# SixLabors/ZlibStream

Hardware: AMD Instinct MI355X
Metric: deflate MB/s (input) at level 6, 64 MiB buffers (higher is better)
Workload: dtype u8; 1 GPU; english64: 1 x 67108864-byte pseudo-random-English (Zipf words of alice29.txt) buffer per GPU, level 6, zlib framing, inputs resident in HBM; level=6, buffer_bytes=67108864, buffers_per_gpu=1, compressed_bytes=27425826, parallelism=independent buffers, 1 GPU(s), no collective in the data path

## Files before the change

### zlibstream_amd/csrc/zs_device.h

```cpp
#pragma once
#include <cstddef>
#include "zs_core.h"
#include "zs_lit_engine.h"
#include "zs_fast_sweep.h"
#include "zs_rle.h"

namespace zs {

constexpr int kMatchTile = 16384;
constexpr int kMatchBack = 32512;
constexpr int kMatchFwd = 272;
constexpr int kMatchLdsBytes = kMatchBack + kMatchTile + kMatchFwd;
constexpr int kMatchLdsLinks = kMatchBack + kMatchTile;
constexpr int kMatchLds = kMatchLdsBytes + 2 * kMatchLdsLinks;
constexpr int kAdlerPiece = 65536;

constexpr int64_t kScratchWindow = 0;
constexpr int64_t kScratchHead = 66560;
constexpr int64_t kScratchPrev = kScratchHead + 2 * kHashSize;
constexpr int64_t kScratchHead32 = kScratchPrev + 2 * kWSize;
constexpr int64_t kScratchBytes = kScratchHead32 + 4 * kHashSize;

struct StreamDesc {
    const uint8_t *in;
    uint8_t *out;
    int64_t out_cap;
    int64_t pos_off;
    int64_t sym_off;
    int32_t n;
    int32_t body_end;
    int32_t kl;
    int32_t nchunks;
    int32_t chunk_off;
    int32_t blk_off;
    int32_t max_blocks;
    int32_t adler_off;
    int32_t n_adler;
    int32_t fast_runs;
    int32_t run_off;
    int32_t run_slots;
    int32_t run_chunk;
    int32_t seg_off;
    int32_t nsegs;
    int32_t sup_off;
    const int32_t *seg_c0, *seg_after, *seg_base, *seg_S, *seg_cl;
    const uint32_t *cl;
    const int32_t *cstart;
    const int32_t *head;
    int32_t grid_chunks;
    int32_t n_wr;
    const int64_t *wr_end;
    const uint8_t *wr_flush;
    int32_t *wr_blk;
    int32_t out_chunk, raw;
    const BlockRec *plan_blk;
    int32_t plan_nblk;
    int32_t final_run;
    struct LitPersist *persist;
    int64_t abs_off;
    int32_t cont;
    int32_t resume, start_slot, cont_bits;
    int32_t mid_write;
    uint32_t start_syms;
    int64_t base0, start_block, persist_off, stop_abs;
    int64_t start_pos;
    uint32_t adler_stream;
    uint32_t carry_byte;
    int32_t fv_end;
    uint32_t *ins_bits;
    int32_t cut_off, cut_cap;
    int32_t rle_end, rle_tile_off;
    int32_t fr_first, fr_n;
    int32_t spec, spec_n, spec_off;
};

struct WorkOffsets {
    uint32_t off[10];
};
constexpr int kK5Feeders = 2;
constexpr int kK5Threads = 64 * (1 + kK5Feeders);
constexpr int kSupSegs = 16;
constexpr size_t kFvBitSlack = (16384 + 512) / 8 + 64;

struct LitPersist {
    int64_t base, avail_end, block_start_abs;
    int32_t strstart, lookahead, match_length, match_start, match_available, prev_length, prev_match;
    int32_t pending_syms;
    FlushAcct fa;
    int32_t fa_valid, stopped;
    int32_t good_prev, pad2_[3];
    uint8_t window[kWindowSize + 512];
    uint16_t prev[kWSize];
    uint16_t head[kHashSize];
    uint32_t syms[kLitBufsize];
};
static_assert(offsetof(LitPersist, window) % 16 == 0 && offsetof(LitPersist, prev) % 16 == 0 && offsetof(LitPersist, head) % 16 == 0, "16-byte copies");

struct StreamState {
    int32_t tail_p, tail_kind;
    uint32_t tail_pend;
    int32_t k_done, preins;
    uint32_t body_syms;
    uint32_t nsyms;
    int32_t nblocks;
    int64_t out_len;
    uint32_t adler;
    int32_t status;
    int64_t end_bits;
    int32_t r_seg, r_slot, r_kfired, r_kslot;
    uint32_t r_total;
    int32_t r_ncut;
    int32_t r_cut_e[8], r_cut_done[8];
    int32_t deferred, r_scan;
    int32_t r_cutidx;
    int32_t nc[2], cuts_same, cut_diff_idx, cut_diff_pos;
    int32_t poison;
    int32_t spec_run_tiles, spec_ok, spec_wrong;
};
constexpr uint32_t kSpecBail = 1u << 30;
ZS_HD uint32_t spec_pack(int guess, int exit_slot, int count, bool bail) {
    return (uint32_t)guess | ((uint32_t)exit_slot << 9) | ((uint32_t)count << 18) | (bail ? kSpecBail : 0u);
}
ZS_HD int spec_guess(uint32_t r) { return (int)(r & 0x1FF); }
ZS_HD int spec_exit(uint32_t r) { return (int)((r >> 9) & 0x1FF); }
ZS_HD int spec_count(uint32_t r) { return (int)((r >> 18) & 0xFFF); }
constexpr int kSpecMinInput = 1 << 20;
constexpr int kSpecLenBits = 10;
constexpr int kSpecWarm = 128;
constexpr int kSpecRunsDen = 8;
struct K5Spec {
    uint32_t *rec;
    uint32_t *base;
    int len_bits, warm, corrupt;
    uint32_t *syms;
    int stride;
};
static_assert(spec_slab_stride(kSpecMaxLenBits) - kSpecSlabPad <= 0xFFF, "spec_pack's count field holds the symbols of the longest chunk");
constexpr int kDeferBudget = 8;
constexpr int kCutBudget = 12;

constexpr int kFastChunk = 262144;
constexpr int kFastWarm = 65536;
constexpr int kFastMinInput = 4 << 20;
constexpr int kFastMinPeriodic = 64 << 10;
constexpr int64_t kFastRunSyms = kFastWarm + kFastChunk + 1024;
constexpr int64_t kFastRunBitWords = (kFastWarm + kFastChunk + 2048) / 32;
constexpr int64_t kFastRunScratch = 2 * kHashSize + 4 * kHashSize;
struct FastRunOut {
    int64_t mark_pos, mark_nsyms;
    int64_t end_pos, nsyms;
    int64_t final_base;
    int64_t sym_dst;
    int64_t ev[16];
    int64_t n_match;
    int32_t ok, n_ev;
};

struct BlockInfo {
    int32_t type;
    int32_t bits;
    int64_t bit_start;
};

}
```

### zlibstream_amd/csrc/zs_engine.hip

```cpp
#include <hip/hip_runtime.h>

#include <algorithm>
#include <cstdio>
#include <cstdlib>
#include <cstring>
#include <string>
#include <thread>
#include <vector>

#define ZS_BUILDING_LIBRARY
#include "../../include/zsgpu.h"
#include "zs_kernels.hip"
#include "zs_inflate_par.hip"
#include "zs_inflate_tok.hip"
#include "zs_png.hip"
#include "zs_crc32.hip"

using namespace zs;

namespace {

struct DevBuf {
    void *p = nullptr;
    size_t cap = 0;
};

enum Stage {
    kStClear, kStAdler, kStLinks, kStMatch, kStChunkMap, kStSegMap, kStResolve, kStExpand, kStEmitSyms, kStTail, kStTrees,
    kStOffsets, kStEmitBits, kStSpecWalk, kStSpecVerify, kStCrc32, kStSpecCompact, kStPngExpand, kStCount
};
const char *const kStageNames[kStCount] = {"clear", "adler", "links", "match", "chunkmap", "segmap", "resolve", "expand",
                                           "emit_syms", "tail", "trees", "offsets", "emit_bits", "spec_walk", "spec_verify", "crc32_frame",
                                           "spec_compact", "png_expand"};

}

struct zs_ctx {
    int device = 0;
    hipStream_t stream = nullptr;
    hipStream_t aux = nullptr;
    hipEvent_t ev_fork = nullptr, ev_join = nullptr, ev_pre0 = nullptr, ev_pre = nullptr;
    hipEvent_t ev_spec[4] = {};
    std::string err;
    bool profiling = false;
    int fast_fallbacks = 0;
    int round_runs = 0;
    int cut_rounds = 0;
    int lit_fallbacks = 0;
    int spec_streams = 0, spec_fallbacks = 0, spec_wrong_chunks = 0;
    int spec_periodic = 0;
    int64_t dbg_blk_off = 0, dbg_chunk_off = 0, dbg_nchunks = 0, dbg_spec_n = 0, dbg_n_spec = 0;
    int64_t lit_engine_bytes = 0;
    std::vector<int64_t> inf_used;
    int64_t *inf_probe = nullptr;
    int inf_lane_streams = 0;
    int64_t png_segments = 0;
    int fast_rounds = 0;
    bool no_rounds_once = false;
    int last_op = 0;
    hipEvent_t ev[kStCount + 1] = {};
    double stage_ms[kStCount] = {};
    uint32_t *crc_tab = nullptr;
    DevBuf sd, st, work, wpre, geo, link, mm, maps, chunk_far, segmap, supmap, seg_entry, seg_symbase, seg_stale, entry, symbase, stale, syms, blk_end, blk_top, blocks, trees, info, pieces, scratch,
        stage_in, stage_out, wr, inf_desc, inf_state, par_ps, par_st, par_work, par_cbits, par_ccnt, par_surv, par_scnt, par_cands, par_tabs, par_toktabs, par_toks, par_ctoks, par_tokstat, par_tails, par_retry, par_fxtab, par_blocks, par_cells,
        par_windows, par_fail, run_syms, run_bits, run_scratch, run_outs, run_fail, adl_tr, adl_res, plan_blk, ins_bits, mm_bak, cut_pos, cut_bkt, win_groups, win_sg, win_maps, win_entries, persist_bak, resume_flag, rle_tiles, own_in, fr_chunks, fr_meta, fr_planes, fr_prov, fr_base, fr_counters, spec_rec, spec_flags, spec_syms, png_img, png_seg, png_ctr, png_fimg, png_scratch, png_a7img, png_inflated, png_passes, crc_desc, crc_res, png_zs, png_gather, png_ximg, png_raw;
    uint32_t *crc32_tab = nullptr;
    hipEvent_t ev_crc[2] = {};
    hipEvent_t ev_expand[2] = {};
    bool resume_poisoned = false;
    void *pinned = nullptr;
    size_t pinned_cap = 0;
    void *pin_io = nullptr;
    size_t pin_io_cap = 0;
    bool pin_io_busy = false;
    void *pin_out = nullptr;
    size_t pin_out_cap = 0;
    bool pin_out_busy = false;
};

namespace {

bool fail(zs_ctx *c, const char *what, hipError_t e) {
    c->err = std::string(what) + ": " + hipGetErrorString(e);
    return false;
}
#define ZS_HIP(c, call)                                  \
    do {                                                 \
        hipError_t e_ = (call);                          \
        if (e_ != hipSuccess) return fail(c, #call, e_); \
    } while (0)

bool ensure(zs_ctx *c, DevBuf &b, size_t bytes) {
    if (bytes <= b.cap) return true;
    if (b.p) (void)hipFree(b.p);
    b.p = nullptr;
    b.cap = 0;
    size_t want = bytes + bytes / 8 + 4096;
    if (hipMalloc(&b.p, want) != hipSuccess) {
        (void)hipGetLastError();
        b.p = nullptr;
        want = bytes + 4096;
        if (hipMalloc(&b.p, want) != hipSuccess) {
            (void)hipGetLastError();
            b.p = nullptr;
            char msg[160];
            snprintf(msg, sizeof msg, "workspace: %zu bytes do not fit the device's free memory (the pipeline needs ~17 bytes per input byte: split the batch)", bytes);
            c->err = msg;
            return false;
        }
    }
    b.cap = want;
    return true;
}
bool ensure_pinned(zs_ctx *c, size_t bytes) {
    if (bytes <= c->pinned_cap) return true;
    if (c->pinned) (void)hipHostFree(c->pinned);
    c->pinned = nullptr;
    c->pinned_cap = 0;
    ZS_HIP(c, hipHostMalloc(&c->pinned, bytes + 4096, hipHostMallocDefault));
    c->pinned_cap = bytes + 4096;
    return true;
}

struct WorkList {
    std::vector<int32_t> pre;
    void add(int stream, int64_t count) {
        while ((int)pre.size() <= stream) pre.push_back(pre.empty() ? 0 : pre.back());
        pre.push_back(pre.back() + (int32_t)count);
    }
    void finish(int n) {
        if (pre.empty()) pre.push_back(0);
        while ((int)pre.size() <= n) pre.push_back(pre.back());
    }
    size_t size() const { return pre.empty() ? 0 : (size_t)pre.back(); }
    bool empty() const { return size() == 0; }
};
constexpr int kWorkLists = 9;
struct Plan {
    std::vector<StreamDesc> sd;
    WorkList w_clear, w_adler, w_links, w_match, w_chunks, w_segs, w_sups, w_blocks, w_runs;
    int64_t n_pos = 0, n_syms = 0;
    int64_t n_chunks = 0, n_segs = 0, n_sups = 0, n_blocks = 0, n_pieces = 0, n_runs = 0;
    int64_t n_spec = 0;
    int max_spec_n = 0, n_spec_streams = 0;
    bool any_fv = false, any_rle = false;
    bool any_dual = false;
    int64_t n_rle_tiles = 0;
    int64_t lit_bytes = 0;
    std::vector<FsChunk> fr_chunks;
    size_t fr_prov = 0;
    int fr_max_n = 0;
    int64_t n_cuts = 0;
    std::vector<int32_t> seg_c0, seg_after, seg_base, seg_S, seg_cl, cstart, head;
    std::vector<uint32_t> cl;
    std::vector<BlockRec> plan_blk;
    std::vector<int32_t> plan_wr_blk;
};

template <class T>
T *dev(DevBuf &b) {
    return (T *)b.p;
}

struct WriteSpec {
    std::vector<int64_t> ends;
    std::vector<uint8_t> flush;
    int chunk = 512;
    bool raw = false;
    bool flushing() const {
        for (uint8_t f : flush)
            if (f) return true;
        return false;
    }
};

struct RunOpts {
    bool final_run = true, cont = false;
    int64_t hist = 0;
    LitPersist *persist = nullptr;
    int64_t abs_off = 0;
    uint32_t adler_stream = 1, carry_byte = 0;
    int64_t end_bits = 0;
    int64_t stop_abs = -1;
    bool resume = false, mid_write = false, at_read = false;
    int64_t p0 = 0, E0 = 0, base0 = 0, start_block = 0;
    int slot = 0;
    uint32_t start_syms = 0;
};

bool run_pipeline(zs_ctx *c, int n, const void *const *in, const int64_t *in_len, void *const *out, const int64_t *out_cap,
                  int64_t *out_len, int *status, int level, int strategy, int hash_variant, hipStream_t stream,
                  const WriteSpec *const *writes = nullptr, int force_seq = 0, RunOpts *ro = nullptr, bool rounds = false,
                  const std::vector<uint8_t> *force_lit = nullptr) {
    if (level == -1) level = 6;
    LevelCfg lv = level_cfg(level);
    static const bool host_times = getenv("ZS_HOST_TIMES") != nullptr;
    const auto ht0 = std::chrono::steady_clock::now();
    auto ht_us = [&]() { return std::chrono::duration<double, std::micro>(std::chrono::steady_clock::now() - ht0).count(); };
    double ht_plan = 0, ht_launched = 0;
    for (int i = 0; i < n; i++) {
        out_len[i] = 0;
        if (status) status[i] = ZS_STREAM_ERROR;
    }
    bool any_writes = false;
    for (int i = 0; i < n && writes; i++) any_writes = any_writes || writes[i] != nullptr;
    if (any_writes && n > 1)
        for (int i = 0; i < n; i++)
            if (ro || (writes[i] && writes[i]->flushing())) {
                c->err = "flush modes and incremental runs take one stream a call";
                return false;
            }
    std::vector<WriteSpec> rle_one;
    std::vector<const WriteSpec *> rle_writes;
    if (any_writes && strategy == kRle && level >= 1 && !ro && !getenv("ZS_NO_RLE_MULTI")) {
        rle_one.resize((size_t)n);
        rle_writes.assign(writes, writes + n);
        for (int i = 0; i < n; i++) {
            const WriteSpec *wr = writes[i];
// ... 210 lines not shown
        }
    }
    {
        int64_t need = 0;
        for (int i = 0; i < n; i++) need += (pl.sd[(size_t)i].spec_n + 63) / 64;
        if (pl.n_spec && (int64_t)((pl.max_spec_n + 63) / 64) * n > 4 * need + 4096) {
            for (int i = 0; i < n; i++) pl.sd[(size_t)i].spec = 0, pl.sd[(size_t)i].spec_n = 0, pl.sd[(size_t)i].spec_off = 0;
            pl.n_spec = 0, pl.max_spec_n = 0, pl.n_spec_streams = 0;
        }
    }
    if (allow_dual && dual_broken) {
        allow_dual = false, dual_broken = false;
        goto plan_again;
    }
    pl.any_dual = allow_dual;
    c->lit_engine_bytes += pl.lit_bytes;
    auto plan_rerun = [&]() { c->lit_engine_bytes -= pl.lit_bytes; };
    c->fast_rounds = 0;
    const bool no_rounds_this_call = c->no_rounds_once;
    c->no_rounds_once = false;
    if (pl.any_fv && !getenv("ZS_FAST_NO_ROUNDS") && !no_rounds_this_call && !(ro && ro->resume && getenv("ZS_NO_RESUME_ROUNDS"))) {
        int64_t pos_fv = 0, max_fv = 0;
        for (int i = 0; i < n; i++)
            if (pl.sd[(size_t)i].fv_end >= 0) {
                pos_fv += pl.sd[(size_t)i].fv_end + 1 - pl.sd[(size_t)i].start_pos;
                max_fv = std::max<int64_t>(max_fv, pl.sd[(size_t)i].fv_end + 1 - pl.sd[(size_t)i].start_pos);
            }
        const double t_stream = (double)max_fv / (level >= 3 ? 20e6 : level == 2 ? 35e6 : 46e6);
        const double t_rounds = std::min(0.016, (double)max_fv / 60e6) + (double)pos_fv / 3.5e9;
        if (getenv("ZS_FR_RATIO") ? (double)pos_fv <= atof(getenv("ZS_FR_RATIO")) * (double)max_fv : t_rounds < t_stream) {
            int64_t target = getenv("ZS_FR_CHUNK") ? atoll(getenv("ZS_FR_CHUNK")) : pos_fv / 250;
            target = target < 2048 ? 2048 : target > kFsChunkMax ? kFsChunkMax : target;
            bool too_short = false;
            for (;;) {
                pl.fr_chunks.clear();
                pl.fr_max_n = 0;
                too_short = false;
                for (int i = 0; i < n; i++) {
                    StreamDesc &s = pl.sd[(size_t)i];
                    if (s.fv_end < 0) continue;
                    s.fr_first = (int32_t)pl.fr_chunks.size();
                    {
                        const int32_t *after = pl.seg_after.data() + s.seg_off;
                        const bool res = s.resume != 0;
                        const int64_t shortest = fs_build_chunks(i, (int64_t)s.fv_end, s.nsegs - 1, [&](int k) { return (int64_t)after[k - 1] - (kMinLookahead - 1); }, (int)target, pl.fr_chunks,
                                                                 res ? 2 : 1, res ? s.start_pos : 0);
                        if (shortest < kFsMinSpan) too_short = true;
                    }
                    s.fr_n = (int32_t)pl.fr_chunks.size() - s.fr_first;
                    pl.fr_max_n = s.fr_n > pl.fr_max_n ? s.fr_n : pl.fr_max_n;
                }
                if (pl.fr_chunks.size() <= 256 || target >= kFsChunkMax || getenv("ZS_FR_CHUNK")) break;
                target += 128;
            }
            if (too_short) {
                pl.fr_chunks.clear();
                pl.fr_max_n = 0;
                for (int i = 0; i < n; i++) pl.sd[(size_t)i].fr_first = pl.sd[(size_t)i].fr_n = 0;
            }
            for (FsChunk &ck : pl.fr_chunks) {
                ck.prov_off = (uint32_t)pl.fr_prov;
                pl.fr_prov += (size_t)(ck.b_hi - ck.b_lo) + kMaxMatch + 64;
            }
            if (pl.fr_prov > 0xFFFF0000u) {
                pl.fr_chunks.clear();
                pl.fr_max_n = 0, pl.fr_prov = 0;
                for (int i = 0; i < n; i++) pl.sd[(size_t)i].fr_first = pl.sd[(size_t)i].fr_n = 0;
            }
        }
    }
    WorkList *const lists[kWorkLists] = {&pl.w_clear, &pl.w_adler, &pl.w_links, &pl.w_match, &pl.w_chunks, &pl.w_segs, &pl.w_sups, &pl.w_blocks, &pl.w_runs};
    for (WorkList *l : lists) l->finish(n);
    size_t n_work = pl.w_clear.size() + pl.w_adler.size() + pl.w_links.size() + pl.w_match.size() + pl.w_chunks.size() +
                    pl.w_segs.size() + pl.w_sups.size() + pl.w_blocks.size() + pl.w_runs.size();
    if (!ensure(c, c->sd, sizeof(StreamDesc) * (size_t)n) || !ensure(c, c->st, sizeof(StreamState) * (size_t)n) ||
        !ensure(c, c->work, sizeof(uint2) * (n_work + 1)) || !ensure(c, c->link, 2 * (size_t)pl.n_pos + 64) ||
        !ensure(c, c->mm, 8 * (size_t)pl.n_pos + 256) ||
        !ensure(c, c->maps, 4 * (size_t)(pl.n_chunks + 1) * kSlots) || !ensure(c, c->segmap, 8 * (size_t)(pl.n_segs + 1) * kSlots) ||
        !ensure(c, c->supmap, 8 * (size_t)(pl.n_sups + 1) * kSlots) || !ensure(c, c->chunk_far, 2 * (size_t)pl.n_chunks + 64) ||
        !ensure(c, c->seg_entry, 2 * (size_t)(pl.n_segs + 2)) || !ensure(c, c->seg_symbase, 4 * (size_t)(pl.n_segs + 2)) ||
        !ensure(c, c->seg_stale, (size_t)pl.n_segs + 64) || !ensure(c, c->entry, 2 * (size_t)(pl.n_chunks + 2)) ||
        !ensure(c, c->symbase, 4 * (size_t)(pl.n_chunks + 2)) || !ensure(c, c->stale, (size_t)pl.n_chunks + 64) ||
        !ensure(c, c->syms, 4 * (size_t)pl.n_syms + 64) || !ensure(c, c->blk_end, 4 * (size_t)pl.n_blocks + 64) ||
        !ensure(c, c->blk_top, 4 * (size_t)pl.n_blocks + 64) || !ensure(c, c->blocks, sizeof(BlockRec) * (size_t)pl.n_blocks) ||
        !ensure(c, c->trees, sizeof(TreeWork) * (size_t)pl.n_blocks) || !ensure(c, c->info, sizeof(BlockInfo) * (size_t)pl.n_blocks) ||
        !ensure(c, c->pieces, 4 * (size_t)pl.n_pieces + 64) || !ensure(c, c->scratch, (size_t)kScratchBytes * (size_t)n) ||
        !ensure(c, c->cut_pos, 8 * (size_t)pl.n_cuts + 64) || !ensure(c, c->cut_bkt, 8 * (size_t)pl.n_cuts + 64) ||
        (pl.n_spec && (!ensure(c, c->spec_rec, 8 * (size_t)pl.n_spec + 64) || !ensure(c, c->spec_flags, 4 * (size_t)n + 64) ||
                       !ensure(c, c->spec_syms, 4 * (size_t)pl.n_spec * (size_t)spec_slab_stride(spec_bits) + 64))))
        return false;
    const size_t o_segcl = 16 * (size_t)pl.n_segs, o_cstart = o_segcl + 4 * ((size_t)pl.n_segs + (size_t)n),
                 o_head = o_cstart + 4 * ((size_t)pl.n_chunks + (size_t)n), o_cl = o_head + 4 * (size_t)pl.n_chunks;
    const size_t geo_bytes = o_cl + 4 * pl.cl.size();
    if (!ensure(c, c->geo, geo_bytes + 64)) return false;
    for (int i = 0; i < n; i++) {
        StreamDesc &s = pl.sd[(size_t)i];
        const int32_t *g = (const int32_t *)c->geo.p;
        const uint8_t *gb = (const uint8_t *)c->geo.p;
        s.seg_c0 = g + s.seg_off, s.seg_after = g + pl.n_segs + s.seg_off, s.seg_base = g + 2 * pl.n_segs + s.seg_off;
        s.seg_S = g + 3 * pl.n_segs + s.seg_off;
        s.seg_cl = (const int32_t *)(gb + o_segcl) + s.seg_off + i;
        s.cstart = (const int32_t *)(gb + o_cstart) + s.chunk_off + i;
        s.head = (const int32_t *)(gb + o_head) + s.chunk_off;
        s.cl = (const uint32_t *)(gb + o_cl);
    }
    if (pl.any_fv) {
        if (!ensure(c, c->ins_bits, (size_t)pl.n_pos / 8 + kFvBitSlack)) return false;
        for (int i = 0; i < n; i++)
            if (pl.sd[(size_t)i].fv_end >= 0) pl.sd[(size_t)i].ins_bits = dev<uint32_t>(c->ins_bits) + pl.sd[(size_t)i].pos_off / 32;
    }
    if (!pl.plan_blk.empty()) {
        if (!ensure(c, c->plan_blk, sizeof(BlockRec) * pl.plan_blk.size())) return false;
        for (int i = 0; i < n; i++)
            if (pl.sd[(size_t)i].plan_nblk) pl.sd[(size_t)i].plan_blk = dev<BlockRec>(c->plan_blk) + (uintptr_t)pl.sd[(size_t)i].plan_blk;
    }
    if (pl.n_runs &&
        (!ensure(c, c->run_syms, 4 * (size_t)pl.n_runs * kFastRunSyms) || !ensure(c, c->run_bits, 4 * (size_t)pl.n_runs * kFastRunBitWords) ||
         !ensure(c, c->run_scratch, (size_t)pl.n_runs * kFastRunScratch) || !ensure(c, c->run_outs, sizeof(FastRunOut) * (size_t)pl.n_runs) ||
         !ensure(c, c->run_fail, 4 * (size_t)n + 64)))
        return false;
    if (any_writes) {
        std::vector<size_t> nws((size_t)n, 0), offs;
        for (int i = 0; i < n; i++) {
            const WriteSpec *wr = writes[i];
            if (wr && (wr->ends.size() > 1 || wr->flushing() || ro)) nws[(size_t)i] = wr->ends.size();
        }
        const size_t wr_bytes = layout_write_blocks(nws, offs);
        if (!ensure(c, c->wr, wr_bytes + 64)) return false;
        std::vector<uint8_t> hw(rounds ? 0 : wr_bytes + 64, 0);
        for (int i = 0; i < n; i++) {
            const WriteSpec *wr = writes[i];
            const size_t nw = nws[(size_t)i];
            if (!wr || !(wr->ends.size() > 1 || wr->flushing() || ro)) continue;
            uint8_t *blk = (uint8_t *)c->wr.p + offs[(size_t)i];
            pl.sd[(size_t)i].wr_end = (const int64_t *)blk;
            if (wr->flushing() || ro) {
                pl.sd[(size_t)i].wr_blk = (int32_t *)(blk + 8 * nw);
                pl.sd[(size_t)i].wr_flush = blk + 12 * nw;
            }
            if (rounds || !nw) continue;
            memcpy(hw.data() + offs[(size_t)i], wr->ends.data(), sizeof(int64_t) * nw);
            if (wr->flushing() || ro) memcpy(hw.data() + offs[(size_t)i] + 12 * nw, wr->flush.data(), nw);
            if (!pl.plan_wr_blk.empty()) memcpy(hw.data() + offs[(size_t)i] + 8 * nw, pl.plan_wr_blk.data(), 4 * nw);
        }
        if (!rounds && wr_bytes) {
            ZS_HIP(c, hipMemcpyAsync(c->wr.p, hw.data(), hw.size(), hipMemcpyHostToDevice, stream));
            ZS_HIP(c, hipStreamSynchronize(stream));
        }
    }
    if (!rounds && !pl.plan_blk.empty()) {
        ZS_HIP(c, hipMemcpyAsync(c->plan_blk.p, pl.plan_blk.data(), sizeof(BlockRec) * pl.plan_blk.size(), hipMemcpyHostToDevice, stream));
        ZS_HIP(c, hipStreamSynchronize(stream));
    }
    const size_t pre_bytes = 4 * (size_t)kWorkLists * (size_t)(n + 1);
    size_t up_bytes = sizeof(StreamDesc) * (size_t)n + pre_bytes + geo_bytes + 16;
    if (!ensure_pinned(c, std::max(up_bytes, sizeof(StreamState) * (size_t)n)) || !ensure(c, c->wpre, pre_bytes + 64)) return false;
    uint8_t *hp = (uint8_t *)c->pinned;
    memcpy(hp, pl.sd.data(), sizeof(StreamDesc) * (size_t)n);
    int32_t *hpre = (int32_t *)(hp + sizeof(StreamDesc) * (size_t)n);
    size_t o_clear = 0, o_adler, o_links, o_match, o_chunks, o_segs, o_sups, o_blocks, o_runs;
    WorkOffsets wo;
    {
        size_t *const offs[kWorkLists] = {&o_clear, &o_adler, &o_links, &o_match, &o_chunks, &o_segs, &o_sups, &o_blocks, &o_runs};
        size_t at = 0;
        for (int l = 0; l < kWorkLists; l++) {
            *offs[l] = at;
            wo.off[l] = (uint32_t)at;
            memcpy(hpre + (size_t)l * (size_t)(n + 1), lists[l]->pre.data(), 4 * (size_t)(n + 1));
            at += lists[l]->size();
        }
        wo.off[kWorkLists] = (uint32_t)at;
    }
    if (geo_bytes) {
        uint8_t *hg = hp + sizeof(StreamDesc) * (size_t)n + pre_bytes;
        if (pl.n_segs) {
            memcpy(hg, pl.seg_c0.data(), 4 * (size_t)pl.n_segs);
            memcpy(hg + 4 * (size_t)pl.n_segs, pl.seg_after.data(), 4 * (size_t)pl.n_segs);
            memcpy(hg + 8 * (size_t)pl.n_segs, pl.seg_base.data(), 4 * (size_t)pl.n_segs);
            memcpy(hg + 12 * (size_t)pl.n_segs, pl.seg_S.data(), 4 * (size_t)pl.n_segs);
        }
        memcpy(hg + o_segcl, pl.seg_cl.data(), 4 * pl.seg_cl.size());
        memcpy(hg + o_cstart, pl.cstart.data(), 4 * pl.cstart.size());
        if (pl.n_chunks) memcpy(hg + o_head, pl.head.data(), 4 * (size_t)pl.n_chunks);
        if (!pl.cl.empty()) memcpy(hg + o_cl, pl.cl.data(), 4 * pl.cl.size());
        if (!rounds) ZS_HIP(c, hipMemcpyAsync(c->geo.p, hg, geo_bytes, hipMemcpyHostToDevice, stream));
    }
    if (!rounds) ZS_HIP(c, hipMemcpyAsync(c->sd.p, hp, sizeof(StreamDesc) * (size_t)n, hipMemcpyHostToDevice, stream));
    if (n_work && !rounds) {
        ZS_HIP(c, hipMemcpyAsync(c->wpre.p, hpre, pre_bytes, hipMemcpyHostToDevice, stream));
        hipLaunchKernelGGL(zs_worklist_kernel, dim3((unsigned)((n_work + 255) / 256)), dim3(256), 0, stream, dev<int32_t>(c->wpre), n, wo,
                           dev<uint2>(c->work));
    }
    if (!rounds) {
        ZeroRegions z;
        auto reg = [&](int r, DevBuf &b, size_t bytes) {
            z.p[r] = b.p;
            z.n16[r] = (uint32_t)(((bytes + 15) / 16 < b.cap / 16) ? (bytes + 15) / 16 : b.cap / 16);
        };
        reg(0, c->stale, (size_t)pl.n_chunks + 64);
        reg(1, c->seg_stale, (size_t)pl.n_segs + 64);
        reg(2, c->st, sizeof(StreamState) * (size_t)n);
        if (pl.any_fv) reg(3, c->ins_bits, (size_t)pl.n_pos / 8 + kFvBitSlack);
        else z.p[3] = nullptr, z.n16[3] = 0;
        uint32_t most = 0;
        for (int r = 0; r < 4; r++) most = z.n16[r] > most ? z.n16[r] : most;
        unsigned blocks = (most + 255) / 256;
        if (blocks > 2048) blocks = 2048;
        if (blocks < 1) blocks = 1;
        hipLaunchKernelGGL(zs_zero_kernel, dim3(blocks), dim3(256), 0, stream, z);
        if (ro && ro->resume && pl.sd[0].fv_end >= 0) {
            const int64_t lo = std::max<int64_t>(0, ro->p0 - kWSize - 64) / 32, hi = ro->p0 / 32;
            if (hi > lo) ZS_HIP(c, hipMemsetAsync(pl.sd[0].ins_bits + lo, 0xFF, (size_t)(hi - lo) * 4, stream));
            ZS_HIP(c, hipMemsetD32Async((hipDeviceptr_t)(pl.sd[0].ins_bits + hi), (int)((1u << (ro->p0 & 31)) - 1u), 1, stream));
        }
    }

    const StreamDesc *d_sd = dev<StreamDesc>(c->sd);
    StreamState *d_st = dev<StreamState>(c->st);
    const uint2 *d_work = dev<uint2>(c->work);
    const bool prof = c->profiling;
    const int k5_ahead = getenv("ZS_K5_AHEAD") ? atoi(getenv("ZS_K5_AHEAD")) : 1;
    c->dbg_blk_off = pl.sd[0].blk_off, c->dbg_chunk_off = pl.sd[0].chunk_off, c->dbg_nchunks = pl.sd[0].nchunks;
    c->dbg_spec_n = pl.sd[0].spec_n, c->dbg_n_spec = pl.n_spec;
    const K5Spec k5s{dev<uint32_t>(c->spec_rec), dev<uint32_t>(c->spec_rec) + pl.n_spec, spec_bits, spec_warm, spec_corrupt,
                     dev<uint32_t>(c->spec_syms), spec_slab_stride(spec_bits)};
    int spec_ok_streams = 0;
    bool need_maps = true, spec_ran = false;
    if (!rounds) c->spec_streams = c->spec_fallbacks = c->spec_wrong_chunks = c->spec_periodic = 0;
    auto mark = [&](int i) {
        if (prof) (void)hipEventRecord(c->ev[i], stream);
    };
    ht_plan = ht_us();
    ZS_HIP(c, hipEventRecord(c->ev_pre0, stream));
    auto side_work = [&]() -> bool {
        ZS_HIP(c, hipStreamWaitEvent(c->aux, c->ev_pre0, 0));
        if (!pl.w_clear.empty())
            hipLaunchKernelGGL(zs_clear_kernel, dim3((unsigned)pl.w_clear.size()), dim3(256), 0, c->aux, d_sd, d_work + o_clear);
        if (!pl.w_adler.empty())
            hipLaunchKernelGGL(zs_adler_kernel, dim3((unsigned)pl.w_adler.size()), dim3(256), 0, c->aux, d_sd, d_work + o_adler,
                               dev<uint32_t>(c->pieces));
        ZS_HIP(c, hipEventRecord(c->ev_pre, c->aux));
        return true;
    };
    const int cut_budget = getenv("ZS_FORCE_ROUNDS") ? 0 : kCutBudget;
    const int defer_mode = ((ro || getenv("ZS_NO_DEFER")) ? 0 : 1) | (getenv("ZS_DEBUG_CUTS") ? 0x100 : 0) | (cut_budget << 16);
    const int cut_stride = (int)pl.n_cuts;
    const bool use_sup = !pl.w_sups.empty() && !getenv("ZS_NO_SUPMAP");
    auto launch_resolve = [&](int mode, int iter) {
        hipLaunchKernelGGL(zs_resolve_kernel, dim3((unsigned)n), dim3(1024), kResolveLds, stream, d_sd, d_st, dev<uint16_t>(c->link),
                           dev<uint2>(c->mm), dev<uint32_t>(c->maps), dev<uint2>(c->segmap),
                           dev<uint16_t>(c->seg_entry), dev<uint32_t>(c->seg_symbase), dev<uint8_t>(c->stale),
                           dev<uint8_t>(c->seg_stale), c->crc_tab, lv, strategy, hash_variant, 0x7FFFFFFF, 0x7FFFFFFF,
                           use_sup ? dev<uint2>(c->supmap) : (const uint2 *)nullptr, dev<uint16_t>(c->chunk_far), mode, dev<int32_t>(c->cut_pos),
                           dev<uint32_t>(c->cut_bkt), cut_stride, iter);
    };
    auto run_cut_rounds = [&]() -> bool {
        const size_t far_off = 8 * (size_t)pl.n_pos + 256;
        if (!ensure(c, c->mm_bak, far_off + 2 * (size_t)pl.n_chunks + 64)) return false;
        ZS_HIP(c, hipMemcpyAsync(c->mm_bak.p, c->mm.p, 8 * (size_t)pl.n_pos + 256, hipMemcpyDeviceToDevice, stream));
        ZS_HIP(c, hipMemcpyAsync((uint8_t *)c->mm_bak.p + far_off, c->chunk_far.p, 2 * (size_t)pl.n_chunks + 64, hipMemcpyDeviceToDevice, stream));
        ZS_HIP(c, hipMemsetAsync(c->cut_pos.p, 0xFF, 8 * (size_t)pl.n_cuts + 64, stream));
        StreamState *hr = (StreamState *)c->pinned;
        for (int iter = 0;; iter++) {
            launch_resolve(3 | (defer_mode & 0x100), iter);
            ZS_HIP(c, hipMemcpyAsync(hr, d_st, sizeof(StreamState) * (size_t)n, hipMemcpyDeviceToHost, stream));
            ZS_HIP(c, hipStreamSynchronize(stream));
            bool all_same = true;
            int max_nc = 0;
            for (int i = 0; i < n; i++)
                if (hr[i].deferred == 1 && !hr[i].cuts_same) all_same = false, max_nc = std::max(max_nc, hr[i].nc[iter & 1]);
            hipLaunchKernelGGL(zs_cuts_apply_kernel, dim3((unsigned)n), dim3(256), 0, stream, d_sd, d_st, dev<uint16_t>(c->link), dev<int32_t>(c->cut_pos),
                               cut_stride, iter);
            if (getenv("ZS_DEBUG")) {
                int nd = 0, nsame = 0;
                for (int i = 0; i < n; i++) nd += hr[i].deferred == 1, nsame += hr[i].deferred == 1 && hr[i].cuts_same;
                fprintf(stderr, "zs: cut round %d: %d streams in the rounds, %d settled, most cuts %d, stream 0: %d cuts, first difference at cut %d (position %d)\n", iter,
                        nd, nsame, max_nc, hr[0].nc[iter & 1], hr[0].cut_diff_idx, hr[0].cut_diff_pos);
            }
            if (all_same && getenv("ZS_DEBUG_CUTS")) {
                const int ncap = hr[0].nc[iter & 1];
                std::vector<int32_t> cp((size_t)ncap);
                std::vector<uint32_t> cb((size_t)ncap);
                (void)hipMemcpy(cp.data(), dev<int32_t>(c->cut_pos) + (size_t)(iter & 1) * (size_t)cut_stride + pl.sd[0].cut_off, 4 * (size_t)ncap, hipMemcpyDeviceToHost);
                (void)hipMemcpy(cb.data(), dev<uint32_t>(c->cut_bkt) + (size_t)(iter & 1) * (size_t)cut_stride + pl.sd[0].cut_off, 4 * (size_t)ncap, hipMemcpyDeviceToHost);
                fprintf(stderr, "zs: cuts of stream 0 (slot: position / bucket):");
                for (int k = 0; k < ncap; k++)
                    if (cp[(size_t)k] >= 0) fprintf(stderr, " %d: %d / %u", k, cp[(size_t)k], cb[(size_t)k]);
                fprintf(stderr, "\n");
            }
            if (all_same) break;
            if (iter >= 4096) {
                c->err = "the cut rounds did not settle";
                return false;
            }
            c->cut_rounds++;
            if (iter > 0)
            hipLaunchKernelGGL(zs_cut_restore_kernel, dim3(2048, (unsigned)std::min(n, 65535)), dim3(256), 0, stream, d_sd, d_st, dev<uint2>(c->mm), (const uint2 *)c->mm_bak.p,
                               dev<uint8_t>(c->stale), dev<uint8_t>(c->seg_stale), dev<uint16_t>(c->chunk_far), (const uint16_t *)((const uint8_t *)c->mm_bak.p + far_off), n);
            if (max_nc > 0) {
                if (max_nc <= 64)
                    hipLaunchKernelGGL((zs_cuts_repair_kernel<256, 1>), dim3(128, (unsigned)max_nc, (unsigned)std::min(n, 65535)), dim3(256), kRepairLds, stream, d_sd, d_st,
                                       dev<uint16_t>(c->link), dev<uint2>(c->mm), dev<uint8_t>(c->stale), dev<uint8_t>(c->seg_stale),
                                       dev<uint16_t>(c->chunk_far), c->crc_tab, lv, hash_variant, dev<int32_t>(c->cut_pos), dev<uint32_t>(c->cut_bkt),
                                       cut_stride, iter, n);
                else if (max_nc <= 2048)
                    hipLaunchKernelGGL((zs_cuts_repair_kernel<256, 8>), dim3(16, (unsigned)max_nc, (unsigned)std::min(n, 65535)), dim3(256), kRepairLds, stream, d_sd, d_st,
                                       dev<uint16_t>(c->link), dev<uint2>(c->mm), dev<uint8_t>(c->stale), dev<uint8_t>(c->seg_stale),
                                       dev<uint16_t>(c->chunk_far), c->crc_tab, lv, hash_variant, dev<int32_t>(c->cut_pos), dev<uint32_t>(c->cut_bkt),
                                       cut_stride, iter, n);
                else
                    hipLaunchKernelGGL((zs_cuts_repair_kernel<1024, 32>), dim3(1, (unsigned)std::min(max_nc, 65535), (unsigned)std::min(n, 65535)), dim3(1024), kRepairLds, stream, d_sd,
                                       d_st, dev<uint16_t>(c->link), dev<uint2>(c->mm), dev<uint8_t>(c->stale), dev<uint8_t>(c->seg_stale),
                                       dev<uint16_t>(c->chunk_far), c->crc_tab, lv, hash_variant, dev<int32_t>(c->cut_pos), dev<uint32_t>(c->cut_bkt),
                                       cut_stride, iter, n);
            }
            hipLaunchKernelGGL(zs_chunkmap_kernel, dim3((unsigned)pl.w_chunks.size()), dim3(512), 0, stream, d_sd, d_work + o_chunks,
                               dev<uint2>(c->mm), dev<uint16_t>(c->link), dev<uint32_t>(c->maps), c->crc_tab, lv, strategy,
                               hash_variant, dev<uint16_t>(c->chunk_far), dev<uint8_t>(c->stale), (const StreamState *)d_st);
            hipLaunchKernelGGL(zs_segmap_kernel, dim3((unsigned)pl.w_segs.size()), dim3(320), 0, stream, d_sd, d_work + o_segs,
                               dev<uint32_t>(c->maps), dev<uint2>(c->segmap));
            ZS_HIP(c, hipMemsetAsync(c->seg_stale.p, 0, (size_t)pl.n_segs + 64, stream));
            if (use_sup)
                hipLaunchKernelGGL(zs_supmap_kernel, dim3((unsigned)pl.w_sups.size()), dim3(320), 0, stream, d_sd, d_work + o_sups,
                                   dev<uint2>(c->segmap), dev<uint8_t>(c->seg_stale), dev<uint2>(c->supmap));
        }
        return true;
    };
    if (!rounds) {
    mark(2);
    if (!pl.w_links.empty())
        hipLaunchKernelGGL(zs_links_kernel, dim3((unsigned)pl.w_links.size()), dim3(1024), kLkLds, stream, d_sd, d_work + o_links,
                           dev<uint16_t>(c->link), c->crc_tab, hash_variant, (int)link_span);
    if (ro && ro->resume)
        hipLaunchKernelGGL(zs_import_chains_kernel, dim3(64), dim3(1024), 0, stream, d_sd, 0, dev<uint16_t>(c->link), c->crc_tab, hash_variant, ro->p0);
    if (pl.any_dual) {
        bool periodic = true;
        if (!getenv("ZS_FAST_NO_PROBE")) {
            hipLaunchKernelGGL(zs_fast_probe_kernel, dim3((unsigned)n), dim3(256), 0, stream, d_sd, dev<uint16_t>(c->link), dev<int32_t>(c->run_fail));
            std::vector<int32_t> np((size_t)n, 0);
            ZS_HIP(c, hipMemcpyAsync(np.data(), c->run_fail.p, 4 * (size_t)n, hipMemcpyDeviceToHost, stream));
            ZS_HIP(c, hipStreamSynchronize(stream));
            for (int i = 0; i < n; i++) periodic = periodic && np[(size_t)i] == 0;
        }
        for (int i = 0; i < n; i++) {
            StreamDesc &sk = pl.sd[(size_t)i];
            if (periodic) sk.fv_end = -1, sk.fr_first = 0, sk.fr_n = 0;
            else sk.fast_runs = 0, sk.run_slots = 0;
        }
        if (periodic) pl.any_fv = false, pl.fr_chunks.clear(), pl.fr_max_n = 0;
        else pl.n_runs = 0;
        memcpy(c->pinned, pl.sd.data(), sizeof(StreamDesc) * (size_t)n);
        ZS_HIP(c, hipMemcpyAsync(c->sd.p, c->pinned, sizeof(StreamDesc) * (size_t)n, hipMemcpyHostToDevice, stream));
        if (getenv("ZS_DEBUG")) fprintf(stderr, "zs: %d stream(s) below 4 MiB at level %d: %s\n", n, level, periodic ? "all period, the speculative runs" : "the sweeps");
    }
    mark(3);
    if (strategy == kHuffmanOnly) {
        ZS_HIP(c, hipMemsetAsync(c->mm.p, 0, 8 * (size_t)pl.n_pos + 64, stream));
    } else if (!pl.w_match.empty())
        hipLaunchKernelGGL(zs_match_kernel, dim3((unsigned)pl.w_match.size()), dim3(1024), kMatchLds + 16, stream, d_sd, d_work + o_match,
                           dev<uint16_t>(c->link), dev<uint2>(c->mm), lv, strategy, d_st);
    mark(4);
    if (!side_work()) return false;
    if (pl.n_spec) {
        spec_ran = true;
        hipLaunchKernelGGL((zs_emit_syms_lane_kernel<4, 1>), dim3((unsigned)((pl.max_spec_n + 63) / 64), (unsigned)n), dim3(kK5Threads), 0, stream, d_sd, d_st,
                           (const uint2 *)nullptr, 0, dev<uint2>(c->mm), dev<uint16_t>(c->link), (const uint16_t *)nullptr, (const uint32_t *)nullptr,
                           (uint32_t *)nullptr, (int32_t *)nullptr, (int32_t *)nullptr, c->crc_tab, lv, strategy, hash_variant, k5_ahead, k5s);
        if (prof) (void)hipEventRecord(c->ev_spec[0], stream);
        hipLaunchKernelGGL(zs_spec_verify_kernel, dim3((unsigned)n), dim3(1024), 0, stream, d_sd, d_st, dev<uint2>(c->mm), dev<uint16_t>(c->link), c->crc_tab, lv,
                           strategy, hash_variant, k5s, dev<int32_t>(c->spec_flags));
        int32_t *hf = (int32_t *)c->pinned;
        ZS_HIP(c, hipMemcpyAsync(hf, c->spec_flags.p, 4 * (size_t)n, hipMemcpyDeviceToHost, stream));
        ZS_HIP(c, hipStreamSynchronize(stream));
        if (prof) (void)hipEventRecord(c->ev_spec[1], stream);
        for (int i = 0; i < n; i++) {
            if (hf[i] == 0) continue;
            c->spec_streams++;
            if (hf[i] == 1) spec_ok_streams++;
            else c->spec_fallbacks++;
            if (hf[i] == 2) c->spec_periodic++;
        }
        if (spec_ok_streams < c->spec_streams) {
            StreamState *hs = (StreamState *)c->pinned;
            ZS_HIP(c, hipMemcpyAsync(hs, d_st, sizeof(StreamState) * (size_t)n, hipMemcpyDeviceToHost, stream));
            ZS_HIP(c, hipStreamSynchronize(stream));
            for (int i = 0; i < n; i++) c->spec_wrong_chunks += hs[i].spec_wrong;
        }
        if (getenv("ZS_DEBUG"))
            fprintf(stderr, "zs: speculative walk: %d streams tried, %d verified, %d wrong guesses (chunks of %d, warm-up %d)\n", c->spec_streams, spec_ok_streams,
                    c->spec_wrong_chunks, 1 << spec_bits, spec_warm);
    }
    need_maps = spec_ok_streams < n;
    const StreamState *spec_st = spec_ok_streams ? (const StreamState *)d_st : nullptr;
    if (!pl.w_chunks.empty() && need_maps)
        hipLaunchKernelGGL(zs_chunkmap_kernel, dim3((unsigned)pl.w_chunks.size()), dim3(512), 0, stream, d_sd, d_work + o_chunks,
                           dev<uint2>(c->mm), dev<uint16_t>(c->link), dev<uint32_t>(c->maps), c->crc_tab, lv, strategy,
                           hash_variant, dev<uint16_t>(c->chunk_far), (uint8_t *)nullptr, (const StreamState *)nullptr, spec_st);
    mark(5);
    if (!pl.w_segs.empty() && need_maps)
        hipLaunchKernelGGL(zs_segmap_kernel, dim3((unsigned)pl.w_segs.size()), dim3(320), 0, stream, d_sd, d_work + o_segs,
                           dev<uint32_t>(c->maps), dev<uint2>(c->segmap), spec_st);
    if (use_sup && need_maps)
        hipLaunchKernelGGL(zs_supmap_kernel, dim3((unsigned)pl.w_sups.size()), dim3(320), 0, stream, d_sd, d_work + o_sups,
                           dev<uint2>(c->segmap), dev<uint8_t>(c->seg_stale), dev<uint2>(c->supmap), spec_st);
    mark(6);
    if (need_maps) launch_resolve(defer_mode, 0);
    }
    mark(7);
    if (pl.any_fv) {
        constexpr int fs_lds = fs_lds_bytes<1024, kFsTile1>();
        if (!pl.fr_chunks.empty()) {
            const size_t nch = pl.fr_chunks.size(), plane_words = (size_t)pl.n_pos / 32 + kFvBitSlack / 4 + 64;
            static const int env_max_rounds = getenv("ZS_FR_MAX_ROUNDS") ? atoi(getenv("ZS_FR_MAX_ROUNDS")) : 0;
            static const int env_range = getenv("ZS_FR_RANGE") ? std::max(1, atoi(getenv("ZS_FR_RANGE"))) : 0;
            static const int env_group = getenv("ZS_FR_GROUP") ? atoi(getenv("ZS_FR_GROUP")) : 4;
            static const int env_tail = getenv("ZS_FR_TAIL_RANGE") ? atoi(getenv("ZS_FR_TAIL_RANGE")) : 1;
            static const bool env_no_seed = getenv("ZS_FR_NO_SEED") != nullptr, env_fixed = getenv("ZS_FR_RANGE_FIXED") != nullptr, env_dbg = getenv("ZS_DEBUG") != nullptr;
            const int max_rounds = env_max_rounds ? env_max_rounds : pl.fr_max_n + 2;
            if (!ensure(c, c->fr_chunks, nch * sizeof(FsChunk)) || !ensure(c, c->fr_meta, 2 * nch * sizeof(FsMeta)) || !ensure(c, c->fr_planes, 16 * plane_words) ||
                !ensure(c, c->fr_prov, 4 * pl.fr_prov + 64) || !ensure(c, c->fr_base, 4 * nch + 64) || !ensure(c, c->fr_counters, 4 * ((size_t)max_rounds + 16))) {
                c->err.clear();
                ZS_HIP(c, hipStreamSynchronize(c->aux));
                ZS_HIP(c, hipStreamSynchronize(stream));
                c->no_rounds_once = true;
                return plan_rerun(), run_pipeline(c, n, in, in_len, out, out_cap, out_len, status, level, strategy, hash_variant, stream, writes, force_seq, ro, false, force_lit);
            }
            ZS_HIP(c, hipMemcpyAsync(c->fr_chunks.p, pl.fr_chunks.data(), nch * sizeof(FsChunk), hipMemcpyHostToDevice, stream));
            ZS_HIP(c, hipMemsetAsync(c->fr_counters.p, 0, 4 * ((size_t)max_rounds + 16), stream));
            const int range_max = env_range ? env_range : nch >= 512 ? (int)((nch + 255) / 256) : 1;
            FsRounds fr{dev<FsChunk>(c->fr_chunks), dev<FsMeta>(c->fr_meta), dev<uint32_t>(c->fr_planes), dev<uint32_t>(c->fr_prov), dev<uint32_t>(c->fr_counters),
                        (int64_t)plane_words, (int)nch, 0, env_no_seed ? 1 : 0, range_max};
            const int group = env_group;
            uint32_t changed = 1;
            int r = 0;
            std::string trace;
            while (r < max_rounds && changed) {
                const int g_n = fr.range > 1 ? 1 : group;
                const unsigned n_wg = (unsigned)((nch + (size_t)fr.range - 1) / (size_t)fr.range);
                for (int g = 0; g < g_n && r < max_rounds; g++, r++) {
                    fr.round = r;
                    hipLaunchKernelGGL((zs_fast_sweep_kernel<1024, kFsTile1, true>), dim3(n_wg), dim3(1024), fs_lds, stream, d_sd, d_st, dev<uint16_t>(c->link),
                                       dev<uint32_t>(c->syms), dev<int32_t>(c->blk_end), dev<int32_t>(c->blk_top), lv, strategy, fr);
                }
                ZS_HIP(c, hipMemcpyAsync(&changed, dev<uint32_t>(c->fr_counters) + (r - 1), 4, hipMemcpyDeviceToHost, stream));
                ZS_HIP(c, hipStreamSynchronize(stream));
                if (env_dbg) {
                    static auto t_last = std::chrono::steady_clock::now();
                    const auto t_now = std::chrono::steady_clock::now();
                    char b[64];
                    snprintf(b, sizeof b, " %u/%d(%.2f)", changed, fr.range, r <= g_n ? 0.0 : std::chrono::duration<double, std::milli>(t_now - t_last).count());
                    t_last = t_now;
                    trace += b;
                }
                if (!env_fixed) {
                    static const double env_wake = getenv("ZS_FR_WAKE") ? atof(getenv("ZS_FR_WAKE")) : 4.0;
                    const size_t awake = std::min<size_t>(nch, (size_t)(env_wake * (double)changed));
                    const int tail = env_tail;
                    fr.range = std::min<int>(range_max, std::max<int>(tail, (int)((awake + 255) / 256)));
                }
            }
            c->fast_rounds = r;
            if (env_dbg) fprintf(stderr, "zs: DeflateFast over %zu chunks of %d streams, up to %d to a workgroup: %d rounds (changed/range:%s)\n", nch, n, range_max, r, trace.c_str());
            if (changed) {
                ZS_HIP(c, hipStreamSynchronize(c->aux));
                c->no_rounds_once = true;
                return plan_rerun(), run_pipeline(c, n, in, in_len, out, out_cap, out_len, status, level, strategy, hash_variant, stream, writes, force_seq, ro, false, force_lit);
            }
            const FsMeta *mf = dev<FsMeta>(c->fr_meta) + (size_t)((r - 1) & 1) * nch;
            hipLaunchKernelGGL(zs_fast_commit_scan_kernel, dim3((unsigned)n), dim3(1024), 0, stream, d_sd, d_st, mf, dev<int32_t>(c->fr_base));
            hipLaunchKernelGGL(zs_fast_commit_kernel, dim3((unsigned)nch), dim3(256), 0, stream, d_sd, fr, mf, dev<int32_t>(c->fr_base), dev<uint16_t>(c->link),
                               dev<uint32_t>(c->syms), dev<int32_t>(c->blk_end), dev<int32_t>(c->blk_top));
        } else {
            hipLaunchKernelGGL((zs_fast_sweep_kernel<1024, kFsTile1, false>), dim3((unsigned)n), dim3(1024), fs_lds, stream, d_sd, d_st, dev<uint16_t>(c->link),
                               dev<uint32_t>(c->syms), dev<int32_t>(c->blk_end), dev<int32_t>(c->blk_top), lv, strategy, FsRounds());
        }
    }
    if (pl.any_rle) {
        const size_t nt = (size_t)pl.n_rle_tiles;
        if (!ensure(c, c->rle_tiles, 4 * (4 * nt + (size_t)n) + 256)) return false;
        int32_t *rb = dev<int32_t>(c->rle_tiles);
        RleTiles rt{rb, rb + nt, rb + 2 * nt, rb + 3 * nt, rb + 4 * nt};
        int max_tiles = 0;
        for (int i = 0; i < n; i++)
            if (pl.sd[(size_t)i].rle_end >= 0) max_tiles = std::max(max_tiles, (pl.sd[(size_t)i].rle_end + kMaxMatch + 1 + 4095) / 4096);
        auto tiles = [&](auto &&launch) {
            for (int s0 = 0; s0 < n; s0 += 65535) launch(dim3((unsigned)((max_tiles + 3) / 4), (unsigned)std::min(n - s0, 65535)), s0);
        };
        tiles([&](dim3 tg, int s0) { hipLaunchKernelGGL(zs_rle_starts_kernel, tg, dim3(256), 0, stream, d_sd, rt, s0); });
        hipLaunchKernelGGL(zs_rle_scan_kernel, dim3((unsigned)n), dim3(1024), 0, stream, d_sd, rt);
        tiles([&](dim3 tg, int s0) {
            hipLaunchKernelGGL(zs_rle_pass_kernel<0>, tg, dim3(256), 0, stream, d_sd, rt, dev<uint32_t>(c->syms), dev<int32_t>(c->blk_end), dev<int32_t>(c->blk_top), s0);
        });
        hipLaunchKernelGGL(zs_rle_sums_kernel, dim3((unsigned)n), dim3(1024), 0, stream, d_sd, d_st, rt);
        tiles([&](dim3 tg, int s0) {
            hipLaunchKernelGGL(zs_rle_pass_kernel<1>, tg, dim3(256), 0, stream, d_sd, rt, dev<uint32_t>(c->syms), dev<int32_t>(c->blk_end), dev<int32_t>(c->blk_top), s0);
        });
    }
    const bool tail_late = ro && (!ro->final_run || ro->resume);
    const bool tail_serial = !tail_late && n >= 64 && (pl.n_pos / n >= (96 << 10) || getenv("ZS_TAIL_SERIAL")) && !getenv("ZS_TAIL_FORK");
    if (!tail_late && !tail_serial) {
        ZS_HIP(c, hipEventRecord(c->ev_fork, stream));
        ZS_HIP(c, hipStreamWaitEvent(c->aux, c->ev_fork, 0));
        hipLaunchKernelGGL(zs_tail_kernel, dim3((unsigned)n), dim3(1024), kTailLds, c->aux, d_sd, d_st, dev<uint16_t>(c->link),
                           dev<uint32_t>(c->syms), dev<int32_t>(c->blk_end), dev<int32_t>(c->blk_top), dev<BlockRec>(c->blocks),
                           dev<uint8_t>(c->scratch), c->crc_tab, lv, strategy, hash_variant, level);
        ZS_HIP(c, hipEventRecord(c->ev_join, c->aux));
    }
    if (!pl.w_segs.empty() && need_maps)
        hipLaunchKernelGGL(zs_expand_kernel, dim3((unsigned)((pl.w_segs.size() + 63) / 64)), dim3(64), 0, stream, d_sd, d_st,
                           d_work + o_segs, (int)pl.w_segs.size(), dev<uint2>(c->mm), dev<uint16_t>(c->link),
                           dev<uint32_t>(c->maps), dev<uint16_t>(c->seg_entry), dev<uint32_t>(c->seg_symbase),
                           dev<uint8_t>(c->stale), dev<uint16_t>(c->entry), dev<uint32_t>(c->symbase), c->crc_tab, lv, strategy,
                           hash_variant);
    mark(8);
    if (!pl.w_chunks.empty() && need_maps)
        hipLaunchKernelGGL((zs_emit_syms_lane_kernel<4, 0>), dim3((unsigned)((pl.w_chunks.size() + 63) / 64)), dim3(kK5Threads), 0, stream, d_sd, d_st,
                           d_work + o_chunks, (int)pl.w_chunks.size(), dev<uint2>(c->mm), dev<uint16_t>(c->link), dev<uint16_t>(c->entry),
                           dev<uint32_t>(c->symbase), dev<uint32_t>(c->syms), dev<int32_t>(c->blk_end), dev<int32_t>(c->blk_top),
                           c->crc_tab, lv, strategy, hash_variant, k5_ahead, k5s);
    if (spec_ok_streams) {
        if (prof) (void)hipEventRecord(c->ev_spec[2], stream);
        hipLaunchKernelGGL(zs_spec_compact_kernel, dim3((unsigned)((pl.max_spec_n + 3) / 4), (unsigned)n), dim3(256), 0, stream, d_sd, d_st, k5s,
                           dev<uint32_t>(c->syms), dev<int32_t>(c->blk_end), dev<int32_t>(c->blk_top));
        if (prof) (void)hipEventRecord(c->ev_spec[3], stream);
    }
    mark(9);
    if (tail_serial)
        hipLaunchKernelGGL(zs_tail_kernel, dim3((unsigned)n), dim3(1024), kTailLds, stream, d_sd, d_st, dev<uint16_t>(c->link),
                           dev<uint32_t>(c->syms), dev<int32_t>(c->blk_end), dev<int32_t>(c->blk_top), dev<BlockRec>(c->blocks),
                           dev<uint8_t>(c->scratch), c->crc_tab, lv, strategy, hash_variant, level);
    else if (!tail_late) ZS_HIP(c, hipStreamWaitEvent(stream, c->ev_join, 0));
    hipLaunchKernelGGL(zs_body_blocks_kernel, dim3((unsigned)n), dim3(256), 0, stream, d_sd, d_st, dev<int32_t>(c->blk_end),
                       dev<int32_t>(c->blk_top), dev<BlockRec>(c->blocks), dev<uint32_t>(c->syms));
    if (tail_late)
        hipLaunchKernelGGL(zs_tail_kernel, dim3((unsigned)n), dim3(1024), kTailLds, stream, d_sd, d_st, dev<uint16_t>(c->link),
                           dev<uint32_t>(c->syms), dev<int32_t>(c->blk_end), dev<int32_t>(c->blk_top), dev<BlockRec>(c->blocks),
                           dev<uint8_t>(c->scratch), c->crc_tab, lv, strategy, hash_variant, level);
    if (pl.n_runs) {
        if (!getenv("ZS_FAST_NO_PROBE") && force_seq == 0 && !pl.any_dual) {
            hipLaunchKernelGGL(zs_fast_probe_kernel, dim3((unsigned)n), dim3(256), 0, stream, d_sd, dev<uint16_t>(c->link), dev<int32_t>(c->run_fail));
            std::vector<int32_t> np((size_t)n, 0);
            ZS_HIP(c, hipMemcpyAsync(np.data(), c->run_fail.p, 4 * (size_t)n, hipMemcpyDeviceToHost, stream));
            ZS_HIP(c, hipStreamSynchronize(stream));
            for (int i = 0; i < n; i++)
                if (np[(size_t)i]) {
                    ZS_HIP(c, hipStreamSynchronize(c->aux));
                    return plan_rerun(), run_pipeline(c, n, in, in_len, out, out_cap, out_len, status, level, strategy, hash_variant, stream, writes, 1, ro, false, force_lit);
                }
        }
        ZS_HIP(c, hipMemsetAsync(c->run_fail.p, 0, 4 * (size_t)n + 64, stream));
        hipLaunchKernelGGL(zs_fast_run_kernel, dim3((unsigned)pl.w_runs.size()), dim3(1024), kFastRunLds, stream, d_sd, d_work + o_runs,
                           dev<uint16_t>(c->link), dev<uint32_t>(c->run_syms), dev<uint32_t>(c->run_bits), dev<uint8_t>(c->run_scratch),
                           dev<FastRunOut>(c->run_outs), c->crc_tab, lv, strategy, hash_variant);
        hipLaunchKernelGGL(zs_fast_verify_kernel, dim3((unsigned)pl.w_runs.size()), dim3(256), 0, stream, d_sd, d_work + o_runs,
                           dev<uint32_t>(c->run_bits), dev<FastRunOut>(c->run_outs), dev<int32_t>(c->run_fail));
        std::vector<int32_t> rfail((size_t)n, 0);
        ZS_HIP(c, hipMemcpyAsync(rfail.data(), c->run_fail.p, 4 * (size_t)n, hipMemcpyDeviceToHost, stream));
        ZS_HIP(c, hipStreamSynchronize(stream));
        for (int i = 0; i < n; i++)
            if (rfail[(size_t)i]) {
                ZS_HIP(c, hipStreamSynchronize(c->aux));
                c->fast_fallbacks++;
                std::vector<FastRunOut> outs((size_t)pl.n_runs);
                ZS_HIP(c, hipMemcpy(outs.data(), c->run_outs.p, sizeof(FastRunOut) * outs.size(), hipMemcpyDeviceToHost));
                if (getenv("ZS_DEBUG"))
                    for (int j = 0; j < pl.sd[(size_t)i].fast_runs; j++) {
                        const FastRunOut &o = outs[(size_t)pl.sd[(size_t)i].run_off + j];
                        fprintf(stderr, "zs: stream %d run %d ok=%d mark=%lld (+%lld syms) end=%lld nsyms=%lld n_ev=%d\n", i, j, o.ok,
                                (long long)o.mark_pos, (long long)o.mark_nsyms, (long long)o.end_pos, (long long)o.nsyms, o.n_ev);
                    }
                double t_engine = 0, t_sweeps = 0;
                for (int k = 0; k < n; k++) {
                    const StreamDesc &sk = pl.sd[(size_t)k];
                    if (sk.fast_runs <= 0) continue;
                    int64_t syms = 0, matches = 0;
                    for (int j = 0; j < sk.fast_runs; j++) syms += outs[(size_t)sk.run_off + j].nsyms, matches += outs[(size_t)sk.run_off + j].n_match;
                    const double scale = sk.fast_runs > 1 ? 0.8 : 1.0;
                    const double te = scale * (1.2e-6 * (double)matches + 0.03e-6 * (double)(syms - matches)) + (double)sk.n / 1.5e9;
                    if (getenv("ZS_DEBUG")) fprintf(stderr, "zs: stream %d: ~%.0f symbols one at a time, ~%.0f in runs of literals, %d bytes\n", k, scale * (double)matches, scale * (double)(syms - matches), sk.n);
                    t_engine = std::max(t_engine, te);
                    t_sweeps = std::max(t_sweeps, (double)sk.n / (level >= 3 ? 20e6 : level == 2 ? 35e6 : 46e6));
                }
                const int mode = (force_seq == 0 && !getenv("ZS_NO_WHOLE_RUNS") && (getenv("ZS_WHOLE_RUNS") || t_engine < 0.7 * t_sweeps)) ? 2 : 1;
                if (getenv("ZS_DEBUG")) fprintf(stderr, "zs: the runs did not verify: %s (engine %.1f ms, sweeps up to %.1f ms)\n", mode == 2 ? "one run per stream" : "the sweeps", t_engine * 1e3, t_sweeps * 1e3);
                return plan_rerun(), run_pipeline(c, n, in, in_len, out, out_cap, out_len, status, level, strategy, hash_variant, stream, writes, mode, ro, false, force_lit);
            }
        hipLaunchKernelGGL(zs_fast_plan_kernel, dim3((unsigned)n), dim3(256), 0, stream, d_sd, d_st, dev<FastRunOut>(c->run_outs), n);
        hipLaunchKernelGGL(zs_fast_stitch_kernel, dim3((unsigned)pl.w_runs.size()), dim3(256), 0, stream, d_sd, d_work + o_runs,
                           dev<uint32_t>(c->run_syms), dev<FastRunOut>(c->run_outs), dev<uint32_t>(c->syms), dev<int32_t>(c->blk_end),
                           dev<int32_t>(c->blk_top));
        hipLaunchKernelGGL(zs_fast_blocks_kernel, dim3((unsigned)n), dim3(64), 0, stream, d_sd, d_st, dev<FastRunOut>(c->run_outs),
                           dev<int32_t>(c->blk_end), dev<int32_t>(c->blk_top), dev<BlockRec>(c->blocks), n);
    }
    mark(10);
    const int trees_threads = pl.w_blocks.size() > 8192 ? 128 : 256;
    if (n >= 64 && !getenv("ZS_NO_LIVE_LIST")) {
        hipLaunchKernelGGL(zs_live_scan_kernel, dim3(1), dim3(1024), 0, stream, d_st, n, dev<int32_t>(c->wpre));
        hipLaunchKernelGGL(zs_live_fill_kernel, dim3((unsigned)((pl.w_blocks.size() + 255) / 256)), dim3(256), 0, stream, dev<int32_t>(c->wpre), n,
                           (uint32_t)pl.w_blocks.size(), dev<uint2>(c->work) + o_blocks);
    }
    hipLaunchKernelGGL(zs_trees_kernel, dim3((unsigned)pl.w_blocks.size()), dim3(trees_threads), 0, stream, d_sd, d_st, d_work + o_blocks,
                       dev<uint32_t>(c->syms), dev<BlockRec>(c->blocks), dev<TreeWork>(c->trees), dev<BlockInfo>(c->info), strategy, level, 2);
    mark(11);
    ZS_HIP(c, hipStreamWaitEvent(stream, c->ev_pre, 0));
    hipLaunchKernelGGL(zs_offsets_kernel, dim3((unsigned)n), dim3(256), 0, stream, d_sd, d_st, dev<BlockRec>(c->blocks),
                       dev<BlockInfo>(c->info), dev<TreeWork>(c->trees), dev<uint32_t>(c->pieces), level, n);
    mark(12);
    hipLaunchKernelGGL(zs_emit_bits_kernel, dim3((unsigned)pl.w_blocks.size()), dim3(256), 0, stream, d_sd, d_st, d_work + o_blocks,
                       dev<uint32_t>(c->syms), dev<BlockRec>(c->blocks), dev<TreeWork>(c->trees), dev<BlockInfo>(c->info));
    mark(13);
    ZS_HIP(c, hipGetLastError());
    StreamState *hst = (StreamState *)c->pinned;
    ZS_HIP(c, hipMemcpyAsync(hst, d_st, sizeof(StreamState) * (size_t)n, hipMemcpyDeviceToHost, stream));
    ht_launched = ht_us();
    ZS_HIP(c, hipStreamSynchronize(stream));
    if (host_times) fprintf(stderr, "zs: host: plan + uploads %.0f us, all launched at %.0f us, device done at %.0f us\n", ht_plan, ht_launched, ht_us());
    c->last_op = lv.func == 1 ? 2 : 0;
    if (getenv("ZS_DEBUG_CHAIN") && n == 1) {
        const int64_t q0 = atoll(getenv("ZS_DEBUG_CHAIN")) - (ro ? ro->abs_off : 0);
        if (q0 > 0 && q0 < in_len[0]) {
            std::vector<uint16_t> lk((size_t)in_len[0]);
            (void)hipMemcpy(lk.data(), dev<uint16_t>(c->link) + pl.sd[0].pos_off, 2 * (size_t)in_len[0], hipMemcpyDeviceToHost);
            fprintf(stderr, "[zs] run of %lld bytes (stream position %lld on), resume %d at %lld: chain of %lld:", (long long)in_len[0], (long long)(ro ? ro->abs_off : 0),
                    pl.sd[0].resume, (long long)pl.sd[0].start_pos, (long long)q0);
            int64_t q = q0;
            int hops = 0;
            const int64_t want = getenv("ZS_DEBUG_CHAIN_WANT") ? atoll(getenv("ZS_DEBUG_CHAIN_WANT")) - (ro ? ro->abs_off : 0) : -1;
            int want_at = -1;
            while (lk[(size_t)q] && hops < 100000) {
                q -= lk[(size_t)q], hops++;
                if (hops <= 12) fprintf(stderr, " %lld", (long long)q);
                if (q == want) want_at = hops;
            }
            fprintf(stderr, " ... %d hops, ends at %lld; position %lld is hop %d\n", hops, (long long)q, (long long)want, want_at);
        }
    }
    if (getenv("ZS_DEBUG_FA") && writes && writes[0] && pl.sd[0].wr_blk) {
        const WriteSpec *wr = writes[0];
        const size_t nw = wr->ends.size();
        std::vector<int32_t> wb(nw);
        (void)hipMemcpy(wb.data(), pl.sd[0].wr_blk, 4 * nw, hipMemcpyDeviceToHost);
        fprintf(stderr, "[zs] run of %lld bytes, %zu Writes, %d blocks, body ends at %d, resume %d; blocks before each Write:", (long long)in_len[0], nw, hst[0].nblocks,
                pl.sd[0].body_end, pl.sd[0].resume);
        for (size_t k = 0; k < nw && k < 24; k++) fprintf(stderr, " %d(end %lld, flush %d)", wb[k], (long long)wr->ends[k], wr->flush.empty() ? 0 : wr->flush[k]);
        fprintf(stderr, "\n");
    }
    if (prof) {
        for (int i = 0; i < kStCount; i++) {
            float ms = 0;
            if (i >= kStLinks && i <= kStEmitBits) (void)hipEventElapsedTime(&ms, c->ev[i], c->ev[i + 1]);
            c->stage_ms[i] = ms;
        }
        if (spec_ran) {
            float a = 0, b = 0, m = 0;
            (void)hipEventElapsedTime(&a, c->ev[kStChunkMap], c->ev_spec[0]);
            (void)hipEventElapsedTime(&b, c->ev_spec[0], c->ev_spec[1]);
            (void)hipEventElapsedTime(&m, c->ev_spec[1], c->ev[kStChunkMap + 1]);
            c->stage_ms[kStSpecWalk] = a, c->stage_ms[kStSpecVerify] = b, c->stage_ms[kStChunkMap] = m;
            float k = 0;
            if (spec_ok_streams) (void)hipEventElapsedTime(&k, c->ev_spec[2], c->ev_spec[3]);
            c->stage_ms[kStSpecCompact] = k;
        }
    }
    {
        bool any_poison = false;
        std::vector<uint8_t> fl(force_lit ? *force_lit : std::vector<uint8_t>((size_t)n, 0));
        for (int i = 0; i < n; i++)
            if (hst[i].poison) any_poison = true, fl[(size_t)i] = 1;
        if (any_poison) {
            ZS_HIP(c, hipStreamSynchronize(c->aux));
            if (ro && ro->resume) {
                c->err = "the resumed run met a read the bulk pipeline leaves to the literal engine";
                c->resume_poisoned = true;
                return false;
            }
            c->lit_fallbacks++;
            return plan_rerun(), run_pipeline(c, n, in, in_len, out, out_cap, out_len, status, level, strategy, hash_variant, stream, writes, force_seq, ro, false, &fl);
        }
    }
    if (!ro && !rounds) {
        bool gave_up = false;
        for (int i = 0; i < n; i++) gave_up = gave_up || hst[i].deferred == 1;
        if (gave_up) {
            ZS_HIP(c, hipStreamSynchronize(c->aux));
            c->round_runs++;
            if (!run_cut_rounds()) return false;
            return plan_rerun(), run_pipeline(c, n, in, in_len, out, out_cap, out_len, status, level, strategy, hash_variant, stream, writes, force_seq, ro, true, force_lit);
        }
    }
    if (ro) ro->end_bits = hst[0].end_bits;
    bool all_ok = true;
    for (int i = 0; i < n; i++) {
        out_len[i] = hst[i].out_len;
        if (status) status[i] = hst[i].status;
        if (hst[i].status != 0 && all_ok) {
            c->err = hst[i].status == ZS_BUF_ERROR ? "buffer error"
                                                   : "stored block larger than the reference's pending buffer (the managed engine throws here)";
            all_ok = false;
        }
    }
    return all_ok;
}

bool device_adlers(zs_ctx *c, int m, const void *const *bufs, const int64_t *lens, const void *const *trailers, uint32_t *adlers,
                   int *ok, hipStream_t stream) {
    if (m <= 0) return true;
    std::vector<StreamDesc> sd((size_t)m);
    std::vector<uint2> work;
    int64_t n_pieces = 0;
    for (int i = 0; i < m; i++) {
        StreamDesc &s = sd[(size_t)i];
        memset(&s, 0, sizeof s);
        s.in = (const uint8_t *)bufs[i];
        s.n = (int32_t)lens[i];
        s.adler_off = (int32_t)n_pieces;
        s.n_adler = (int32_t)((lens[i] + kAdlerPiece - 1) / kAdlerPiece);
        n_pieces += s.n_adler;
        for (int k = 0; k < s.n_adler; k++) work.push_back(make_uint2((unsigned)i, (unsigned)k));
    }
    const size_t b_sd = sizeof(StreamDesc) * (size_t)m, b_work = sizeof(uint2) * work.size(), b_tr = sizeof(void *) * (size_t)m;
    if (!ensure(c, c->sd, b_sd) || !ensure(c, c->work, b_work + 16) || !ensure(c, c->pieces, 4 * (size_t)n_pieces + 64) ||
        !ensure(c, c->adl_tr, b_tr) || !ensure(c, c->adl_res, sizeof(uint2) * (size_t)m) ||
        !ensure_pinned(c, b_sd + b_work + b_tr + sizeof(uint2) * (size_t)m))
        return false;
    uint8_t *hp = (uint8_t *)c->pinned;
    memcpy(hp, sd.data(), b_sd);
    if (b_work) memcpy(hp + b_sd, work.data(), b_work);
    if (trailers) memcpy(hp + b_sd + b_work, trailers, b_tr);
    ZS_HIP(c, hipMemcpyAsync(c->sd.p, hp, b_sd, hipMemcpyHostToDevice, stream));
    if (b_work) ZS_HIP(c, hipMemcpyAsync(c->work.p, hp + b_sd, b_work, hipMemcpyHostToDevice, stream));
    if (trailers) ZS_HIP(c, hipMemcpyAsync(c->adl_tr.p, hp + b_sd + b_work, b_tr, hipMemcpyHostToDevice, stream));
    if (!work.empty())
        hipLaunchKernelGGL(zs_adler_kernel, dim3((unsigned)work.size()), dim3(256), 0, stream, dev<StreamDesc>(c->sd), dev<uint2>(c->work),
                           dev<uint32_t>(c->pieces));
    hipLaunchKernelGGL(zs_adler_finish_kernel, dim3((unsigned)m), dim3(256), 0, stream, dev<StreamDesc>(c->sd), dev<uint32_t>(c->pieces),
                       trailers ? (const uint8_t *const *)c->adl_tr.p : nullptr, dev<uint2>(c->adl_res));
    uint2 *hres = (uint2 *)(hp + b_sd + b_work + b_tr);
    ZS_HIP(c, hipMemcpyAsync(hres, c->adl_res.p, sizeof(uint2) * (size_t)m, hipMemcpyDeviceToHost, stream));
    ZS_HIP(c, hipStreamSynchronize(stream));
    for (int i = 0; i < m; i++) {
        if (adlers) adlers[i] = hres[i].x;
        if (ok) ok[i] = (int)hres[i].y;
    }
    return true;
}

int batch_prefix_that_fits(zs_ctx *c, int n, const int64_t *in_len, const int64_t *out_cap, int lo, int per_byte) {
    size_t free_b = 0, total_b = 0;
    if (hipMemGetInfo(&free_b, &total_b) != hipSuccess) return n;
    const DevBuf *held[] = {&c->link, &c->mm, &c->maps, &c->segmap, &c->supmap, &c->syms, &c->trees, &c->blocks, &c->info, &c->stage_in, &c->stage_out,
                            &c->scratch, &c->ins_bits, &c->mm_bak};
    size_t have = 0;
    for (const DevBuf *b : held) have += b->cap;
    const double budget = 0.55 * ((double)free_b + (double)have);
    double need = 0;
    int hi = lo;
    while (hi < n) {
        const double add = (double)in_len[hi] * per_byte + (per_byte > 19 ? (double)out_cap[hi] : 0.0) + 4.0e6;
        if (hi > lo && need + add > budget) break;
        need += add;
        hi++;
    }
    return hi;
}

bool check_args(zs_ctx *c, int n, const int64_t *in_len, int level, int strategy) {
    if (!c) return false;
    if (n < 0 || level < -1 || level > 9 || strategy < 0 || strategy > 4) {
        c->err = "stream error";
        return false;
    }
    for (int i = 0; i < n; i++)
        if (in_len[i] < 0 || in_len[i] > 0x7FFFFFFF - 1024) {
            c->err = "stream error";
            return false;
        }
    return true;
}

}

extern "C" {

void zs_ctx_destroy(zs_ctx *c);
int zs_ctx_create(int device, zs_ctx **out) {
    if (!out) return ZS_STREAM_ERROR;
    *out = nullptr;
    int count = 0;
    if (hipGetDeviceCount(&count) != hipSuccess || count <= 0 || device < 0 || device >= count) return ZS_STREAM_ERROR;
    if (hipSetDevice(device) != hipSuccess) return ZS_STREAM_ERROR;
    zs_ctx *c = new zs_ctx();
    c->device = device;
    if (hipStreamCreateWithFlags(&c->stream, hipStreamNonBlocking) != hipSuccess) {
        zs_ctx_destroy(c);
        return ZS_MEM_ERROR;
    }
    for (auto &e : c->ev) (void)hipEventCreate(&e);
    for (auto &e : c->ev_spec) (void)hipEventCreate(&e);
    for (auto &e : c->ev_crc) (void)hipEventCreate(&e);
    for (auto &e : c->ev_expand) (void)hipEventCreate(&e);
    {
        int *d_ok = nullptr, ok = 0;
        if (hipMalloc((void **)&d_ok, sizeof(int)) != hipSuccess) {
            zs_ctx_destroy(c);
            return ZS_MEM_ERROR;
        }
        hipLaunchKernelGGL(zs_lds_order_kernel, dim3(1), dim3(64), 0, c->stream, d_ok);
        const bool copied = hipMemcpyAsync(&ok, d_ok, sizeof(int), hipMemcpyDeviceToHost, c->stream) == hipSuccess &&
                            hipStreamSynchronize(c->stream) == hipSuccess;
        (void)hipFree(d_ok);
        if (!copied || !ok) {
            fprintf(stderr, "zsgpu: LDS lane-order self-test failed on device %d; this build cannot run there\n", device);
            zs_ctx_destroy(c);
            return ZS_STREAM_ERROR;
        }
    }
    if (hipStreamCreateWithFlags(&c->aux, hipStreamNonBlocking) != hipSuccess ||
        hipEventCreateWithFlags(&c->ev_fork, hipEventDisableTiming) != hipSuccess ||
        hipEventCreateWithFlags(&c->ev_join, hipEventDisableTiming) != hipSuccess ||
        hipEventCreateWithFlags(&c->ev_pre0, hipEventDisableTiming) != hipSuccess ||
        hipEventCreateWithFlags(&c->ev_pre, hipEventDisableTiming) != hipSuccess) {
        zs_ctx_destroy(c);
        return ZS_MEM_ERROR;
    }
    std::vector<uint32_t> tab(1024);
    for (int t = 0; t < 4; t++)
        for (int i = 0; i < 256; i++) tab[(size_t)t * 256 + i] = crc32c_table_entry(t, (uint32_t)i);
    if (hipMalloc((void **)&c->crc_tab, 4096) != hipSuccess ||
        hipMemcpy(c->crc_tab, tab.data(), 4096, hipMemcpyHostToDevice) != hipSuccess ||
        hipFuncSetAttribute((const void *)zs_match_kernel, hipFuncAttributeMaxDynamicSharedMemorySize, kMatchLds + 16) != hipSuccess ||
        hipFuncSetAttribute((const void *)zs_resolve_kernel, hipFuncAttributeMaxDynamicSharedMemorySize, kResolveLds) != hipSuccess ||
        hipFuncSetAttribute((const void *)zs_links_kernel, hipFuncAttributeMaxDynamicSharedMemorySize, kLkLds) != hipSuccess ||
        hipFuncSetAttribute((const void *)zs_tail_kernel, hipFuncAttributeMaxDynamicSharedMemorySize, kTailLds) != hipSuccess ||
        hipFuncSetAttribute((const void *)zs_fast_run_kernel, hipFuncAttributeMaxDynamicSharedMemorySize, kFastRunLds) != hipSuccess ||
        hipFuncSetAttribute((const void *)zs_fast_sweep_kernel<1024, kFsTile1, false>, hipFuncAttributeMaxDynamicSharedMemorySize, (fs_lds_bytes<1024, kFsTile1>())) != hipSuccess ||
        hipFuncSetAttribute((const void *)zs_fast_sweep_kernel<1024, kFsTile1, true>, hipFuncAttributeMaxDynamicSharedMemorySize, (fs_lds_bytes<1024, kFsTile1>())) != hipSuccess ||
        hipFuncSetAttribute((const void *)zs_inf_window_kernel, hipFuncAttributeMaxDynamicSharedMemorySize, kWinMapLds) != hipSuccess ||
        hipFuncSetAttribute((const void *)zs_inf_chain_par_kernel, hipFuncAttributeMaxDynamicSharedMemorySize, kChainParLds) != hipSuccess ||
        hipFuncSetAttribute((const void *)zs_inf_expand_kernel, hipFuncAttributeMaxDynamicSharedMemorySize, kExpLds) != hipSuccess ||
        hipFuncSetAttribute((const void *)zs_cuts_repair_kernel<256, 1>, hipFuncAttributeMaxDynamicSharedMemorySize, kRepairLds) != hipSuccess ||
        hipFuncSetAttribute((const void *)zs_cuts_repair_kernel<256, 8>, hipFuncAttributeMaxDynamicSharedMemorySize, kRepairLds) != hipSuccess ||
        hipFuncSetAttribute((const void *)zs_cuts_repair_kernel<1024, 32>, hipFuncAttributeMaxDynamicSharedMemorySize, kRepairLds) != hipSuccess ||
        hipFuncSetAttribute((const void *)zs_png_unfilter_kernel, hipFuncAttributeMaxDynamicSharedMemorySize, kPngMaxLds) != hipSuccess ||
        hipFuncSetAttribute((const void *)zs_inflate_kernel, hipFuncAttributeMaxDynamicSharedMemorySize, kInfLds) != hipSuccess) {
        zs_ctx_destroy(c);
        return ZS_MEM_ERROR;
    }
    hipFuncAttributes fa;
    if (hipFuncGetAttributes(&fa, (const void *)zs_match_kernel) != hipSuccess || fa.sharedSizeBytes != 0) {
        fprintf(stderr, "zsgpu: zs_match_kernel has static LDS; its tile addressing assumes none\n");
        zs_ctx_destroy(c);
        return ZS_STREAM_ERROR;
    }
    *out = c;
    return ZS_OK;
}

void zs_ctx_destroy(zs_ctx *c) {
    if (!c) return;
    (void)hipSetDevice(c->device);
    DevBuf *bufs[] = {&c->sd, &c->st, &c->work, &c->wpre, &c->geo, &c->link, &c->mm, &c->maps, &c->chunk_far, &c->segmap, &c->supmap, &c->seg_entry, &c->seg_symbase, &c->seg_stale, &c->entry, &c->symbase, &c->stale, &c->syms,
                      &c->blk_end, &c->blk_top, &c->blocks, &c->trees, &c->info, &c->pieces, &c->scratch, &c->stage_in, &c->stage_out, &c->wr, &c->inf_desc, &c->inf_state, &c->par_ps, &c->par_st, &c->par_work, &c->par_cbits, &c->par_ccnt, &c->par_surv, &c->par_scnt,
                      &c->par_cands, &c->par_tabs, &c->par_toktabs, &c->par_toks, &c->par_ctoks, &c->par_tokstat, &c->par_tails, &c->par_retry, &c->par_fxtab, &c->par_blocks, &c->par_cells, &c->par_windows, &c->par_fail, &c->run_syms, &c->run_bits,
                      &c->run_scratch, &c->run_outs, &c->run_fail, &c->adl_tr, &c->adl_res, &c->plan_blk, &c->ins_bits, &c->mm_bak, &c->cut_pos, &c->cut_bkt, &c->win_groups, &c->win_sg, &c->win_maps, &c->win_entries, &c->persist_bak, &c->resume_flag, &c->rle_tiles, &c->own_in, &c->fr_chunks, &c->fr_meta, &c->fr_planes, &c->fr_prov, &c->fr_base, &c->fr_counters, &c->spec_rec, &c->spec_flags, &c->spec_syms, &c->png_img, &c->png_seg, &c->png_ctr, &c->png_fimg, &c->png_scratch, &c->png_a7img, &c->png_inflated, &c->png_passes, &c->crc_desc, &c->crc_res, &c->png_zs, &c->png_gather, &c->png_ximg, &c->png_raw};
    for (DevBuf *b : bufs)
        if (b->p) (void)hipFree(b->p);
    if (c->crc_tab) (void)hipFree(c->crc_tab);
    if (c->crc32_tab) (void)hipFree(c->crc32_tab);
    for (auto &e : c->ev_crc)
        if (e) (void)hipEventDestroy(e);
    for (auto &e : c->ev_expand)
        if (e) (void)hipEventDestroy(e);
    if (c->pinned) (void)hipHostFree(c->pinned);
    if (c->pin_io) (void)hipHostFree(c->pin_io);
    if (c->pin_out) (void)hipHostFree(c->pin_out);
    for (auto &e : c->ev)
        if (e) (void)hipEventDestroy(e);
    for (auto &e : c->ev_spec)
        if (e) (void)hipEventDestroy(e);
    if (c->ev_fork) (void)hipEventDestroy(c->ev_fork);
    if (c->ev_join) (void)hipEventDestroy(c->ev_join);
    if (c->ev_pre0) (void)hipEventDestroy(c->ev_pre0);
    if (c->ev_pre) (void)hipEventDestroy(c->ev_pre);
    if (c->aux) (void)hipStreamDestroy(c->aux);
    if (c->stream) (void)hipStreamDestroy(c->stream);
    delete c;
}

const char *zs_ctx_last_error(const zs_ctx *c) { return c ? c->err.c_str() : "no context"; }

int64_t zs_deflate_bound(int64_t n) { return n + (n >> 3) + 1024; }

void zs_ctx_set_profiling(zs_ctx *c, int enable) {
    if (c) c->profiling = enable != 0;
}
int zs_ctx_stage_count(const zs_ctx *) { return kStCount; }
int64_t zs_ctx_counter(const zs_ctx *c, const char *name) {
    if (!c || !name) return -1;
    const std::string k(name);
    if (k == "fast_rounds") return c->fast_rounds;
    if (k == "fast_fallbacks") return c->fast_fallbacks;
    if (k == "round_runs") return c->round_runs;
    if (k == "cut_rounds") return c->cut_rounds;
    if (k == "lit_fallbacks") return c->lit_fallbacks;
    if (k == "lit_engine_bytes") return c->lit_engine_bytes;
    if (k == "spec_streams") return c->spec_streams;
    if (k == "spec_fallbacks") return c->spec_fallbacks;
    if (k == "spec_periodic") return c->spec_periodic;
    if (k == "spec_wrong_chunks") return c->spec_wrong_chunks;
    if (k == "inf_lane_streams") return c->inf_lane_streams;
    if (k == "png_segments") return c->png_segments;
    return -1;
}

int64_t zs_ctx_debug_read(zs_ctx *c, const char *name, void *out, int64_t cap) {
    if (!c || !name || !out || !c->st.p) return -1;
    const std::string k(name);
    (void)hipSetDevice(c->device);
    StreamState ss;
    if (hipMemcpy(&ss, c->st.p, sizeof ss, hipMemcpyDeviceToHost) != hipSuccess) return -1;
    const void *src = nullptr;
    int64_t bytes = 0;
    const int32_t state[6] = {ss.tail_p, ss.tail_kind, (int32_t)ss.tail_pend, ss.k_done, ss.preins, (int32_t)ss.body_syms};
    if (k == "state") {
        if (cap < (int64_t)sizeof state) return -1;
        memcpy(out, state, sizeof state);
        return sizeof state;
    }
    if (k == "blk_end") src = dev<int32_t>(c->blk_end) + c->dbg_blk_off, bytes = 4 * (int64_t)(ss.body_syms / kBlockSyms);
    else if (k == "blk_top") src = dev<int32_t>(c->blk_top) + c->dbg_blk_off, bytes = 4 * (int64_t)(ss.body_syms / kBlockSyms);
    else if (k == "symbase") src = dev<uint32_t>(c->symbase) + c->dbg_chunk_off, bytes = 4 * c->dbg_nchunks;
    else if (k == "spec_base") src = dev<uint32_t>(c->spec_rec) + c->dbg_n_spec, bytes = 4 * c->dbg_spec_n;
    else return -1;
    if (bytes > cap || (bytes > 0 && !src)) return -1;
    if (bytes > 0 && hipMemcpy(out, src, (size_t)bytes, hipMemcpyDeviceToHost) != hipSuccess) return -1;
    return bytes;
}

const char *zs_ctx_stage_name(const zs_ctx *c, int s) {
    static const char *const inf_names[6] = {"inf_find", "inf_measure", "inf_chain", "inf_decode", "inf_windows", "inf_resolve"};
    if (s == kStCrc32 || s == kStSpecCompact || s == kStPngExpand) return kStageNames[s];
    if (c && c->last_op == 1) return s >= 0 && s < 6 ? inf_names[s] : "";
    if (c && c->last_op == 2 && s == kStExpand) return "fast_sweep";
    if (c && c->last_op == 2 && s == kStTail) return "fast_runs+tail";
    return s >= 0 && s < kStCount ? kStageNames[s] : "";
}
double zs_ctx_stage_ms(const zs_ctx *c, int s) { return c && s >= 0 && s < kStCount ? c->stage_ms[s] : 0.0; }

int zs_deflate_batch_device(zs_ctx *c, int n, const void *const *in, const int64_t *in_len, void *const *out,
                            const int64_t *out_cap, int64_t *out_len, int *status, int level, int strategy, int hash_variant,
                            void *hip_stream) {
    if (!check_args(c, n, in_len, level, strategy)) return ZS_STREAM_ERROR;
    if (n == 0) return ZS_OK;
    if (hipSetDevice(c->device) != hipSuccess) return ZS_STREAM_ERROR;
    hipStream_t s = hip_stream ? (hipStream_t)hip_stream : c->stream;
    int rc = ZS_OK;
    for (int lo = 0; lo < n;) {
        const int hi = batch_prefix_that_fits(c, n, in_len, out_cap, lo, 19);
        if (!run_pipeline(c, hi - lo, in + lo, in_len + lo, out + lo, out_cap + lo, out_len + lo, status ? status + lo : nullptr, level, strategy,
                          hash_variant, s) && rc == ZS_OK)
            rc = c->err == "buffer error" ? ZS_BUF_ERROR : ZS_STREAM_ERROR;
        lo = hi;
    }
    return rc;
}

int zs_deflate_writes_batch_device(zs_ctx *c, int n, const void *const *in, const int64_t *in_len, const int64_t *const *write_ends,
                                   const int64_t *n_writes, void *const *out, const int64_t *out_cap, int64_t *out_len, int *status, int level,
                                   int strategy, int hash_variant, void *hip_stream) {
    if (!write_ends) return zs_deflate_batch_device(c, n, in, in_len, out, out_cap, out_len, status, level, strategy, hash_variant, hip_stream);
    if (!check_args(c, n, in_len, level, strategy)) return ZS_STREAM_ERROR;
    if (n == 0) return ZS_OK;
    std::vector<WriteSpec> specs((size_t)n);
    std::vector<const WriteSpec *> ptrs((size_t)n, nullptr);
    for (int i = 0; i < n; i++) {
        if (!write_ends[i] || (n_writes && n_writes[i] <= 0)) continue;
        if (!n_writes || !write_list_ends(write_ends[i], n_writes[i], in_len[i], specs[(size_t)i].ends)) {
            c->err = "stream error";
            return ZS_STREAM_ERROR;
        }
        if (specs[(size_t)i].ends.empty()) continue;
        specs[(size_t)i].flush.assign(specs[(size_t)i].ends.size(), 0);
        ptrs[(size_t)i] = &specs[(size_t)i];
    }
    if (hipSetDevice(c->device) != hipSuccess) return ZS_STREAM_ERROR;
    hipStream_t s = hip_stream ? (hipStream_t)hip_stream : c->stream;
    int rc = ZS_OK;
    for (int lo = 0; lo < n;) {
        const int hi = batch_prefix_that_fits(c, n, in_len, out_cap, lo, 19);
        if (!run_pipeline(c, hi - lo, in + lo, in_len + lo, out + lo, out_cap + lo, out_len + lo, status ? status + lo : nullptr, level, strategy,
                          hash_variant, s, ptrs.data() + lo) && rc == ZS_OK)
            rc = c->err == "buffer error" ? ZS_BUF_ERROR : ZS_STREAM_ERROR;
        lo = hi;
    }
    return rc;
}

int zs_deflate_writes_device(zs_ctx *c, const void *in, int64_t in_len, const int64_t *write_ends, int64_t n_writes, void *out,
                             int64_t out_cap, int64_t *out_len, int level, int strategy, int hash_variant, void *hip_stream) {
    if (!check_args(c, 1, &in_len, level, strategy)) return ZS_STREAM_ERROR;
    if (hipSetDevice(c->device) != hipSuccess) return ZS_STREAM_ERROR;
    WriteSpec ws;
    if (!write_list_ends(write_ends, n_writes, in_len, ws.ends)) {
        c->err = "stream error";
        return ZS_STREAM_ERROR;
    }
    ws.flush.assign(ws.ends.size(), 0);
    const WriteSpec *const one = &ws;
    hipStream_t s = hip_stream ? (hipStream_t)hip_stream : c->stream;
    int st = 0;
    if (!run_pipeline(c, 1, &in, &in_len, &out, &out_cap, out_len, &st, level, strategy, hash_variant, s, ws.ends.size() > 1 ? &one : nullptr))
        return c->err == "buffer error" ? ZS_BUF_ERROR : ZS_STREAM_ERROR;
    return ZS_OK;
}

namespace {
int deflate_batch_host_once(zs_ctx *c, int n, const void *const *in, const int64_t *in_len, void *const *out, const int64_t *out_cap,
                            int64_t *out_len, int *status, int level, int strategy, int hash_variant) {
    std::vector<const void *> din((size_t)n);
    std::vector<void *> dout((size_t)n);
    std::vector<int64_t> dcap((size_t)n);
    size_t tin = 0, tout = 0;
    for (int i = 0; i < n; i++) {
        tin += ((size_t)in_len[i] + 255) & ~(size_t)255;
        dcap[(size_t)i] = out_cap[i];
        tout += ((size_t)out_cap[i] + 255) & ~(size_t)255;
    }
    auto chk = [&](hipError_t e, const char *what) {
        if (e != hipSuccess) fail(c, what, e);
        return e == hipSuccess;
    };
    if (!ensure(c, c->stage_in, tin + 256) || !ensure(c, c->stage_out, tout + 256)) return ZS_MEM_ERROR;
    size_t oi = 0, oo = 0;
    for (int i = 0; i < n; i++) {
        din[(size_t)i] = (uint8_t *)c->stage_in.p + oi;
        dout[(size_t)i] = (uint8_t *)c->stage_out.p + oo;
        if (in_len[i] &&
            !chk(hipMemcpyAsync((void *)din[(size_t)i], in[i], (size_t)in_len[i], hipMemcpyHostToDevice, c->stream), "H2D"))
            return ZS_STREAM_ERROR;
        oi += ((size_t)in_len[i] + 255) & ~(size_t)255;
        oo += ((size_t)out_cap[i] + 255) & ~(size_t)255;
    }
    std::vector<int> st_local;
    if (!status) st_local.assign((size_t)n, 0), status = st_local.data();
    const bool ok = run_pipeline(c, n, din.data(), in_len, dout.data(), dcap.data(), out_len, status, level, strategy, hash_variant, c->stream);
    const std::string first_err = c->err;
    for (int i = 0; i < n; i++)
        if (status[i] == 0 && out_len[i] > 0 && out_len[i] <= out_cap[i] &&
            !chk(hipMemcpyAsync(out[i], dout[(size_t)i], (size_t)out_len[i], hipMemcpyDeviceToHost, c->stream), "D2H"))
            return ZS_STREAM_ERROR;
    if (!chk(hipStreamSynchronize(c->stream), "sync")) return ZS_STREAM_ERROR;
    if (!ok) {
        c->err = first_err;
        return first_err == "buffer error" ? ZS_BUF_ERROR : ZS_STREAM_ERROR;
    }
    return ZS_OK;
}
}

int zs_deflate_batch(zs_ctx *c, int n, const void *const *in, const int64_t *in_len, void *const *out, const int64_t *out_cap,
                     int64_t *out_len, int *status, int level, int strategy, int hash_variant) {
    if (!check_args(c, n, in_len, level, strategy)) return ZS_STREAM_ERROR;
// ... 1559 lines not shown
```

### zlibstream_amd/csrc/zs_kernels.hip

```cpp
#include <hip/hip_runtime.h>

#include <type_traits>

#include "zs_device.h"
#include "zs_png.h"

namespace zs {

typedef uint32_t __attribute__((aligned(1))) u32u;
typedef uint64_t __attribute__((aligned(1))) u64u;
typedef const __attribute__((address_space(1))) uint8_t *gcbytes;
typedef __attribute__((address_space(1))) uint8_t *gbytes_w;
__device__ __forceinline__ gcbytes as_global(const uint8_t *p) { return (gcbytes)(uintptr_t)p; }
__device__ __forceinline__ gbytes_w as_global(uint8_t *p) { return (gbytes_w)(uintptr_t)p; }
typedef const __attribute__((address_space(1))) uint32_t __attribute__((aligned(1))) *gcu32u;
typedef const __attribute__((address_space(1))) uint64_t __attribute__((aligned(1))) *gcu64u;
__device__ __forceinline__ uint32_t g_u32_bytes(gcbytes p) {
    return (uint32_t)p[0] | ((uint32_t)p[1] << 8) | ((uint32_t)p[2] << 16) | ((uint32_t)p[3] << 24);
}
typedef uint32_t u32x4 __attribute__((ext_vector_type(4)));
typedef const __attribute__((address_space(1))) u32x4 *gcu32x4;
__device__ __forceinline__ uint32_t lds_u32(const uint8_t *base, int idx) {
    const uint32_t *q = (const uint32_t *)(base + (idx & ~3));
    return __builtin_amdgcn_alignbyte(q[1], q[0], (uint32_t)idx & 3u);
// ... 940 lines not shown
                    if (!snap && (n_eval == k4 || nice_exit)) ny = best >= kMinMatch ? pack_match(best, bdist) : kNoMatch, snap = true;
                    if (nice_exit || n_eval == lv.chain) break;
                    l = lkf(c);
                    if (!l) break;
                    c -= l;
                    if (c < 1 || q - c >= kMaxDist) break;
                }
                nx = best >= kMinMatch ? pack_match(best, bdist) : kNoMatch;
                if (!snap) ny = nx;
            }
        }
        if (nx != x || ny != y) {
            a[p] = make_uint2(nx | (old.x & ~kRecMask), ny);
            int cp = chunk_of(s, p);
            for (int k = 0; k < 2; k++) {
                const int cc = cp + k;
                if (k == 1 && !(p + 1 == (int64_t)s.cstart[cp + 1] && cp + 1 < nch)) break;
                r.seg_stale[s.seg_off + seg_of(s, cc)] = 1;
                r.stale[s.chunk_off + cc] = 1;
                if (mark && cc - c0r >= 0 && cc - c0r < 24 && atomicExch(&mark[cc - c0r], 1u) == 0) {
                    const int at = atomicAdd(nlist, 1);
                    if (at < 24) list[at] = cc;
                }
            }
        }
    }
    __threadfence();
    __syncthreads();
    return 2;
}

__global__ __launch_bounds__(1024) void zs_resolve_kernel(const StreamDesc *sd, StreamState *st, uint16_t *link, uint2 *mm,
                                                         uint32_t *maps, const uint2 *segmap,
                                                         uint16_t *seg_entry, uint32_t *seg_symbase, uint8_t *stale,
                                                         uint8_t *seg_stale, const uint32_t *crc_tab_g, LevelCfg lv,
                                                         int strategy, int hash_variant, int seg_limit, int mm_limit,
                                                         const uint2 *supmap, const uint16_t *chunk_far, int defer_mode_in,
                                                         int32_t *cut_pos, uint32_t *cut_bkt, int cut_stride, int cut_iter) {
    const int defer_mode = defer_mode_in & 0xFF;
    const bool dry = defer_mode == 3;
    const uint32_t attn = dry ? 0x4000u : 0x8000u;
    const int cut_budget = (defer_mode_in >> 16) & 0xFF;
    const bool dbg = (defer_mode_in & 0x100) != 0;
    extern __shared__ __attribute__((aligned(16))) uint8_t smem[];
    uint2 *rows = (uint2 *)smem;
    uint32_t *tab = (uint32_t *)(smem + kSegBatch * kSlots * 8);
    uint32_t *out_base = tab + 1024;
    uint16_t *out_slot = (uint16_t *)(out_base + kSegBatch);
    uint32_t *row_meta = (uint32_t *)(out_slot + kSegBatch);
    uint2 *gmap = (uint2 *)(row_meta + kSegBatch);
    __shared__ int g_slot[kSegBatch / kSegGroup], g_kf[kSegBatch / kSegGroup], g_ks[kSegBatch / kSegGroup], g_fast[kSegBatch / kSegGroup];
    __shared__ uint32_t g_base[kSegBatch / kSegGroup];
    __shared__ int sh_kf, sh_ks;
    __shared__ int sh_seg, sh_slot, sh_scan, sh_kfired, sh_kslot;
    __shared__ int sh_defer, sh_nexp, sh_ncut_any, sh_cutidx, sh_poison, sh_cut_e, sh_nc, sh_diff;
    __shared__ int row_cs[kSegBatch];
    __shared__ int b_seg0, b_nrow, b_groups;
    __shared__ uint32_t sh_total;
    const StreamDesc s = sd[blockIdx.x];
    StreamState &ss = st[blockIdx.x];
#ifdef ZS_FV_PROF
    const long long k4_t0 = wall_clock64();
#endif
    load_crc_tab(tab, crc_tab_g);
    if (threadIdx.x == 0)
        sh_seg = ss.r_seg, sh_slot = ss.r_slot, sh_total = ss.r_total, sh_kfired = ss.r_kfired, sh_kslot = ss.r_kslot, sh_scan = ss.r_scan,
        ss.r_scan = dry ? ss.r_scan : 0, b_seg0 = 0, b_nrow = 0, b_groups = 0, sh_defer = 0, sh_nexp = 0, sh_ncut_any = 0, sh_cutidx = ss.r_cutidx, sh_poison = 0,
        sh_cut_e = -1, sh_nc = 0, sh_diff = 0x7FFFFFFF;
    __syncthreads();
    if (dry && ss.deferred != 1) return;
    if (ss.spec_ok) return;
    if (s.resume && threadIdx.x == 0 && sh_seg == 0 && sh_slot == 0 && sh_total == 0) sh_slot = s.start_slot, sh_total = s.start_syms;
    __syncthreads();
    if (s.body_end < 0) {
        if (threadIdx.x == 0) ss.tail_p = 0, ss.tail_kind = kR, ss.tail_pend = 0, ss.k_done = 0, ss.preins = -1, ss.body_syms = 0;
        return;
    }
    uint16_t *lk = link + s.pos_off;
    uint2 *a = mm + s.pos_off;
    GlobalAcc acc{as_global(s.in), a, tab, strategy, hash_variant, lk};
    const int nseg = s.nsegs < seg_limit ? s.nsegs : seg_limit, nch = s.nchunks;
    const int64_t mm_end = (int64_t)s.body_end < (int64_t)mm_limit ? (int64_t)s.body_end : (int64_t)mm_limit;
    __shared__ int rp_to, rp_nlist, rp_list[24];
    __shared__ unsigned int rp_mark[24];
    auto repair = [&](int64_t e, int64_t from, int64_t to_all, bool scan_only) {
        RepairArgs ra{&s, a, lk, tab, (uint8_t *)rows, stale, seg_stale, chunk_far, nch, lv, hash_variant};
        const int rc = repair_cut<1024, 32>(ra, e, from, to_all, scan_only, &rp_to, rp_list, &rp_nlist, rp_mark);
        if (rc != 2) return rc;
        if (supmap != nullptr && rp_nlist <= 24) {
            uint32_t *c_fk = (uint32_t *)rows, *c_fk4 = c_fk + kChunk + 1, *c_tbl = c_fk4 + kChunk + 1;
            const int nl = rp_nlist;
            for (int k = 0; k < nl; k++) {
                const int cc = rp_list[k];
                __syncthreads();
                chunkmap_compute<1024>(s, cc, mm, link, maps, lv, strategy, hash_variant, c_fk, c_fk4, c_tbl, tab, nullptr, nullptr);
                __syncthreads();
                if (threadIdx.x == 0) stale[s.chunk_off + cc] = 0;
            }
        }
        __syncthreads();
        if (threadIdx.x == 0) b_nrow = 0;
        return rc;
    };
    const bool can_sup = supmap != nullptr && seg_limit >= s.nsegs && (int64_t)mm_limit >= (int64_t)s.body_end && s.nsegs > kSupSegs;
    __shared__ int fs_try, fs_n;
    __shared__ unsigned long long fp_kf;
    {
        const int nc = ss.r_ncut;
        int keep = 0;
        for (int i = 0; i < nc; i++) {
            const int64_t e = ss.r_cut_e[i], from = ss.r_cut_done[i];
            int64_t full = e + kMaxDist;
            if (full > s.body_end) full = s.body_end;
            const int64_t to = full < mm_end ? full : mm_end;
            if (to > from) repair(e, from, to, false);
            __syncthreads();
            if (threadIdx.x == 0 && to < full) ss.r_cut_e[keep] = (int32_t)e, ss.r_cut_done[keep] = (int32_t)to;
            if (to < full) keep++;
        }
        __threadfence_block();
        __syncthreads();
        if (threadIdx.x == 0) ss.r_ncut = keep;
    }
    struct NthEqualEv {
        int want, seen;
        int64_t pos;
        __device__ void operator()(int64_t p, bool eq) {
            if (!eq) return;
            if (seen == want) pos = p;
            seen++;
        }
    };
    auto process_cuts = [&]() {
        const ChunkCtx cx = chunk_ctx(s, s.seg_c0[sh_seg]);
        for (;;) {
            if (threadIdx.x == 0) {
                if (cx.m == 1) {
                    sh_cut_e = sh_cutidx == 0 ? (int)(sh_slot <= 256 ? cx.cs + sh_slot : cx.cs) : -1;
                } else {
                    NthEqualEv ne{sh_cutidx, 0, -1};
                    NullSink nsk;
                    int kind, ns;
                    int64_t pp;
                    uint32_t fl;
                    chunk_special_prefix(acc, nsk, cx, sh_slot, lv, strategy, kind, pp, ns, fl, ne);
                    sh_cut_e = (int)ne.pos;
                    if (fl & kMapPoisonBit) sh_poison = 1;
                }
            }
            __syncthreads();
            const int64_t e = sh_cut_e;
            if (dbg && threadIdx.x == 0) printf("zs resolve: segment %d slot %d cut #%d at %ld (defer mode %d)\n", sh_seg, sh_slot, sh_cutidx, (long)e, defer_mode);
            if (e < 0 || sh_poison) break;
            if (threadIdx.x == 0) lk[e] = 0, sh_cutidx++;
            __threadfence_block();
            __syncthreads();
            int64_t full = e + kMaxDist;
            if (full > s.body_end) full = s.body_end;
            const int64_t to = full < mm_end ? full : mm_end;
            {
                const int rc = repair(e, e, to, false);
                if (threadIdx.x == 0 && to < full) {
                    const int k = ss.r_ncut < 8 ? ss.r_ncut++ : 7;
                    ss.r_cut_e[k] = (int32_t)e, ss.r_cut_done[k] = (int32_t)to;
                }
                if (defer_mode == 1 && threadIdx.x == 0 && ((rc == 2 && ++sh_nexp > (cut_budget < kDeferBudget ? cut_budget : kDeferBudget)) || ++sh_ncut_any > cut_budget)) sh_defer = 1;
            }
            __threadfence_block();
            __syncthreads();
            if (sh_defer) break;
        }
        __syncthreads();
        if (threadIdx.x == 0 && !sh_defer) sh_cutidx = 0;
        __syncthreads();
    };
    int32_t *cl_out = cut_pos ? cut_pos + (size_t)(cut_iter & 1) * (size_t)cut_stride + s.cut_off : nullptr;
    const int cl_cap = s.nsegs > 0 ? s.seg_cl[s.nsegs] - s.seg_cl[0] + s.nsegs : 0;
    if (dry) {
        for (int i = threadIdx.x; i < cl_cap; i += blockDim.x) cl_out[i] = -1;
        __threadfence_block();
        __syncthreads();
    }
    auto collect_cuts = [&](int seg, int slot, int skip, int cs_single) {
        const int k0 = s.seg_cl[seg];
        int32_t *dst = cl_out + (k0 - s.seg_cl[0]) + seg;
        if (cs_single < 0) {
            const int64_t cs = cs_single & 0x7FFFFFFF;
            if (skip == 0) dst[0] = (int32_t)(slot <= 256 ? cs + slot : cs);
            return;
        }
        const ChunkCtx cx = chunk_ctx(s, seg_first(s, seg));
        if (cx.m == 1) {
            if (skip == 0) dst[0] = (int32_t)(slot <= 256 ? cx.cs + slot : cx.cs);
            return;
        }
        struct SlotEqualEv {
            int32_t *dst;
            int skip, seen, n, cap;
            __device__ void operator()(int64_t p, bool eq) {
                if (eq && seen++ >= skip && n < cap) dst[n++] = (int32_t)p;
            }
        } ae{dst, skip, 0, 0, cx.m};
        NullSink nsk;
        int kind, ns;
        int64_t pp;
        uint32_t fl;
        chunk_special_prefix(acc, nsk, cx, slot, lv, strategy, kind, pp, ns, fl, ae);
        if (fl & kMapPoisonBit) sh_poison = 1;
    };
    if (sh_scan && sh_seg < nseg) {
        if (dry) {
            if (threadIdx.x == 0) collect_cuts(sh_seg, sh_slot, sh_cutidx, 0);
            __syncthreads();
        } else {
            process_cuts();
        }
    }
#ifdef ZS_FV_PROF
    long long kp[6] = {0, 0, 0, 0, 0, 0}, kt = wall_clock64();
    const long long k4_t1 = kt;
    int kiter = 0;
#define K4_PF(i) { const long long now_ = wall_clock64(); kp[i] += now_ - kt; kt = now_; }
#else
#define K4_PF(i)
#endif
    constexpr int kPendRows = 512;
    __shared__ uint16_t pf_slot[kPendRows];
    __shared__ uint32_t pf_base[kPendRows];
    __shared__ int pf_g0, pf_n;
    if (threadIdx.x == 0) pf_g0 = 0, pf_n = 0, fp_kf = 0;
    __syncthreads();
    auto flush_fill = [&]() {
        const int n_p = pf_n, g_p = pf_g0;
        if (n_p == 0) return;
        for (int t = threadIdx.x; t < n_p; t += blockDim.x) {
            const int g = g_p + t;
            int cur = pf_slot[t];
            uint32_t total = pf_base[t];
            unsigned long long kf = 0;
            uint32_t metas[kSupSegs];
#pragma unroll
            for (int r = 0; r < kSupSegs; r++) {
                const int seg = g * kSupSegs + r;
                metas[r] = seg < s.nsegs ? seg_row_meta(s, seg, seg_stale) : 0u;
            }
#pragma unroll
            for (int r = 0; r < kSupSegs; r++) {
                const int seg = g * kSupSegs + r;
                if (seg < s.nsegs) {
                    const uint2 v = segmap[((int64_t)s.seg_off + seg) * kSlots + cur];
                    const uint32_t m = metas[r];
                    if ((m & 1u) && (uint32_t)(cur <= 256 ? cur : 0) <= (m >> 2)) {
                        kf = ((unsigned long long)(seg + 1) << 16) | (unsigned)cur;
                        if (dry && (v.x & kMapEqualBit) && strategy != kHuffmanOnly) collect_cuts(seg, cur, 0, 0);
                    }
                    seg_entry[s.seg_off + seg] = (uint16_t)cur;
                    seg_symbase[s.seg_off + seg] = total;
                    cur = (int)(v.x & 0x1FF);
                    total += v.y;
                }
            }
            if (kf) atomicMax(&fp_kf, kf);
        }
        __syncthreads();
        if (threadIdx.x == 0) {
            if (fp_kf) sh_kfired = (int)(fp_kf >> 16) - 1, sh_kslot = (int)(fp_kf & 0xFFFF);
            pf_n = 0, fp_kf = 0;
        }
        __syncthreads();
    };
    for (;;) {
        const bool k4_done = sh_seg >= nseg || sh_defer || sh_poison;
#ifdef ZS_FV_PROF
        kiter++;
        kt = wall_clock64();
#endif
        bool went_fast = false;
        if (!k4_done && can_sup && (sh_seg % kSupSegs) == 0 && !sh_scan) {
            const int g0 = sh_seg / kSupSegs, nsup = (s.nsegs + kSupSegs - 1) / kSupSegs;
            int nrow = nsup - g0;
            if (nrow > kSegBatch) nrow = kSegBatch;
            if (threadIdx.x == 0) fs_try = !(supmap[((int64_t)s.sup_off + g0) * kSlots + sh_slot].x & attn), fs_n = 0;
            __syncthreads();
            K4_PF(0);
            if (fs_try) {
                const uint4 *src = (const uint4 *)(supmap + ((int64_t)s.sup_off + g0) * kSlots);
                for (int i = threadIdx.x; i < nrow * kSlots / 2; i += blockDim.x) ((uint4 *)rows)[i] = src[i];
                if ((int)threadIdx.x < nrow) {
                    uint32_t st_any = 0;
                    for (int r = 0; r < kSupSegs; r++) {
                        const int seg = (g0 + (int)threadIdx.x) * kSupSegs + r;
                        if (seg < s.nsegs) st_any |= seg_stale[s.seg_off + seg];
                    }
                    row_meta[threadIdx.x] = st_any;
                }
                __syncthreads();
                K4_PF(1);
                if (threadIdx.x == 0) {
                    int slot = sh_slot, i = 0;
                    uint32_t total = sh_total;
                    if (pf_n == 0) pf_g0 = g0;
                    for (; i < nrow; i++) {
                        const uint2 e = rows[i * kSlots + slot];
                        if ((e.x & attn) || row_meta[i]) break;
                        pf_slot[pf_n + i] = (uint16_t)slot, pf_base[pf_n + i] = total;
                        slot = (int)(e.x & 0x1FF), total += e.y;
                    }
// ... 153 lines not shown
                out_base[i] = total;
                cur = (int)(v.x & 0x1FF);
                total += v.y;
            }
            g_kf[g] = kf, g_ks[g] = ks;
        }
        __syncthreads();
        if (threadIdx.x == 0) {
            int kf = sh_kf, ks = sh_ks;
            for (int g = 0; g < kSegBatch / kSegGroup; g++)
                if (g_fast[g] && g_kf[g] > kf) kf = g_kf[g], ks = g_ks[g];
            if (kf >= 0) sh_kfired = kf, sh_kslot = ks;
        }
        __syncthreads();
        for (int i = threadIdx.x; i < sh_seg - seg0; i += blockDim.x) {
            seg_entry[s.seg_off + seg0 + i] = out_slot[i];
            seg_symbase[s.seg_off + seg0 + i] = out_base[i];
        }
        K4_PF(3);
        if (sh_poison) break;
        if (!sh_scan) {
            if (sh_seg >= nseg) break;
            continue;
        }
        process_cuts();
        __syncthreads();
        K4_PF(4);
        if (sh_defer || sh_poison) break;
    }
#ifdef ZS_FV_PROF
    const long long k4_t2 = wall_clock64();
    if (threadIdx.x == 0 && blockIdx.x == 0 && kiter > 4)
        printf("K4PROF iterations=%d ticks: stage+meta=%lld compose=%lld walk=%lld fill+flush=%lld repair=%lld\n", kiter, kp[0], kp[1], kp[2], kp[3], kp[4]);
#endif
    if (threadIdx.x == 0 && !dry) ss.r_seg = sh_seg, ss.r_slot = sh_slot, ss.r_total = sh_total, ss.r_kfired = sh_kfired, ss.r_kslot = sh_kslot, ss.r_cutidx = sh_cutidx;
    if (dry && !sh_poison) {
        const int cur = cut_iter & 1;
        const int32_t *a = cut_pos + (size_t)cur * (size_t)cut_stride + s.cut_off, *b = cut_pos + (size_t)(cur ^ 1) * (size_t)cut_stride + s.cut_off;
        uint32_t *cbw = cut_bkt + (size_t)cur * (size_t)cut_stride + s.cut_off;
        __threadfence_block();
        __syncthreads();
        for (int i = threadIdx.x; i < cl_cap; i += blockDim.x) {
            const int32_t e = a[i];
            if (e >= 0) cbw[i] = acc.bucket(e);
            if (e != b[i]) atomicMin(&sh_diff, i);
        }
        __syncthreads();
        if (threadIdx.x == 0) {
            const int di = sh_diff < cl_cap ? sh_diff : cl_cap;
            int64_t dp = 0x7FFFFFFF;
            if (di < cl_cap) {
                if (a[di] >= 0) dp = a[di];
                if (b[di] >= 0 && b[di] < dp) dp = b[di];
            }
            ss.nc[cur] = cl_cap, ss.cuts_same = di >= cl_cap ? 1 : 0, ss.cut_diff_idx = di, ss.cut_diff_pos = (int32_t)dp;
        }
    }
    if (sh_poison) {
        if (threadIdx.x == 0) ss.poison = 1, ss.deferred = 3;
        return;
    }
    if (sh_defer) {
        if (threadIdx.x == 0) ss.deferred = sh_defer, ss.r_scan = 1;
        return;
    }
    if (sh_seg < s.nsegs) return;
    if (threadIdx.x == 0) {
        int slot = sh_slot;
        int64_t ce = (int64_t)s.body_end + 1;
        int kind = slot <= 256 ? kR : slot - 256;
        int64_t p = slot <= 256 ? ce + slot : ce;
        ss.tail_p = (int32_t)p;
        ss.tail_kind = kind;
        ss.tail_pend = kind == kXK ? acc.mK(p - 1) : kind == kXK4 ? acc.mK4(p - 1) : 0;
        ss.k_done = sh_kfired;
        struct LastEv {
            int64_t pos;
            __device__ void operator()(int64_t q, bool) { pos = q; }
        } lev{-1};
        if (s.nsegs > 0) {
            NullSink nsk;
            int k2, n2;
            int64_t p2;
            uint32_t f2;
            chunk_special_prefix(acc, nsk, chunk_ctx(s, s.seg_c0[sh_kfired]), sh_kslot, lv, strategy, k2, p2, n2, f2, lev);
        }
        ss.preins = lev.pos >= 0 ? (int32_t)lev.pos + 1 : -1;
        ss.body_syms = sh_total;
#ifdef ZS_FV_PROF
        const long long k4_t3 = wall_clock64();
        if (blockIdx.x == 0) printf("K4PROF ticks: prologue=%lld loop=%lld epilogue=%lld segs=%d; fast stretches: try=%lld stage=%lld walk=%lld fill=%lld\n", k4_t1 - k4_t0, k4_t2 - k4_t1, k4_t3 - k4_t2, s.nsegs, kp[0], kp[1], kp[2], kp[5]);
#endif
    }
}

constexpr int kRepairLds = ((kMaxDist + 16 + 273 + 15) & ~15) + 2 * (kMaxDist + 32) + 64;
__global__ __launch_bounds__(256) void zs_cut_restore_kernel(const StreamDesc *sd, const StreamState *st, uint2 *mm, const uint2 *bak, uint8_t *stale,
                                                             uint8_t *seg_stale, uint16_t *chunk_far, const uint16_t *far_bak, int n_streams) {
    for (int si = (int)blockIdx.y; si < n_streams; si += (int)gridDim.y) {
        const StreamDesc s = sd[si];
        const StreamState &ss = st[si];
        if (ss.deferred != 1 || ss.cuts_same) continue;
        const int64_t from = (int64_t)ss.cut_diff_pos + 1, to = s.body_end;
        for (int64_t p = from + (int64_t)blockIdx.x * 256 + threadIdx.x; p <= to; p += (int64_t)gridDim.x * 256) {
            const uint2 want = bak[s.pos_off + p], have = mm[s.pos_off + p];
            if (want.x == have.x && want.y == have.y) continue;
            mm[s.pos_off + p] = want;
            const int cp = chunk_of(s, p);
            stale[s.chunk_off + cp] = 1, seg_stale[s.seg_off + seg_of(s, cp)] = 1;
            chunk_far[s.chunk_off + cp] = far_bak[s.chunk_off + cp];
            if (p + 1 == (int64_t)s.cstart[cp + 1] && cp + 1 < s.nchunks) stale[s.chunk_off + cp + 1] = 1, seg_stale[s.seg_off + seg_of(s, cp + 1)] = 1;
        }
    }
}
template <int NT, int U>
__global__ __launch_bounds__(NT) void zs_cuts_repair_kernel(const StreamDesc *sd, const StreamState *st, uint16_t *link, uint2 *mm, uint8_t *stale,
                                                             uint8_t *seg_stale, const uint16_t *chunk_far, const uint32_t *crc_tab_g, LevelCfg lv,
                                                             int hash_variant, const int32_t *cut_pos, const uint32_t *cut_bkt, int cut_stride, int cut_iter,
                                                             int n_streams) {
    extern __shared__ __attribute__((aligned(16))) uint8_t smem[];
    __shared__ uint32_t tab[1024];
    __shared__ int sh_to;
    load_crc_tab(tab, crc_tab_g);
    __syncthreads();
    for (int si = (int)blockIdx.z; si < n_streams; si += (int)gridDim.z) {
        const StreamDesc s = sd[si];
        const StreamState &ss = st[si];
        if (ss.deferred != 1 || ss.cuts_same) continue;
        const int cur = cut_iter & 1, nc = ss.nc[cur];
        const int32_t *cl = cut_pos + (size_t)cur * (size_t)cut_stride + s.cut_off;
        const uint32_t *cb = cut_bkt + (size_t)cur * (size_t)cut_stride + s.cut_off;
        const int64_t dp = ss.cut_diff_pos;
        for (int j = (int)blockIdx.y; j < nc; j += (int)gridDim.y) {
            const int64_t e = cl[j];
            if (e < 0) continue;
            int64_t full = e + kMaxDist;
            if (full > s.body_end) full = s.body_end;
            const int64_t from = e > dp ? e : dp;
            if (from >= full) continue;
            RepairArgs ra{&s, mm + s.pos_off, link + s.pos_off, tab, smem, stale, seg_stale, chunk_far, s.nchunks, lv, hash_variant, cl, cb, j, nc};
            repair_cut<NT, U>(ra, e, from, full, false, &sh_to, nullptr, nullptr, nullptr, (int)blockIdx.x, (int)gridDim.x);
            __syncthreads();
        }
    }
}
__global__ __launch_bounds__(256) void zs_cuts_apply_kernel(const StreamDesc *sd, StreamState *st, uint16_t *link, const int32_t *cut_pos, int cut_stride,
                                                            int cut_iter) {
    const StreamDesc s = sd[blockIdx.x];
    StreamState &ss = st[blockIdx.x];
    if (ss.deferred != 1 || !ss.cuts_same) return;
    const int cur = cut_iter & 1, nc = ss.nc[cur];
    const int32_t *cl = cut_pos + (size_t)cur * (size_t)cut_stride + s.cut_off;
    for (int i = threadIdx.x; i < nc; i += 256)
        if (cl[i] >= 0) link[s.pos_off + cl[i]] = 0;
    __syncthreads();
    if (threadIdx.x == 0) ss.deferred = 0, ss.r_scan = 0;
}

__global__ __launch_bounds__(64) void zs_expand_kernel(const StreamDesc *sd, const StreamState *st, const uint2 *work, int nwork, const uint2 *mm,
                                                       const uint16_t *link, const uint32_t *maps, const uint16_t *seg_entry,
                                                       const uint32_t *seg_symbase, const uint8_t *stale, uint16_t *entry,
                                                       uint32_t *symbase, const uint32_t *crc_tab_g, LevelCfg lv, int strategy,
                                                       int hash_variant) {
    int i = blockIdx.x * 64 + threadIdx.x;
    if (i >= nwork) return;
    uint2 w = work[i];
    if (st[w.x].deferred || st[w.x].spec_ok) return;
    const StreamDesc s = sd[w.x];
    const int seg = (int)w.y;
    GlobalAcc acc{as_global(s.in), mm + s.pos_off, crc_tab_g, strategy, hash_variant, link + s.pos_off};
    int slot = seg_entry[s.seg_off + seg];
    uint32_t total = seg_symbase[s.seg_off + seg];
    const int c0 = seg_first(s, seg), c1 = seg_first(s, seg + 1);
    for (int c = c0; c < c1; c++) {
        entry[s.chunk_off + c] = (uint16_t)slot;
        symbase[s.chunk_off + c] = total;
        int ex, cnt;
        if (stale[s.chunk_off + c]) {
            NullSink ns;
            walk_chunk(acc, ns, chunk_ctx(s, c), slot, lv, strategy, ex, cnt);
        } else {
            uint32_t m = maps[((int64_t)s.chunk_off + c) * kSlots + slot];
            ex = map_exit(m), cnt = map_count(m);
        }
        slot = ex;
        total += (uint32_t)cnt;
    }
}

struct GlobalSymSink {
    uint32_t *out;
    uint32_t base;
    int32_t *blk_end, *blk_top;
    uint32_t next_cut;
    __device__ GlobalSymSink(uint32_t *o, uint32_t b, int32_t *be, int32_t *bt)
        : out(o), base(b), blk_end(be), blk_top(bt), next_cut((b / kBlockSyms + 1) * kBlockSyms - 1 - b) {}
    __device__ void operator()(int i, uint32_t sym, int64_t end, int64_t top) {
        out[i] = sym;
        if ((uint32_t)i == next_cut) {
            const uint32_t bi = (base + (uint32_t)i) / kBlockSyms;
            blk_end[bi] = (int32_t)end;
            blk_top[bi] = (int32_t)top;
            next_cut += kBlockSyms;
        }
    }
};
constexpr uint32_t kK5Idle = 0xFFFFFFFEu, kK5Done = 0xFFFFFFFFu;
template <int R>
__device__ __forceinline__ uint32_t k5_slot(uint32_t line) {
    if constexpr (R == 4) return line & 3u;
    else return line - (uint32_t)R * ((line * (uint32_t)(512 / R + 1)) >> 9);
}
static_assert(512 / 3 + 1 == 171, "k5_slot<3>: floor(L * 171 / 512) = floor(L / 3) for L < 512");
typedef __attribute__((address_space(3))) uint32_t *lds_u32p;
__device__ __forceinline__ void k5_publish(lds_u32p slot, uint32_t v) {
    asm volatile("ds_write_b32 %0, %1" ::"v"((uint32_t)(uintptr_t)slot), "v"(v) : "memory");
}
__device__ __forceinline__ uint32_t k5_peek(lds_u32p slot) { return *(volatile __attribute__((address_space(3))) uint32_t *)slot; }
__device__ __forceinline__ uint64_t k5_peek64(uint32_t addr) { return *(volatile __attribute__((address_space(3))) uint64_t *)(uintptr_t)addr; }
template <int kK5Ring, int MODE>
__global__ __launch_bounds__(kK5Threads) void zs_emit_syms_lane_kernel(const StreamDesc *sd, const StreamState *st, const uint2 *work, int nwork, const uint2 *mm,
                                                               const uint16_t *link, const uint16_t *entry, const uint32_t *symbase, uint32_t *syms,
                                                               int32_t *blk_end, int32_t *blk_top, const uint32_t *crc_tab_g,
                                                               LevelCfg lv, int strategy, int hash_variant, int ahead, K5Spec sp) {
    __shared__ uint4 sh_ring_[kK5Ring * 64 * 128 / 16];
    __shared__ uint32_t sh_line_[64], sh_last_[64], sh_base_[64], sh_filled_[64];
    const int lane = (int)(threadIdx.x & 63);
    const lds_u32p sh_line = (lds_u32p)sh_line_ + lane, sh_last = (lds_u32p)sh_last_ + lane, sh_base = (lds_u32p)sh_base_ + lane,
                   sh_filled = (lds_u32p)sh_filled_ + lane;
    if (threadIdx.x < 64) {
        k5_publish(sh_line, kK5Idle);
        k5_publish(sh_filled, (uint32_t)-1);
    }
    __syncthreads();
    if (threadIdx.x >= 64) {
        if (ahead <= 0) return;
        constexpr int kG = 8 / kK5Feeders;
        const int piece = lane & 7, wsub = lane >> 3;
        const int g0 = __builtin_amdgcn_readfirstlane((int)(threadIdx.x >> 6) - 1) * kG;
        int32_t nf[kG];
#pragma unroll
        for (int g = 0; g < kG; g++) nf[g] = 0;
        for (;;) {
            uint32_t c[kG], la[kG], ba[kG];
#pragma unroll
            for (int g = 0; g < kG; g++) {
                c[g] = k5_peek((lds_u32p)sh_line_ + 8 * (g0 + g) + wsub);
                la[g] = k5_peek((lds_u32p)sh_last_ + 8 * (g0 + g) + wsub);
                ba[g] = k5_peek((lds_u32p)sh_base_ + 8 * (g0 + g) + wsub);
            }
            bool busy = false, did = false;
            int32_t pub[kG];
#pragma unroll
            for (int g = 0; g < kG; g++) {
                busy |= c[g] != kK5Done;
                pub[g] = -1;
                if (c[g] < kK5Idle) {
                    const int32_t cl = (int32_t)c[g], lo = nf[g] > cl ? nf[g] : cl;
                    int32_t hi = cl + kK5Ring - 1;
                    hi = hi > (int32_t)la[g] ? (int32_t)la[g] : hi;
                    const int lo_slot = (int)k5_slot<kK5Ring>((uint32_t)lo);
#pragma unroll
                    for (int r = 0; r < kK5Ring; r++) {
                        const int32_t L = lo + (r >= lo_slot ? r - lo_slot : r + kK5Ring - lo_slot);
                        if (L <= hi) {
                            const uint2 *src = mm + (((size_t)ba[g] + (size_t)L) << 4) + 2 * piece;
                            __builtin_amdgcn_global_load_lds((const __attribute__((address_space(1))) void *)(uintptr_t)src,
                                                             (__attribute__((address_space(3))) void *)((__attribute__((address_space(3))) uint8_t *)sh_ring_ + r * 8192 + (g0 + g) * 1024),
                                                             16, 0, 0);
                            did = true;
                        }
                    }
                    if (lo <= hi) {
                        nf[g] = hi + 1;
                        pub[g] = hi;
                    }
                }
            }
            if (__ballot(busy) == 0) break;
            if (__ballot(did) != 0) {
                asm volatile("s_waitcnt vmcnt(0)" ::: "memory");
#pragma unroll
                for (int g = 0; g < kG; g++)
                    if (pub[g] >= 0 && piece == 0) k5_publish((lds_u32p)sh_filled_ + 8 * (g0 + g) + wsub, (uint32_t)pub[g]);
            } else {
                __builtin_amdgcn_s_sleep(2);
            }
        }
        asm volatile("s_waitcnt vmcnt(0)" ::: "memory");
        return;
    }
    struct Done {
        lds_u32p slot;
        __device__ ~Done() { k5_publish(slot, kK5Done); }
    } done{sh_line};
    const int i = blockIdx.x * 64 + lane;
    int si, c;
    if constexpr (MODE == 0) {
        if (i >= nwork) return;
        const uint2 w = work[i];
        if (st[w.x].deferred || st[w.x].spec_ok) return;
        si = (int)w.x, c = (int)w.y;
    } else {
        si = (int)blockIdx.y, c = i;
        if (!sd[si].spec || c >= sd[si].spec_n) return;
        if (spec_periodic(sd[si], st[si])) return;
    }
// ... 180 lines not shown
#pragma unroll
        for (int e = 0; e < kPer; e++) {
            r[e] = sh_rec[kPer * t + e];
            const int c = T + kPer * t + e;
            if (c < n) {
                bad |= (r[e] & kSpecBail) != 0;
                wrong += spec_guess(r[e]) != (c > 0 ? spec_exit(prev) : 0);
                sum += (uint32_t)spec_count(r[e]);
            }
            prev = r[e];
        }
        uint32_t inc = sum;
#pragma unroll
        for (int d = 1; d < 64; d <<= 1) {
            const uint32_t v = __shfl_up(inc, d, 64);
            if ((t & 63) >= d) inc += v;
        }
        if ((t & 63) == 63) sh_wave[t >> 6] = inc;
        __syncthreads();
        uint32_t at = sh_carry + inc - sum;
        for (int w = 0; w < (t >> 6); w++) at += sh_wave[w];
#pragma unroll
        for (int e = 0; e < kPer; e++) {
            sh_rec[kPer * t + e] = at;
            at += T + kPer * t + e < n ? (uint32_t)spec_count(r[e]) : 0u;
        }
        __syncthreads();
#pragma unroll
        for (int k = 0; k < kPer; k++)
            if (T + t + 1024 * k < n) base[T + t + 1024 * k] = sh_rec[t + 1024 * k];
        if (t == 1023) sh_carry = at, sh_prev = r[kPer - 1];
    }
    if (bad) atomicOr(&sh_bad, 1);
    if (wrong) atomicAdd(&sh_wrong, wrong);
    __syncthreads();
    const bool ok = !sh_bad && sh_wrong == 0;
    if (!ok) {
        if (t == 0) flags[si] = sh_bad ? 3 : 4, ss.spec_ok = 0, ss.spec_wrong = sh_wrong;
        return;
    }
    if (t != 0) return;
    GlobalAcc acc{as_global(s.in), mm + s.pos_off, crc_tab_g, strategy, hash_variant, link + s.pos_off};
    const int slot = spec_exit(rec[n - 1]);
    const int64_t ce = (int64_t)s.body_end + 1;
    const int kind = slot <= 256 ? (int)kR : slot - 256;
    const int64_t p = slot <= 256 ? ce + slot : ce;
    ss.tail_p = (int32_t)p;
    ss.tail_kind = kind;
    ss.tail_pend = kind == kXK ? acc.mK(p - 1) : kind == kXK4 ? acc.mK4(p - 1) : 0;
    int k_done = 0;
    int64_t preins = -1;
    for (int k = s.nsegs - 1; k >= 1; k--) {
        const int j = (int)(((int64_t)kWindowSize + (int64_t)kWSize * (k - 1)) >> sp.len_bits);
        if (j >= n) continue;
        const ChunkCtx cx = spec_chunk_ctx(s, j, sp.len_bits);
        const int g = spec_guess(rec[j]);
        if ((g <= 256 ? cx.cs + g : cx.cs) > (int64_t)s.body_end) continue;
        struct LastEv {
            int64_t pos;
            __device__ void operator()(int64_t q, bool) { pos = q; }
        } lev{-1};
        NullSink nsk;
        int k2, n2;
        int64_t p2;
        uint32_t f2;
        chunk_special_prefix(acc, nsk, cx, g, lv, strategy, k2, p2, n2, f2, lev);
        k_done = k;
        preins = lev.pos >= 0 ? lev.pos + 1 : -1;
        break;
    }
    ss.k_done = k_done;
    ss.preins = (int32_t)preins;
    ss.body_syms = sh_carry;
    ss.deferred = 0;
    ss.spec_ok = 1, ss.spec_wrong = 0;
    flags[si] = 1;
}

__global__ __launch_bounds__(256) void zs_spec_compact_kernel(const StreamDesc *sd, const StreamState *st, K5Spec sp, uint32_t *syms, int32_t *blk_end,
                                                             int32_t *blk_top) {
    const int si = (int)blockIdx.y, c = (int)blockIdx.x * 4 + (int)(threadIdx.x >> 6), lane = (int)(threadIdx.x & 63);
    const StreamDesc &s = sd[si];
    if (!s.spec || c >= s.spec_n || !st[si].spec_ok) return;
    const uint32_t r = sp.rec[s.spec_off + c], base = sp.base[s.spec_off + c];
    const int count = spec_count(r), cut = spec_cut_index(base, count);
    const uint32_t *slab = sp.syms + (size_t)(s.spec_off + c) * (size_t)sp.stride;
    uint32_t *out = syms + s.sym_off + base;
    int before = 0;
    for (int i = lane; i < count; i += 64) {
        const uint32_t v = slab[i];
        out[i] = v;
        before += i < cut ? sym_len(v) : 0;
    }
    if (cut < 0) return;
#pragma unroll
    for (int d = 32; d >= 1; d >>= 1) before += __shfl_xor(before, d, 64);
    if (lane != 0) return;
    const ChunkCtx cx = spec_chunk_ctx(s, c, sp.len_bits);
    const int64_t start = spec_first_start(cx.cs, spec_guess(r)) + before;
    const bool odd = cx.m != 0 && slab[sp.stride - 1] == (uint32_t)cut;
    const uint32_t bi = (base + (uint32_t)cut) / kBlockSyms;
    blk_end[s.blk_off + bi] = (int32_t)spec_sym_end(start, slab[cut]);
    blk_top[s.blk_off + bi] = (int32_t)spec_sym_top(start, odd);
}

__global__ __launch_bounds__(256) void zs_body_blocks_kernel(const StreamDesc *sd, const StreamState *st, const int32_t *blk_end,
                                                             const int32_t *blk_top, BlockRec *blocks, uint32_t *syms) {
    const StreamDesc s = sd[blockIdx.x];
    if (s.fast_runs > 0 || st[blockIdx.x].deferred) return;
    if (s.resume)
        for (uint32_t i = threadIdx.x; i < s.start_syms; i += blockDim.x) syms[s.sym_off + i] = s.persist->syms[i];
    const int nb_body = (int)(st[blockIdx.x].body_syms / kBlockSyms);
    BlockRec *blk = blocks + s.blk_off;
    for (int i = threadIdx.x; i < nb_body; i += blockDim.x) {
        int64_t start = i ? blk_end[s.blk_off + i - 1] : (s.resume ? s.start_block : 0);
        int64_t end = blk_end[s.blk_off + i];
        BlockRec r;
        r.start = start;
        r.sym_start = (int64_t)i * kBlockSyms;
        r.stored_len = (int32_t)(end - start);
        r.nsyms = kBlockSyms;
        r.can_store = start >= s.base0 + (int64_t)kWSize * (s.rle_end >= 0 ? rle_refills_fired_at(blk_top[s.blk_off + i], s.kl)
                                                                            : refills_fired_at(blk_top[s.blk_off + i] - s.base0, s.kl));
        r.eof = 0;
        blk[i] = r;
    }
    if (s.wr_blk && s.wr_end && s.n_wr > 1) {
        const StreamState &ss = st[blockIdx.x];
        const int64_t read_to = s.nsegs > 0 ? (int64_t)s.seg_after[ss.k_done] : 0;
        for (int w = 1 + (int)threadIdx.x; w < s.n_wr; w += blockDim.x) {
            if (s.wr_end[w - 1] >= read_to) continue;
            const int64_t bound = s.wr_end[w - 1] - (kMinLookahead - 1);
            int lo = 0, hi = nb_body;
            while (lo < hi) {
                const int mid = (lo + hi) >> 1;
                if ((int64_t)blk_top[s.blk_off + mid] < bound) lo = mid + 1;
                else hi = mid;
            }
            s.wr_blk[w] = lo;
        }
    }
    if (threadIdx.x == 0 && nb_body > 0 && s.final_run) {
        BlockRec r = blk[nb_body];
        if (r.can_store < 0) {
            const int64_t base = (int64_t)(-r.can_store - 1) * kWSize, start = blk_end[s.blk_off + nb_body - 1];
            r.start = start;
            r.stored_len -= (int32_t)start;
            r.can_store = start >= base;
            blk[nb_body] = r;
        }
    }
}

__global__ __launch_bounds__(1024) void zs_tail_kernel(const StreamDesc *sd, StreamState *st, const uint16_t *link, uint32_t *syms,
                                                     const int32_t *blk_end, const int32_t *blk_top, BlockRec *blocks,
                                                     uint8_t *scratch, const uint32_t *crc_tab_g, LevelCfg lv, int strategy,
                                                     int hash_variant, int level) {
#ifdef ZS_FV_PROF
    const long long tk_start = wall_clock64();
    long long pf_restore[4] = {0, 0, 0, 0};
#endif
    const StreamDesc s = sd[blockIdx.x];
    if (s.fast_runs > 0) return;
    StreamState &ss = st[blockIdx.x];
    if (ss.deferred) return;
    const int tid = threadIdx.x, nth = blockDim.x;
    if (s.plan_nblk > 0) {
        for (int i = tid; i < s.plan_nblk; i += nth) blocks[s.blk_off + i] = s.plan_blk[i];
        if (tid == 0) ss.nsyms = 0, ss.nblocks = s.plan_nblk;
        return;
    }
    uint8_t *sc = scratch + (int64_t)blockIdx.x * kScratchBytes;
    BlockRec *blk = blocks + s.blk_off;
    const uint32_t body_syms = ss.body_syms;
    const int nb_body = (int)(body_syms / kBlockSyms);
    extern __shared__ __attribute__((aligned(16))) uint8_t smem[];
    LitEngine e;
    le_defaults(e);
    e.window = smem;
    e.head = (uint16_t *)(sc + kScratchHead);
    e.prev = (uint16_t *)(smem + kScratchHead);
    uint32_t *head32 = (uint32_t *)(sc + kScratchHead32);
    uint32_t *tabl = (uint32_t *)(smem + kScratchHead + 2 * kWSize);
    load_crc_tab(tabl, crc_tab_g);
    e.crc_tab = tabl;
    e.data = s.in;
    e.n = s.n;
    e.wr_end = s.wr_end;
    e.n_wr = s.n_wr;
    e.cur_wr = 0;
    e.wr_flush = s.wr_flush;
    e.wr_blk = s.wr_blk;
    e.lv = lv;
    e.strategy = strategy;
    e.hash_variant = hash_variant;
    e.syms = syms + s.sym_off;
    e.nsyms = body_syms;
    e.blocks = blk;
    e.nblocks = nb_body;
    e.block_start_abs = 0;
    e.defer_start = nb_body > 0;
    if ((!s.final_run || s.resume) && nb_body > 0) {
        e.block_start_abs = blk_end[s.blk_off + nb_body - 1];
        e.defer_start = 0;
    }
    if (s.resume && nb_body == 0) e.block_start_abs = s.start_block;
    e.block_sym_start = (int64_t)nb_body * kBlockSyms;
    e.block_syms = level == 0 ? (kLitBufsize / 2) - 1 : kBlockSyms;
    const uint16_t *lk = link + s.pos_off;
    const int64_t p = ss.tail_p;
    e.final_run = s.final_run;
    LitPersist *ps = s.persist;
    bool use_rec = false, no_head = false;
    if (s.cont) {
        for (int i = tid * 16; i < kWindowSize + 512; i += nth * 16) *(uint4 *)(smem + i) = *(const uint4 *)(ps->window + i);
        for (int i = tid * 8; i < kWSize; i += nth * 8) *(uint4 *)(e.prev + i) = *(const uint4 *)(ps->prev + i);
        for (int i = tid; i < ps->pending_syms; i += nth) e.syms[i] = ps->syms[i];
        e.head = ps->head;
        e.data = s.in - s.abs_off;
        e.n = s.abs_off + (int64_t)s.n;
        e.base = ps->base, e.avail_end = ps->avail_end, e.block_start_abs = ps->block_start_abs;
        e.strstart = ps->strstart, e.lookahead = ps->lookahead, e.match_length = ps->match_length, e.match_start = ps->match_start;
        e.match_available = ps->match_available, e.prev_length = ps->prev_length, e.prev_match = ps->prev_match;
        e.nsyms = ps->pending_syms, e.block_sym_start = 0, e.nblocks = 0, e.defer_start = 0;
        e.stop_abs = s.stop_abs;
        __syncthreads();
    } else {
        const bool have_seg = s.nsegs > 0;
#ifdef ZS_FV_PROF
        long long tk0 = wall_clock64(), tk1 = 0, tk2 = 0, tk3 = 0;
#endif
        int64_t base_in = have_seg ? s.seg_base[ss.k_done] : 0;
        const int64_t after_in = have_seg ? s.seg_after[ss.k_done] : 0;
        const bool preslid = lv.func == 2 && strategy != kRle && strategy != kHuffmanOnly && s.fv_end < 0 &&
                             le_tail_preslide(e, p, base_in, after_in, ss.preins);
        if (preslid) base_in += kWSize;
        le_restore(e, p, base_in, after_in, ss.tail_kind, ss.tail_pend, lk, ss.preins, tid, nth, preslid);
        const int64_t img_base = preslid ? e.base - kWSize : e.base;
        const bool same_window = s.resume && ps && ps->base - s.persist_off == img_base;
        if (same_window) {
            const int64_t valid = e.avail_end - img_base;
            for (int w = tid; w < kWindowSize + 512; w += nth) {
                const int wi = preslid && w < kWSize ? w + kWSize : w;
                if (wi >= valid) e.window[w] = ps->window[wi];
            }
        }
        use_rec = lv.func == 2 && strategy != kRle && strategy != kHuffmanOnly && s.fv_end < 0 && le_tail_reads_done(e) && ss.preins < p &&
                  le_tail_record_end(e) > p && le_tail_record_end(e) - p <= kTailRecMax;
        no_head = use_rec && s.final_run && !e.wr_end && le_no_head_ok(e) && !(s.resume && p - (kWSize - 1) < s.start_pos);
        if (!no_head) {
            const int64_t shift = s.resume && ps ? e.base - (ps->base - s.persist_off) : 0;
            for (int i = tid; i < kHashSize; i += nth) {
                int64_t hv = s.resume && ps ? (int64_t)ps->head[i] : 0;
                hv = hv != 0 && hv - shift > 0 ? hv - shift : 0;
                head32[i] = hv ? (uint32_t)hv + 1u : 0u;
            }
        }
        __syncthreads();
#ifdef ZS_FV_PROF
        tk1 = wall_clock64();
#endif
        if (e.avail_end > 0) {
            int64_t lo = p - (kWSize - 1);
            if (lo < e.base) lo = e.base;
            if (lo < 0) lo = 0;
            int64_t hi = p;
            if (hi > (int64_t)s.n - 5) hi = (int64_t)s.n - 5;
            const uint32_t *gb = s.ins_bits;
            auto insf = [gb](int64_t c) { return ((gb[c >> 5] >> (c & 31)) & 1u) != 0; };
            for (int64_t q = lo + tid; q < hi; q += nth) {
                if (s.fv_end >= 0) {
                    if (!insf(q)) continue;
                    le_restore_prev_ins(e, q, lk, insf);
                } else {
                    le_restore_prev(e, q, lk);
                }
                if (!no_head && q >= s.start_pos) atomicMax(&head32[le_bucket(e, q)], (uint32_t)(q - e.base) + 1u);
            }
            __syncthreads();
#ifdef ZS_FV_PROF
            tk2 = wall_clock64();
#endif
            if (!no_head)
                for (int i = tid; i < kHashSize; i += nth) e.head[i] = (uint16_t)(head32[i] ? head32[i] - 1 : 0);
        }
        __syncthreads();
#ifdef ZS_FV_PROF
        tk3 = wall_clock64();
        pf_restore[0] = tk0 - tk_start, pf_restore[1] = tk1 - tk0, pf_restore[2] = tk2 - tk1, pf_restore[3] = tk3 - tk2;
#endif
    }
    __shared__ uint32_t pre_tab[2 * kTailRecMax];
    __shared__ uint32_t sh_tail_head[3];
    {
        const int64_t hi = le_tail_record_end(e);
        if (use_rec) {
            for (int64_t q = p + tid; q < (no_head ? e.n - 5 : hi); q += nth) le_restore_prev(e, q, lk);
            if (tid < 3) sh_tail_head[tid] = 0;
            __syncthreads();
            if (no_head) {
                const uint32_t hb0 = le_tail_head_bucket(e, 0), hb1 = le_tail_head_bucket(e, 1), hb2 = le_tail_head_bucket(e, 2);
                int64_t lo = p - (kWSize - 1);
                if (lo < e.base) lo = e.base;
                if (lo < 1) lo = 1;
                for (int64_t q = lo + tid; q < e.n - 3; q += nth) {
                    const uint32_t h = le_bucket(e, q);
                    if (h == hb0 && q < e.n - 5) atomicMax(&sh_tail_head[0], (uint32_t)(q - e.base));
                    if (h == hb1 && q < e.n - 4) atomicMax(&sh_tail_head[1], (uint32_t)(q - e.base));
                    if (h == hb2 && q < e.n - 3) atomicMax(&sh_tail_head[2], (uint32_t)(q - e.base));
                }
            }
            __syncthreads();
            e.no_head = no_head ? 1 : 0;
            e.tail_head[0] = (int)sh_tail_head[0], e.tail_head[1] = (int)sh_tail_head[1], e.tail_head[2] = (int)sh_tail_head[2];
            for (int64_t q = p + tid; q < hi; q += nth) {
                pre_tab[2 * (q - p)] = le_tail_record(e, (int)(q - e.base), (int)(e.n - q), lv.chain);
                pre_tab[2 * (q - p) + 1] = le_tail_record(e, (int)(q - e.base), (int)(e.n - q), lv.chain >> 2);
            }
            e.pre_rec = pre_tab, e.pre_lo = p, e.pre_hi = hi;
            __syncthreads();
        }
    }
#ifdef ZS_FV_PROF
    const long long tk_pre = wall_clock64() - tk_start;
#endif
    if (tid >= 64) return;
#ifdef ZS_FV_PROF
    long long te0 = wall_clock64();
#endif
    if (!s.cont && e.avail_end > 0) {
        if (s.fv_end >= 0) {
            const uint32_t *gb = s.ins_bits;
            le_restore_finish(e, p, lk, ss.preins, [gb](int64_t c) { return ((gb[c >> 5] >> (c & 31)) & 1u) != 0; });
        } else {
            le_restore_finish(e, p, lk, ss.preins);
        }
    }
    __syncthreads();
    le_run(e, level, tid, 64);
#ifdef ZS_FV_PROF
    if (tid == 0 && blockIdx.x == 0)
        printf("TAILPROF setup=%lld window+clear=%lld prev+head=%lld convert=%lld; before the engine (with the searches ahead) %lld; kernel so far %lld; engine ticks=%lld syms=%lld: refill=%lld insert=%lld match=%lld tally=%lld flush=%lld\n", pf_restore[0], pf_restore[1], pf_restore[2], pf_restore[3], tk_pre, wall_clock64() - tk_start, wall_clock64() - te0,
               (long long)(e.nsyms - body_syms), e.pf[0], e.pf[1], e.pf[2], e.pf[3], e.pf[4]);
#endif
    if (tid == 0 && e.stopped && e.wr_blk)
        for (int w = e.cur_wr + 1; w < e.n_wr; w++) e.wr_blk[w] = 0x7FFFFFFF;
    if (tid == 0) {
        ss.nsyms = (uint32_t)e.nsyms;
        ss.nblocks = e.nblocks;
    }
    if (!ps || s.final_run) return;
    __syncthreads();
    for (int i = tid * 16; i < kWindowSize + 512; i += 64 * 16) *(uint4 *)(ps->window + i) = *(const uint4 *)(smem + i);
    for (int i = tid * 8; i < kWSize; i += 64 * 8) *(uint4 *)(ps->prev + i) = *(const uint4 *)(e.prev + i);
    if (e.head != ps->head)
        for (int i = tid * 8; i < kHashSize; i += 64 * 8) *(uint4 *)(ps->head + i) = *(const uint4 *)(e.head + i);
    const int pending = (int)(e.nsyms - e.block_sym_start);
    for (int i = tid; i < pending; i += 64) ps->syms[i] = e.syms[e.block_sym_start + i];
    if (tid == 0) {
        const int64_t po = s.resume ? s.persist_off : 0;
        ps->base = e.base + po, ps->avail_end = e.avail_end + po, ps->block_start_abs = e.block_start_abs + po;
        ps->strstart = e.strstart, ps->lookahead = e.lookahead, ps->match_length = e.match_length, ps->match_start = e.match_start;
        ps->match_available = e.match_available, ps->prev_length = e.prev_length, ps->prev_match = e.prev_match;
        ps->pending_syms = pending;
        ps->stopped = e.stopped, ps->good_prev = e.prev_length >= lv.good ? 1 : 0;
    }
}

constexpr int kTailLds = (int)kScratchHead + 2 * kWSize + 4096;
constexpr int kFastRunLds = kTailLds + kHeadCacheLds;
static_assert(kFastRunLds + 1024 <= 160 * 1024, "a run's LDS");

__global__ __launch_bounds__(1024) void zs_fast_run_kernel(const StreamDesc *sd, const uint2 *work, const uint16_t *link,
                                                           uint32_t *run_syms, uint32_t *run_bits, uint8_t *run_scratch,
                                                           FastRunOut *outs, const uint32_t *crc_tab_g, LevelCfg lv, int strategy,
                                                           int hash_variant) {
    extern __shared__ __attribute__((aligned(16))) uint8_t smem[];
    __shared__ BlockRec dummy_blk[2];
    const uint2 w = work[blockIdx.x];
    const StreamDesc s = sd[w.x];
    const int j = (int)w.y;
    const int64_t run = (int64_t)s.run_off + j;
    const int tid = threadIdx.x, nth = blockDim.x;
    const int64_t cj = (int64_t)j * s.run_chunk;
    const bool last = j + 1 == s.fast_runs;
    int64_t x = cj - kFastWarm;
    if (x < 0) x = 0;
    uint8_t *sc = run_scratch + run * kFastRunScratch;
    uint32_t *bits = run_bits + run * kFastRunBitWords;
    for (int64_t i = tid; i < kFastRunBitWords * (s.fast_runs == 1 ? (int64_t)s.run_slots : 1); i += nth) bits[i] = 0;
    LitEngine e;
    le_defaults(e);
    e.window = smem;
    e.prev = (uint16_t *)(smem + kScratchHead);
    e.head = (uint16_t *)sc;
    uint32_t *head32 = (uint32_t *)(sc + 2 * kHashSize);
    uint32_t *tabl = (uint32_t *)(smem + kScratchHead + 2 * kWSize);
    load_crc_tab(tabl, crc_tab_g);
    e.crc_tab = tabl;
    e.hc_val = (uint16_t *)(smem + kTailLds), e.hc_nib = (uint32_t *)(smem + kTailLds + 2 * kHeadCache), e.hc_pres = e.hc_nib + kHeadCache / 8;
    e.hc_claim = e.hc_pres + kHashSize / 32;
    for (int i = tid; i < kHeadCache / 32; i += nth) e.hc_claim[i] = 0;
    e.data = s.in;
    e.n = s.n;
    e.lv = lv;
    e.strategy = strategy;
    e.hash_variant = hash_variant;
    e.syms = run_syms + run * kFastRunSyms;
    e.blocks = dummy_blk;
    e.no_blocks = 1;
    e.stop_abs = last ? -1 : cj + s.run_chunk;
    e.mark_abs = cj;
    e.ins_bits = bits;
    e.ins_base = x;
    e.ev_log = outs[run].ev;
    const uint16_t *lk = link + s.pos_off;
    const int k_done = x == 0 ? 0 : refills_fired_at(x, s.kl);
    le_restore(e, x, (int64_t)kWSize * k_done, read_end_before(k_done + 1), kR, 0, lk, -1, tid, nth);
    for (int i = tid; i < kHashSize; i += nth) head32[i] = 0;
    __syncthreads();
    if (e.avail_end > 0) {
        int64_t lo = x - (kWSize - 1);
        if (lo < e.base) lo = e.base;
        if (lo < 0) lo = 0;
        for (int64_t q = lo + tid; q < x; q += nth) {
            le_restore_prev(e, q, lk);
            atomicMax(&head32[le_bucket(e, q)], (uint32_t)(q - e.base) + 1u);
        }
        __syncthreads();
        for (int i = tid; i < kHashSize; i += nth) e.head[i] = (uint16_t)(head32[i] ? head32[i] - 1 : 0);
    }
    __syncthreads();
    for (int w = tid; w < kHashSize / 32; w += nth) {
        uint32_t bits_w = 0;
        for (int k = 0; k < 32; k++) bits_w |= (uint32_t)(e.head[32 * w + k] != 0) << k;
        e.hc_pres[w] = bits_w;
    }
    for (int w = tid; w < kHeadCache / 8; w += nth) {
        uint32_t nw = 0;
        for (int k = 0; k < 8; k++) {
            const int i = 8 * w + k;
            int best_v = 0, best_t = 0;
            for (int t = 0; t < 4; t++) {
                const int v = e.head[t * kHeadCache + i];
                if (v > best_v) best_v = v, best_t = t;
            }
            e.hc_val[i] = (uint16_t)best_v;
            if (best_v) nw |= (8u | (uint32_t)best_t) << (4 * k);
        }
        e.hc_nib[w] = nw;
    }
    __syncthreads();
#ifdef ZS_FV_PROF
    const long long tk_pre = wall_clock64();
#endif
    if (tid >= 64) return;
    le_run_fast_hot(e, tid);
    le_flush_ins(e);
#ifdef ZS_FV_PROF
    if (tid == 0 && (blockIdx.x == 3 || blockIdx.x == 100))
        printf("FASTRUN %d: engine ticks(100MHz)=%lld syms=%lld: refill+checks=%lld insert=%lld match=%lld tally+advance=%lld flush=%lld\n", (int)blockIdx.x,
               wall_clock64() - tk_pre, (long long)e.nsyms, e.pf[0], e.pf[1], e.pf[2], e.pf[3], e.pf[4]);
#endif
    if (tid == 0) {
        FastRunOut &o = outs[run];
        o.mark_pos = e.mark_pos, o.mark_nsyms = e.mark_nsyms;
        o.end_pos = (e.stop_abs >= 0 && e.lookahead > 0) ? e.base + e.strstart : (int64_t)s.n;
        if (e.stop_abs >= 0 && e.base + e.strstart < e.stop_abs) o.end_pos = -1;
        o.nsyms = e.nsyms;
        o.final_base = e.base;
        o.sym_dst = 0;
        o.ok = 1, o.n_ev = e.n_ev;
        o.n_match = e.n_match;
        if (j == 0) o.mark_pos = 0, o.mark_nsyms = 0;
    }
}

__global__ __launch_bounds__(256) void zs_fast_probe_kernel(const StreamDesc *sd, const uint16_t *link, int32_t *not_periodic) {
    __shared__ int same;
    const StreamDesc s = sd[blockIdx.x];
    if (s.fast_runs <= 0) {
        if (threadIdx.x == 0) not_periodic[blockIdx.x] = 0;
        return;
    }
    if (threadIdx.x == 0) same = 0;
    __syncthreads();
    const uint16_t *lk = link + s.pos_off;
    const int64_t span = (int64_t)s.n - 8 - kWSize;
    int mine = 0;
    for (int w = 0; w < 64; w++) {
        const int64_t p = kWSize + span * w / 64 + threadIdx.x;
        if (p + 8 < s.n) mine += lk[p] != 0 && lk[p] == lk[p - 1];
    }
    atomicAdd(&same, mine);
    __syncthreads();
    if (threadIdx.x == 0) not_periodic[blockIdx.x] = s.n >= kFastMinInput ? same * 4 < 64 * 256 * 3 : same * 16 < 64 * 256 * 15;
}

__global__ __launch_bounds__(256) void zs_fast_verify_kernel(const StreamDesc *sd, const uint2 *work, const uint32_t *run_bits,
                                                             FastRunOut *outs, int32_t *stream_fail) {
    __shared__ int bad;
    const uint2 w = work[blockIdx.x];
    const StreamDesc s = sd[w.x];
    const int j = (int)w.y;
    if (j == 0) return;
    const int64_t run = (int64_t)s.run_off + j;
    const FastRunOut a = outs[run - 1], b = outs[run];
    if (threadIdx.x == 0) bad = (b.mark_pos < 0 || b.mark_pos != a.end_pos);
    __syncthreads();
    if (!bad) {
        const int64_t xa = (j - 1) * (int64_t)s.run_chunk - kFastWarm < 0 ? 0 : (j - 1) * (int64_t)s.run_chunk - kFastWarm;
        const int64_t xb = (int64_t)j * s.run_chunk - kFastWarm < 0 ? 0 : (int64_t)j * s.run_chunk - kFastWarm;
        const uint32_t *ba = run_bits + (run - 1) * kFastRunBitWords, *bb = run_bits + run * kFastRunBitWords;
        int64_t lo = b.mark_pos - kWSize;
        if (lo < 0) lo = 0;
        int mism = 0;
        for (int64_t p = lo + threadIdx.x; p < b.mark_pos; p += 256) {
            const int64_t ia = p - xa, ib = p - xb;
            const uint32_t va = (ba[ia >> 5] >> (ia & 31)) & 1u;
            const uint32_t vb = ib >= 0 ? (bb[ib >> 5] >> (ib & 31)) & 1u : va;
            const uint32_t want = ib >= 0 ? vb : 1u;
            mism |= (va != want);
// ... 970 lines not shown
```

### zlibstream_amd/csrc/zs_lit_engine.h

```cpp
#pragma once
#include "zs_core.h"

#if defined(__HIP_DEVICE_COMPILE__)
#define ZS_WAVE_SYNC() __syncthreads()
#else
#define ZS_WAVE_SYNC() ((void)0)
#endif

namespace zs {

struct BlockRec {
    int64_t start;
    int64_t sym_start;
    int32_t stored_len;
    int32_t nsyms;
    int32_t can_store;
    int32_t eof;
};

struct LitEngine {
#ifdef ZS_FV_PROF
    long long pf[5] = {0, 0, 0, 0, 0};
#endif
    uint8_t *window;
// ... 713 lines not shown
                    pl[str & kWMask] = hit ? (uint16_t)cv : (uint16_t)0;
                    syms[nsyms + lane] = lit;
                }
                for (int i0 = ins_off + strstart, left = m; left > 0;) {
                    const int wi = i0 >> 5, take = 32 - (i0 & 31) < left ? 32 - (i0 & 31) : left;
                    const uint32_t mask = (take >= 32 ? 0xFFFFFFFFu : ((1u << take) - 1u)) << (i0 & 31);
                    if (wi == ins_idx) {
                        ins_word |= mask;
                    } else if (wi > ins_idx) {
                        if (ins_idx >= 0) (void)__hip_atomic_fetch_or(bits + ins_idx, ins_word, __ATOMIC_RELAXED, __HIP_MEMORY_SCOPE_AGENT);
                        ins_idx = wi, ins_word = mask;
                    } else {
                        (void)__hip_atomic_fetch_or(bits + wi, mask, __ATOMIC_RELAXED, __HIP_MEMORY_SCOPE_AGENT);
                    }
                    i0 += take, left -= take;
                }
                strstart += m, lookahead -= m, nsyms += m;
                HOT_PF(3);
                continue;
            }
            lit_streak = 0;
        }
        int hash_head = 0;
        n_match++;
        if (lookahead >= kMinMatch) hash_head = insert(strstart);
        HOT_PF(1);
        if (hash_head != 0 && strstart - hash_head <= kMaxDist && search) {
            int chain_length = chain_eff, best_len = best0, cur_match = hash_head;
            const int limit = strstart > kMaxDist ? strstart - kMaxDist : 0;
            const int nice = nice_cfg > lookahead ? lookahead : nice_cfg;
            const int off = lane < 33 ? lane * 8 : 0;
            const uint64_t sx = le_load64(win + strstart + off);
            do {
                if (cur_match >= strstart) break;
                const int next = pl[cur_match & kWMask];
                const uint64_t x = le_load64(win + cur_match + off) ^ sx;
                const uint64_t differ = __ballot(x != 0 && lane < 33);
                int len = kMaxMatch;
                if (differ) {
                    const int fl = (int)__builtin_ctzll(differ);
                    const uint32_t lo = (uint32_t)__builtin_amdgcn_readlane((int)(uint32_t)x, fl), hi = (uint32_t)__builtin_amdgcn_readlane((int)(uint32_t)(x >> 32), fl);
                    len = fl * 8 + (int)(__builtin_ctzll((uint64_t)lo | ((uint64_t)hi << 32)) >> 3);
                    len = len < kMaxMatch ? len : kMaxMatch;
                }
                if (len > best_len) {
                    match_start = cur_match;
                    best_len = len;
                    if (len >= nice) break;
                }
                cur_match = next;
            } while (cur_match > limit && --chain_length != 0);
            match_length = best_len < lookahead ? best_len : lookahead;
        }
        HOT_PF(2);
        if (match_length >= kMinMatch) {
            if (lane == 0) syms[nsyms] = ((uint32_t)(strstart - match_start) << 16) | (uint32_t)(match_length - kMinMatch);
            nsyms++;
            lookahead -= match_length;
            if (match_length <= lazy && lookahead >= kMinMatch) {
                match_length--;
                do {
                    strstart++;
                    (void)insert(strstart);
                } while (--match_length != 0);
                strstart++;
            } else {
                strstart += match_length;
                match_length = 0;
            }
            lit_streak = 0;
        } else {
            if (lane == 0) syms[nsyms] = (uint32_t)wl[strstart];
            nsyms++;
            lookahead--;
            strstart++;
            lit_streak = (hash_head == 0 || strstart - 1 - hash_head > kMaxDist) ? lit_streak + 1 : 0;
        }
        HOT_PF(3);
    }
}
#endif

ZS_HD_NOINLINE inline void le_run_stored(LitEngine &e, int lane, int nlanes) {
    const int max_block_size = 32768 - 5;
    for (;;) {
        if (e.lookahead <= 1) {
            int dummy = 0;
            le_refill(e, lane, nlanes, dummy, 1);
            if (e.suspended) return;
            if (e.lookahead == 0) {
                if (!le_write_flushes(e)) break;
                le_end_write(e, lane, nlanes);
                continue;
            }
        }
        e.strstart += e.lookahead;
        e.lookahead = 0;
        const int block_start = (int)(e.block_start_abs - e.base);
        const int max_start = block_start + max_block_size;
        if (e.strstart == 0 || e.strstart >= max_start) {
            e.lookahead = e.strstart - max_start;
            e.strstart = max_start;
            le_flush_block(e, false, lane);
        }
        if (e.strstart - (int)(e.block_start_abs - e.base) >= kMaxDist) le_flush_block(e, false, lane);
    }
    le_flush_block(e, true, lane);
}

ZS_HD_NOINLINE inline void le_run_rle(LitEngine &e, int lane, int nlanes) {
    for (;;) {
        if (e.lookahead <= kMaxMatch) {
            int dummy = 0;
            le_refill(e, lane, nlanes, dummy, kMaxMatch + 1);
            if (e.suspended) return;
        }
        if (e.lookahead == 0) {
            if (!le_write_flushes(e)) break;
            le_end_write(e, lane, nlanes);
            continue;
        }
        e.match_length = 0;
        if (e.lookahead >= kMinMatch && e.strstart > 0) {
            const uint8_t *w = e.window + e.strstart;
            const uint8_t prev = w[-1];
            if (prev == w[0] && prev == w[1] && prev == w[2]) {
                const int len = le_match_len_wave(w, w - 1);
                e.match_length = len < e.lookahead ? len : e.lookahead;
            }
        }
        bool bflush;
        if (e.match_length >= kMinMatch) {
            bflush = le_tally(e, 1, e.match_length - kMinMatch, lane);
            e.lookahead -= e.match_length;
            e.strstart += e.match_length;
            e.match_length = 0;
        } else {
            bflush = le_tally(e, 0, le_wbyte(e, e.strstart), lane);
            e.lookahead--;
            e.strstart++;
        }
        if (bflush) le_flush_block(e, false, lane);
    }
    le_flush_block(e, true, lane);
}

ZS_HD void le_run(LitEngine &e, int level, int lane, int nlanes) {
    if (e.strategy == kRle) le_run_rle(e, lane, nlanes);
    else if (level == 0) le_run_stored(e, lane, nlanes);
    else if (e.lv.func == 1) le_run_fast(e, lane, nlanes);
    else le_run_slow(e, lane, nlanes);
}

ZS_HD_NOINLINE inline void le_restore(LitEngine &e, int64_t p, int64_t base, int64_t avail_end, int kind, uint32_t pend,
                                      const uint16_t *link, int64_t preins, int lane, int nlanes, bool preslid = false) {
    e.base = base;
    e.avail_end = avail_end;
    if (e.avail_end > e.n) e.avail_end = e.n;
    bool started = (p > 0 || base > 0 || kind != kR);
    if (!started) e.avail_end = 0;
    e.cur_wr = 0;
    if (e.wr_end) {
        int lo = 0, hi = e.n_wr - 1;
        while (lo < hi) {
            const int mid = (lo + hi) >> 1;
            if (e.wr_end[mid] < e.avail_end) lo = mid + 1;
            else hi = mid;
        }
        e.cur_wr = lo;
    }
    const int64_t ib = preslid ? e.base - kWSize : e.base;
    const int64_t valid = e.avail_end - ib;
    for (int w = lane; w < kWindowSize + 512; w += nlanes) {
        const int wi = preslid && w < kWSize ? w + kWSize : w;
        uint8_t v = 0;
        if (wi < valid) v = e.data[ib + wi];
        else if (ib >= kWSize && wi < kWindowSize) v = e.data[ib + wi - kWSize];
        e.window[w] = v;
    }
    for (int i = lane; i < kHashSize; i += nlanes) e.head[i] = 0;
    for (int i = lane; i < kWSize; i += nlanes) e.prev[i] = 0;
    e.strstart = (int)(p - e.base);
    e.lookahead = (int)(e.avail_end - p);
    e.match_available = (kind == kR) ? 0 : 1;
    e.match_length = (kind == kXK || kind == kXK4) ? match_len(pend) : kMinMatch - 1;
    e.match_start = (kind == kXK || kind == kXK4) ? (int)((p - 1 - match_dist(pend)) - e.base) : 0;
    e.prev_length = kMinMatch - 1;
    e.prev_match = 0;
}

ZS_HD void le_restore_prev(LitEngine &e, int64_t q, const uint16_t *link) {
    int w = (int)(q - e.base);
    int64_t c = link[q] ? q - (int64_t)link[q] : -1;
    e.prev[w & kWMask] = (uint16_t)(c >= e.base ? c - e.base : 0);
}
template <class Ins>
ZS_HD void le_restore_prev_ins(LitEngine &e, int64_t q, const uint16_t *link, const Ins &ins) {
    int64_t c = q;
    for (;;) {
        const int l = link[c];
        if (!l) {
            c = -1;
            break;
        }
        c -= l;
        if (c < e.base || ins(c)) break;
    }
    e.prev[(int)(q - e.base) & kWMask] = (uint16_t)(c >= e.base ? c - e.base : 0);
}
ZS_HD uint32_t le_bucket(const LitEngine &e, int64_t q) { return le_hash(e, le_load32(e.window + (q - e.base) + 2)); }

struct AllIns {
    ZS_HD bool operator()(int64_t) const { return true; }
};
template <class Ins>
ZS_HD_NOINLINE inline void le_restore_finish(LitEngine &e, int64_t p, const uint16_t *link, int64_t preins, const Ins &ins) {
    int64_t q = e.n - 5;
    if (q < 0) q = 0;
    if (q < e.base) q = e.base;
    for (; q < p && q <= e.n - kMinMatch; q++)
        if (ins(q)) le_insert(e, (int)(q - e.base));
    if (preins >= p && preins >= 1) {
        int w = (int)(preins - e.base);
        uint32_t h1 = le_hash(e, le_load32(e.window + w + 2));
        uint32_t h0 = le_hash(e, le_load32(e.window + w - 1 + 2));
        if (h0 == h1) {
            e.prev[(w - 1) & kWMask] = (uint16_t)w;
        } else {
            int64_t c = preins;
            for (;;) {
                const int l = link[c];
                if (!l) {
                    c = -1;
                    break;
                }
                c -= l;
                if (c < e.base || ins(c)) break;
            }
            e.prev[w & kWMask] = (uint16_t)(c >= e.base ? c - e.base : 0);
            e.head[h1] = (uint16_t)w;
        }
    }
}
ZS_HD_NOINLINE inline void le_restore_finish(LitEngine &e, int64_t p, const uint16_t *link, int64_t preins) {
    le_restore_finish(e, p, link, preins, AllIns());
}

}
```

Baseline: 15120 MB/s.

## Precompute tail window state on aux stream and launch tail kernel early

Adds a tail-prepare kernel that runs on the aux stream right after the links stage. It builds the tail's window, prev chains, head-bucket maxima and match records into a TailPrep buffer, which the tail kernel then adopts instead of rebuilding them. When speculation is in use, the tail kernel and spec compaction are also launched before the host waits on the spec flags, with a second tail launch only if some streams fall back. This aims to take the serial tail stage off the critical path by overlapping it with matching. The cost is an extra kernel, a device buffer and fits/refuse logic that adds risk of mismatch.

Measured after the change: 15180 MB/s (median of 3 runs). Within noise of the previous version (+0.4%).

```diff
diff --git a/zlibstream_amd/csrc/zs_device.h b/zlibstream_amd/csrc/zs_device.h
--- a/zlibstream_amd/csrc/zs_device.h
+++ b/zlibstream_amd/csrc/zs_device.h
@@ -72,6 +72,7 @@
     int32_t rle_end, rle_tile_off;
     int32_t fr_first, fr_n;
     int32_t spec, spec_n, spec_off;
+    int32_t tail_prep;
 };
 
 struct WorkOffsets {
@@ -116,6 +117,7 @@
     int32_t nc[2], cuts_same, cut_diff_idx, cut_diff_pos;
     int32_t poison;
     int32_t spec_run_tiles, spec_ok, spec_wrong;
+    int32_t link_cut, tail_prep;
 };
 constexpr uint32_t kSpecBail = 1u << 30;
 ZS_HD uint32_t spec_pack(int guess, int exit_slot, int count, bool bail) {
diff --git a/zlibstream_amd/csrc/zs_engine.hip b/zlibstream_amd/csrc/zs_engine.hip
--- a/zlibstream_amd/csrc/zs_engine.hip
+++ b/zlibstream_amd/csrc/zs_engine.hip
@@ -40,6 +40,7 @@
     hipStream_t stream = nullptr;
     hipStream_t aux = nullptr;
     hipEvent_t ev_fork = nullptr, ev_join = nullptr, ev_pre0 = nullptr, ev_pre = nullptr;
+    hipEvent_t ev_links = nullptr;
     hipEvent_t ev_spec[4] = {};
     std::string err;
     bool profiling = false;
@@ -49,6 +50,7 @@
     int lit_fallbacks = 0;
     int spec_streams = 0, spec_fallbacks = 0, spec_wrong_chunks = 0;
     int spec_periodic = 0;
+    int tail_prep_used = 0, tail_prep_refused = 0;
     int64_t dbg_blk_off = 0, dbg_chunk_off = 0, dbg_nchunks = 0, dbg_spec_n = 0, dbg_n_spec = 0;
     int64_t lit_engine_bytes = 0;
     std::vector<int64_t> inf_used;
@@ -63,7 +65,7 @@
     uint32_t *crc_tab = nullptr;
     DevBuf sd, st, work, wpre, geo, link, mm, maps, chunk_far, segmap, supmap, seg_entry, seg_symbase, seg_stale, entry, symbase, stale, syms, blk_end, blk_top, blocks, trees, info, pieces, scratch,
         stage_in, stage_out, wr, inf_desc, inf_state, par_ps, par_st, par_work, par_cbits, par_ccnt, par_surv, par_scnt, par_cands, par_tabs, par_toktabs, par_toks, par_ctoks, par_tokstat, par_tails, par_retry, par_fxtab, par_blocks, par_cells,
-        par_windows, par_fail, run_syms, run_bits, run_scratch, run_outs, run_fail, adl_tr, adl_res, plan_blk, ins_bits, mm_bak, cut_pos, cut_bkt, win_groups, win_sg, win_maps, win_entries, persist_bak, resume_flag, rle_tiles, own_in, fr_chunks, fr_meta, fr_planes, fr_prov, fr_base, fr_counters, spec_rec, spec_flags, spec_syms, png_img, png_seg, png_ctr, png_fimg, png_scratch, png_a7img, png_inflated, png_passes, crc_desc, crc_res, png_zs, png_gather, png_ximg, png_raw;
+        par_windows, par_fail, run_syms, run_bits, run_scratch, run_outs, run_fail, adl_tr, adl_res, plan_blk, ins_bits, mm_bak, cut_pos, cut_bkt, win_groups, win_sg, win_maps, win_entries, persist_bak, resume_flag, rle_tiles, own_in, fr_chunks, fr_meta, fr_planes, fr_prov, fr_base, fr_counters, spec_rec, spec_flags, spec_syms, tail_prep, png_img, png_seg, png_ctr, png_fimg, png_scratch, png_a7img, png_inflated, png_passes, crc_desc, crc_res, png_zs, png_gather, png_ximg, png_raw;
     uint32_t *crc32_tab = nullptr;
     hipEvent_t ev_crc[2] = {};
     hipEvent_t ev_expand[2] = {};
@@ -580,6 +582,15 @@
         ZS_HIP(c, hipMemcpyAsync(c->plan_blk.p, pl.plan_blk.data(), sizeof(BlockRec) * pl.plan_blk.size(), hipMemcpyHostToDevice, stream));
         ZS_HIP(c, hipStreamSynchronize(stream));
     }
+    const bool tail_late = ro && (!ro->final_run || ro->resume);
+    const bool tail_serial = !tail_late && n >= 64 && (pl.n_pos / n >= (96 << 10) || getenv("ZS_TAIL_SERIAL")) && !getenv("ZS_TAIL_FORK");
+    int n_tail_prep = 0;
+    if (!tail_late && !tail_serial && n < 64 && lv.func == 2 && strategy != kRle && strategy != kHuffmanOnly && !getenv("ZS_NO_TAIL_PREP"))
+        for (int i = 0; i < n; i++) {
+            StreamDesc &s = pl.sd[(size_t)i];
+            if (!s.wr_end && s.final_run && !s.resume && !s.cont && !s.persist && s.fv_end < 0 && s.plan_nblk == 0 && s.body_end >= 0) s.tail_prep = ++n_tail_prep;
+        }
+    if (n_tail_prep && !ensure(c, c->tail_prep, sizeof(TailPrep) * (size_t)n_tail_prep)) return false;
     const size_t pre_bytes = 4 * (size_t)kWorkLists * (size_t)(n + 1);
     size_t up_bytes = sizeof(StreamDesc) * (size_t)n + pre_bytes + geo_bytes + 16;
     if (!ensure_pinned(c, std::max(up_bytes, sizeof(StreamState) * (size_t)n)) || !ensure(c, c->wpre, pre_bytes + 64)) return false;
@@ -646,6 +657,7 @@
     const StreamDesc *d_sd = dev<StreamDesc>(c->sd);
     StreamState *d_st = dev<StreamState>(c->st);
     const uint2 *d_work = dev<uint2>(c->work);
+    const TailPrep *d_prep = dev<TailPrep>(c->tail_prep);
     const bool prof = c->profiling;
     const int k5_ahead = getenv("ZS_K5_AHEAD") ? atoi(getenv("ZS_K5_AHEAD")) : 1;
     c->dbg_blk_off = pl.sd[0].blk_off, c->dbg_chunk_off = pl.sd[0].chunk_off, c->dbg_nchunks = pl.sd[0].nchunks;
@@ -654,6 +666,7 @@
                      dev<uint32_t>(c->spec_syms), spec_slab_stride(spec_bits)};
     int spec_ok_streams = 0;
     bool need_maps = true, spec_ran = false;
+    bool early_tail = false;
     if (!rounds) c->spec_streams = c->spec_fallbacks = c->spec_wrong_chunks = c->spec_periodic = 0;
     auto mark = [&](int i) {
         if (prof) (void)hipEventRecord(c->ev[i], stream);
@@ -761,6 +774,12 @@
                            dev<uint16_t>(c->link), c->crc_tab, hash_variant, (int)link_span);
     if (ro && ro->resume)
         hipLaunchKernelGGL(zs_import_chains_kernel, dim3(64), dim3(1024), 0, stream, d_sd, 0, dev<uint16_t>(c->link), c->crc_tab, hash_variant, ro->p0);
+    if (n_tail_prep) {
+        ZS_HIP(c, hipEventRecord(c->ev_links, stream));
+        ZS_HIP(c, hipStreamWaitEvent(c->aux, c->ev_links, 0));
+        hipLaunchKernelGGL(zs_tail_prepare_kernel, dim3((unsigned)n), dim3(1024), kTailLds, c->aux, d_sd, dev<uint16_t>(c->link), dev<TailPrep>(c->tail_prep),
+                           c->crc_tab, lv, strategy, hash_variant);
+    }
     if (pl.any_dual) {
         bool periodic = true;
         if (!getenv("ZS_FAST_NO_PROBE")) {
@@ -799,8 +818,21 @@
                            strategy, hash_variant, k5s, dev<int32_t>(c->spec_flags));
         int32_t *hf = (int32_t *)c->pinned;
         ZS_HIP(c, hipMemcpyAsync(hf, c->spec_flags.p, 4 * (size_t)n, hipMemcpyDeviceToHost, stream));
-        ZS_HIP(c, hipStreamSynchronize(stream));
-        if (prof) (void)hipEventRecord(c->ev_spec[1], stream);
+        ZS_HIP(c, hipEventRecord(c->ev_spec[1], stream));
+        early_tail = !tail_late && !tail_serial;
+        if (early_tail) {
+            ZS_HIP(c, hipEventRecord(c->ev_fork, stream));
+            ZS_HIP(c, hipStreamWaitEvent(c->aux, c->ev_fork, 0));
+            hipLaunchKernelGGL(zs_tail_kernel, dim3((unsigned)n), dim3(1024), kTailLds, c->aux, d_sd, d_st, dev<uint16_t>(c->link),
+                               dev<uint32_t>(c->syms), dev<int32_t>(c->blk_end), dev<int32_t>(c->blk_top), dev<BlockRec>(c->blocks),
+                               dev<uint8_t>(c->scratch), c->crc_tab, lv, strategy, hash_variant, level, d_prep, 1);
+            ZS_HIP(c, hipEventRecord(c->ev_join, c->aux));
+            if (prof) (void)hipEventRecord(c->ev_spec[2], stream);
+            hipLaunchKernelGGL(zs_spec_compact_kernel, dim3((unsigned)((pl.max_spec_n + 3) / 4), (unsigned)n), dim3(256), 0, stream, d_sd, d_st, k5s,
+                               dev<uint32_t>(c->syms), dev<int32_t>(c->blk_end), dev<int32_t>(c->blk_top));
+            if (prof) (void)hipEventRecord(c->ev_spec[3], stream);
+        }
+        ZS_HIP(c, hipEventSynchronize(c->ev_spec[1]));
         for (int i = 0; i < n; i++) {
             if (hf[i] == 0) continue;
             c->spec_streams++;
@@ -924,14 +956,12 @@
             hipLaunchKernelGGL(zs_rle_pass_kernel<1>, tg, dim3(256), 0, stream, d_sd, rt, dev<uint32_t>(c->syms), dev<int32_t>(c->blk_end), dev<int32_t>(c->blk_top), s0);
         });
     }
-    const bool tail_late = ro && (!ro->final_run || ro->resume);
-    const bool tail_serial = !tail_late && n >= 64 && (pl.n_pos / n >= (96 << 10) || getenv("ZS_TAIL_SERIAL")) && !getenv("ZS_TAIL_FORK");
-    if (!tail_late && !tail_serial) {
+    if (!tail_late && !tail_serial && !(early_tail && spec_ok_streams == n)) {
         ZS_HIP(c, hipEventRecord(c->ev_fork, stream));
         ZS_HIP(c, hipStreamWaitEvent(c->aux, c->ev_fork, 0));
         hipLaunchKernelGGL(zs_tail_kernel, dim3((unsigned)n), dim3(1024), kTailLds, c->aux, d_sd, d_st, dev<uint16_t>(c->link),
                            dev<uint32_t>(c->syms), dev<int32_t>(c->blk_end), dev<int32_t>(c->blk_top), dev<BlockRec>(c->blocks),
-                           dev<uint8_t>(c->scratch), c->crc_tab, lv, strategy, hash_variant, level);
+                           dev<uint8_t>(c->scratch), c->crc_tab, lv, strategy, hash_variant, level, d_prep, early_tail ? 2 : 0);
         ZS_HIP(c, hipEventRecord(c->ev_join, c->aux));
     }
     if (!pl.w_segs.empty() && need_maps)
@@ -946,7 +976,7 @@
                            d_work + o_chunks, (int)pl.w_chunks.size(), dev<uint2>(c->mm), dev<uint16_t>(c->link), dev<uint16_t>(c->entry),
                            dev<uint32_t>(c->symbase), dev<uint32_t>(c->syms), dev<int32_t>(c->blk_end), dev<int32_t>(c->blk_top),
                            c->crc_tab, lv, strategy, hash_variant, k5_ahead, k5s);
-    if (spec_ok_streams) {
+    if (spec_ok_streams && !early_tail) {
         if (prof) (void)hipEventRecord(c->ev_spec[2], stream);
         hipLaunchKernelGGL(zs_spec_compact_kernel, dim3((unsigned)((pl.max_spec_n + 3) / 4), (unsigned)n), dim3(256), 0, stream, d_sd, d_st, k5s,
                            dev<uint32_t>(c->syms), dev<int32_t>(c->blk_end), dev<int32_t>(c->blk_top));
@@ -956,14 +986,14 @@
     if (tail_serial)
         hipLaunchKernelGGL(zs_tail_kernel, dim3((unsigned)n), dim3(1024), kTailLds, stream, d_sd, d_st, dev<uint16_t>(c->link),
                            dev<uint32_t>(c->syms), dev<int32_t>(c->blk_end), dev<int32_t>(c->blk_top), dev<BlockRec>(c->blocks),
-                           dev<uint8_t>(c->scratch), c->crc_tab, lv, strategy, hash_variant, level);
+                           dev<uint8_t>(c->scratch), c->crc_tab, lv, strategy, hash_variant, level, d_prep, 0);
     else if (!tail_late) ZS_HIP(c, hipStreamWaitEvent(stream, c->ev_join, 0));
     hipLaunchKernelGGL(zs_body_blocks_kernel, dim3((unsigned)n), dim3(256), 0, stream, d_sd, d_st, dev<int32_t>(c->blk_end),
                        dev<int32_t>(c->blk_top), dev<BlockRec>(c->blocks), dev<uint32_t>(c->syms));
     if (tail_late)
         hipLaunchKernelGGL(zs_tail_kernel, dim3((unsigned)n), dim3(1024), kTailLds, stream, d_sd, d_st, dev<uint16_t>(c->link),
                            dev<uint32_t>(c->syms), dev<int32_t>(c->blk_end), dev<int32_t>(c->blk_top), dev<BlockRec>(c->blocks),
-                           dev<uint8_t>(c->scratch), c->crc_tab, lv, strategy, hash_variant, level);
+                           dev<uint8_t>(c->scratch), c->crc_tab, lv, strategy, hash_variant, level, d_prep, 0);
     if (pl.n_runs) {
         if (!getenv("ZS_FAST_NO_PROBE") && force_seq == 0 && !pl.any_dual) {
             hipLaunchKernelGGL(zs_fast_probe_kernel, dim3((unsigned)n), dim3(256), 0, stream, d_sd, dev<uint16_t>(c->link), dev<int32_t>(c->run_fail));
@@ -1042,6 +1072,8 @@
     ZS_HIP(c, hipMemcpyAsync(hst, d_st, sizeof(StreamState) * (size_t)n, hipMemcpyDeviceToHost, stream));
     ht_launched = ht_us();
     ZS_HIP(c, hipStreamSynchronize(stream));
+    c->tail_prep_used = c->tail_prep_refused = 0;
+    for (int i = 0; i < n; i++) c->tail_prep_used += hst[i].tail_prep == 1, c->tail_prep_refused += hst[i].tail_prep == 2;
     if (host_times) fprintf(stderr, "zs: host: plan + uploads %.0f us, all launched at %.0f us, device done at %.0f us\n", ht_plan, ht_launched, ht_us());
     c->last_op = lv.func == 1 ? 2 : 0;
     if (getenv("ZS_DEBUG_CHAIN") && n == 1) {
@@ -1083,10 +1115,10 @@
             float a = 0, b = 0, m = 0;
             (void)hipEventElapsedTime(&a, c->ev[kStChunkMap], c->ev_spec[0]);
             (void)hipEventElapsedTime(&b, c->ev_spec[0], c->ev_spec[1]);
-            (void)hipEventElapsedTime(&m, c->ev_spec[1], c->ev[kStChunkMap + 1]);
+            (void)hipEventElapsedTime(&m, c->ev_spec[early_tail ? 3 : 1], c->ev[kStChunkMap + 1]);
             c->stage_ms[kStSpecWalk] = a, c->stage_ms[kStSpecVerify] = b, c->stage_ms[kStChunkMap] = m;
             float k = 0;
-            if (spec_ok_streams) (void)hipEventElapsedTime(&k, c->ev_spec[2], c->ev_spec[3]);
+            if (spec_ok_streams || early_tail) (void)hipEventElapsedTime(&k, c->ev_spec[2], c->ev_spec[3]);
             c->stage_ms[kStSpecCompact] = k;
         }
     }
@@ -1247,7 +1279,8 @@
         hipEventCreateWithFlags(&c->ev_fork, hipEventDisableTiming) != hipSuccess ||
         hipEventCreateWithFlags(&c->ev_join, hipEventDisableTiming) != hipSuccess ||
         hipEventCreateWithFlags(&c->ev_pre0, hipEventDisableTiming) != hipSuccess ||
-        hipEventCreateWithFlags(&c->ev_pre, hipEventDisableTiming) != hipSuccess) {
+        hipEventCreateWithFlags(&c->ev_pre, hipEventDisableTiming) != hipSuccess ||
+        hipEventCreateWithFlags(&c->ev_links, hipEventDisableTiming) != hipSuccess) {
         zs_ctx_destroy(c);
         return ZS_MEM_ERROR;
     }
@@ -1260,6 +1293,7 @@
         hipFuncSetAttribute((const void *)zs_resolve_kernel, hipFuncAttributeMaxDynamicSharedMemorySize, kResolveLds) != hipSuccess ||
         hipFuncSetAttribute((const void *)zs_links_kernel, hipFuncAttributeMaxDynamicSharedMemorySize, kLkLds) != hipSuccess ||
         hipFuncSetAttribute((const void *)zs_tail_kernel, hipFuncAttributeMaxDynamicSharedMemorySize, kTailLds) != hipSuccess ||
+        hipFuncSetAttribute((const void *)zs_tail_prepare_kernel, hipFuncAttributeMaxDynamicSharedMemorySize, kTailLds) != hipSuccess ||
         hipFuncSetAttribute((const void *)zs_fast_run_kernel, hipFuncAttributeMaxDynamicSharedMemorySize, kFastRunLds) != hipSuccess ||
         hipFuncSetAttribute((const void *)zs_fast_sweep_kernel<1024, kFsTile1, false>, hipFuncAttributeMaxDynamicSharedMemorySize, (fs_lds_bytes<1024, kFsTile1>())) != hipSuccess ||
         hipFuncSetAttribute((const void *)zs_fast_sweep_kernel<1024, kFsTile1, true>, hipFuncAttributeMaxDynamicSharedMemorySize, (fs_lds_bytes<1024, kFsTile1>())) != hipSuccess ||
@@ -1290,7 +1324,7 @@
     DevBuf *bufs[] = {&c->sd, &c->st, &c->work, &c->wpre, &c->geo, &c->link, &c->mm, &c->maps, &c->chunk_far, &c->segmap, &c->supmap, &c->seg_entry, &c->seg_symbase, &c->seg_stale, &c->entry, &c->symbase, &c->stale, &c->syms,
                       &c->blk_end, &c->blk_top, &c->blocks, &c->trees, &c->info, &c->pieces, &c->scratch, &c->stage_in, &c->stage_out, &c->wr, &c->inf_desc, &c->inf_state, &c->par_ps, &c->par_st, &c->par_work, &c->par_cbits, &c->par_ccnt, &c->par_surv, &c->par_scnt,
                       &c->par_cands, &c->par_tabs, &c->par_toktabs, &c->par_toks, &c->par_ctoks, &c->par_tokstat, &c->par_tails, &c->par_retry, &c->par_fxtab, &c->par_blocks, &c->par_cells, &c->par_windows, &c->par_fail, &c->run_syms, &c->run_bits,
-                      &c->run_scratch, &c->run_outs, &c->run_fail, &c->adl_tr, &c->adl_res, &c->plan_blk, &c->ins_bits, &c->mm_bak, &c->cut_pos, &c->cut_bkt, &c->win_groups, &c->win_sg, &c->win_maps, &c->win_entries, &c->persist_bak, &c->resume_flag, &c->rle_tiles, &c->own_in, &c->fr_chunks, &c->fr_meta, &c->fr_planes, &c->fr_prov, &c->fr_base, &c->fr_counters, &c->spec_rec, &c->spec_flags, &c->spec_syms, &c->png_img, &c->png_seg, &c->png_ctr, &c->png_fimg, &c->png_scratch, &c->png_a7img, &c->png_inflated, &c->png_passes, &c->crc_desc, &c->crc_res, &c->png_zs, &c->png_gather, &c->png_ximg, &c->png_raw};
+                      &c->run_scratch, &c->run_outs, &c->run_fail, &c->adl_tr, &c->adl_res, &c->plan_blk, &c->ins_bits, &c->mm_bak, &c->cut_pos, &c->cut_bkt, &c->win_groups, &c->win_sg, &c->win_maps, &c->win_entries, &c->persist_bak, &c->resume_flag, &c->rle_tiles, &c->own_in, &c->fr_chunks, &c->fr_meta, &c->fr_planes, &c->fr_prov, &c->fr_base, &c->fr_counters, &c->spec_rec, &c->spec_flags, &c->spec_syms, &c->tail_prep, &c->png_img, &c->png_seg, &c->png_ctr, &c->png_fimg, &c->png_scratch, &c->png_a7img, &c->png_inflated, &c->png_passes, &c->crc_desc, &c->crc_res, &c->png_zs, &c->png_gather, &c->png_ximg, &c->png_raw};
     for (DevBuf *b : bufs)
         if (b->p) (void)hipFree(b->p);
     if (c->crc_tab) (void)hipFree(c->crc_tab);
@@ -1310,6 +1344,7 @@
     if (c->ev_join) (void)hipEventDestroy(c->ev_join);
     if (c->ev_pre0) (void)hipEventDestroy(c->ev_pre0);
     if (c->ev_pre) (void)hipEventDestroy(c->ev_pre);
+    if (c->ev_links) (void)hipEventDestroy(c->ev_links);
     if (c->aux) (void)hipStreamDestroy(c->aux);
     if (c->stream) (void)hipStreamDestroy(c->stream);
     delete c;
@@ -1336,6 +1371,8 @@
     if (k == "spec_fallbacks") return c->spec_fallbacks;
     if (k == "spec_periodic") return c->spec_periodic;
     if (k == "spec_wrong_chunks") return c->spec_wrong_chunks;
+    if (k == "tail_prep_used") return c->tail_prep_used;
+    if (k == "tail_prep_refused") return c->tail_prep_refused;
     if (k == "inf_lane_streams") return c->inf_lane_streams;
     if (k == "png_segments") return c->png_segments;
     return -1;
diff --git a/zlibstream_amd/csrc/zs_kernels.hip b/zlibstream_amd/csrc/zs_kernels.hip
--- a/zlibstream_amd/csrc/zs_kernels.hip
+++ b/zlibstream_amd/csrc/zs_kernels.hip
@@ -1116,7 +1116,7 @@
             const int64_t e = sh_cut_e;
             if (dbg && threadIdx.x == 0) printf("zs resolve: segment %d slot %d cut #%d at %ld (defer mode %d)\n", sh_seg, sh_slot, sh_cutidx, (long)e, defer_mode);
             if (e < 0 || sh_poison) break;
-            if (threadIdx.x == 0) lk[e] = 0, sh_cutidx++;
+            if (threadIdx.x == 0) lk[e] = 0, ss.link_cut = 1, sh_cutidx++;
             __threadfence_block();
             __syncthreads();
             int64_t full = e + kMaxDist;
@@ -1576,7 +1576,7 @@
     const int cur = cut_iter & 1, nc = ss.nc[cur];
     const int32_t *cl = cut_pos + (size_t)cur * (size_t)cut_stride + s.cut_off;
     for (int i = threadIdx.x; i < nc; i += 256)
-        if (cl[i] >= 0) link[s.pos_off + cl[i]] = 0;
+        if (cl[i] >= 0) link[s.pos_off + cl[i]] = 0, ss.link_cut = 1;
     __syncthreads();
     if (threadIdx.x == 0) ss.deferred = 0, ss.r_scan = 0;
 }
@@ -2063,10 +2063,67 @@
     }
 }
 
+constexpr int kTailLds = (int)kScratchHead + 2 * kWSize + 4096;
+
+__global__ __launch_bounds__(1024) void zs_tail_prepare_kernel(const StreamDesc *sd, const uint16_t *link, TailPrep *prep,
+                                                             const uint32_t *crc_tab_g, LevelCfg lv, int strategy, int hash_variant) {
+    const StreamDesc s = sd[blockIdx.x];
+    if (!s.tail_prep) return;
+    TailPrep &t = prep[s.tail_prep - 1];
+    const int tid = threadIdx.x, nth = blockDim.x;
+    extern __shared__ __attribute__((aligned(16))) uint8_t smem[];
+    __shared__ uint32_t sh_tail_head[3];
+    LitEngine e;
+    le_defaults(e);
+    e.window = smem;
+    e.head = nullptr;
+    e.prev = (uint16_t *)(smem + kScratchHead);
+    uint32_t *tabl = (uint32_t *)(smem + kScratchHead + 2 * kWSize);
+    load_crc_tab(tabl, crc_tab_g);
+    e.crc_tab = tabl;
+    e.data = s.in;
+    e.n = s.n;
+    e.lv = lv;
+    e.strategy = strategy;
+    e.hash_variant = hash_variant;
+    e.syms = nullptr, e.blocks = nullptr;
+    const uint16_t *lk = link + s.pos_off;
+    const int64_t p_lo = (int64_t)s.body_end + 1;
+    int k_done = 0;
+    for (int k = s.nsegs - 1; k >= 1; k--)
+        if (s.cstart[s.seg_c0[k]] <= s.body_end) {
+            k_done = k;
+            break;
+        }
+    const int64_t base_in = s.nsegs > 0 ? s.seg_base[k_done] : 0, after_in = s.nsegs > 0 ? s.seg_after[k_done] : 0;
+    bool preslid = false;
+    if (!le_tail_prep_plan(e, p_lo, base_in, after_in, preslid)) {
+        if (tid == 0) t.valid = 0;
+        return;
+    }
+    le_restore_image(e, tid, nth, preslid, false);
+    __syncthreads();
+    le_restore_prev_range(e, le_tail_prev_lo(e, p_lo), p_lo, lk, tid, nth);
+    if (tid < 3) sh_tail_head[tid] = 0;
+    __syncthreads();
+    le_restore_prev_range(e, p_lo, e.n - 5, lk, tid, nth);
+    le_tail_head_scan(e, p_lo, tid, nth, [&](int k, uint32_t w) { atomicMax(&sh_tail_head[k], w); });
+    __syncthreads();
+    e.no_head = 1;
+    const int64_t hi = le_tail_record_end(e);
+    le_tail_records(e, p_lo, hi, t.pre_tab, tid, nth);
+    for (int i = tid * 16; i < kWindowSize + 512; i += nth * 16) *(uint4 *)(t.window + i) = *(const uint4 *)(smem + i);
+    for (int i = tid * 8; i < kWSize; i += nth * 8) *(uint4 *)(t.prev + i) = *(const uint4 *)(e.prev + i);
+    if (tid == 0) {
+        t.valid = 1, t.preslid = preslid ? 1 : 0, t.p_lo = (int32_t)p_lo, t.hi = (int32_t)hi, t.base = e.base;
+        t.tail_head[0] = (int32_t)sh_tail_head[0], t.tail_head[1] = (int32_t)sh_tail_head[1], t.tail_head[2] = (int32_t)sh_tail_head[2];
+    }
+}
+
 __global__ __launch_bounds__(1024) void zs_tail_kernel(const StreamDesc *sd, StreamState *st, const uint16_t *link, uint32_t *syms,
                                                      const int32_t *blk_end, const int32_t *blk_top, BlockRec *blocks,
                                                      uint8_t *scratch, const uint32_t *crc_tab_g, LevelCfg lv, int strategy,
-                                                     int hash_variant, int level) {
+                                                     int hash_variant, int level, const TailPrep *prep, int only) {
 #ifdef ZS_FV_PROF
     const long long tk_start = wall_clock64();
     long long pf_restore[4] = {0, 0, 0, 0};
@@ -2075,6 +2132,7 @@
     if (s.fast_runs > 0) return;
     StreamState &ss = st[blockIdx.x];
     if (ss.deferred) return;
+    if (only != 0 && (ss.spec_ok != 0) != (only == 1)) return;
     const int tid = threadIdx.x, nth = blockDim.x;
     if (s.plan_nblk > 0) {
         for (int i = tid; i < s.plan_nblk; i += nth) blocks[s.blk_off + i] = s.plan_blk[i];
@@ -2122,7 +2180,9 @@
     const int64_t p = ss.tail_p;
     e.final_run = s.final_run;
     LitPersist *ps = s.persist;
-    bool use_rec = false, no_head = false;
+    bool use_rec = false, no_head = false, took = false;
+    __shared__ uint32_t pre_tab[2 * kTailRecMax];
+    __shared__ uint32_t sh_tail_head[3];
     if (s.cont) {
         for (int i = tid * 16; i < kWindowSize + 512; i += nth * 16) *(uint4 *)(smem + i) = *(const uint4 *)(ps->window + i);
         for (int i = tid * 8; i < kWSize; i += nth * 8) *(uint4 *)(e.prev + i) = *(const uint4 *)(ps->prev + i);
@@ -2146,88 +2206,82 @@
         const bool preslid = lv.func == 2 && strategy != kRle && strategy != kHuffmanOnly && s.fv_end < 0 &&
                              le_tail_preslide(e, p, base_in, after_in, ss.preins);
         if (preslid) base_in += kWSize;
-        le_restore(e, p, base_in, after_in, ss.tail_kind, ss.tail_pend, lk, ss.preins, tid, nth, preslid);
-        const int64_t img_base = preslid ? e.base - kWSize : e.base;
-        const bool same_window = s.resume && ps && ps->base - s.persist_off == img_base;
-        if (same_window) {
-            const int64_t valid = e.avail_end - img_base;
-            for (int w = tid; w < kWindowSize + 512; w += nth) {
-                const int wi = preslid && w < kWSize ? w + kWSize : w;
-                if (wi >= valid) e.window[w] = ps->window[wi];
-            }
-        }
-        use_rec = lv.func == 2 && strategy != kRle && strategy != kHuffmanOnly && s.fv_end < 0 && le_tail_reads_done(e) && ss.preins < p &&
-                  le_tail_record_end(e) > p && le_tail_record_end(e) - p <= kTailRecMax;
-        no_head = use_rec && s.final_run && !e.wr_end && le_no_head_ok(e) && !(s.resume && p - (kWSize - 1) < s.start_pos);
-        if (!no_head) {
-            const int64_t shift = s.resume && ps ? e.base - (ps->base - s.persist_off) : 0;
-            for (int i = tid; i < kHashSize; i += nth) {
-                int64_t hv = s.resume && ps ? (int64_t)ps->head[i] : 0;
-                hv = hv != 0 && hv - shift > 0 ? hv - shift : 0;
-                head32[i] = hv ? (uint32_t)hv + 1u : 0u;
-            }
-        }
-        __syncthreads();
-#ifdef ZS_FV_PROF
-        tk1 = wall_clock64();
-#endif
-        if (e.avail_end > 0) {
-            int64_t lo = p - (kWSize - 1);
-            if (lo < e.base) lo = e.base;
-            if (lo < 0) lo = 0;
-            int64_t hi = p;
-            if (hi > (int64_t)s.n - 5) hi = (int64_t)s.n - 5;
-            const uint32_t *gb = s.ins_bits;
-            auto insf = [gb](int64_t c) { return ((gb[c >> 5] >> (c & 31)) & 1u) != 0; };
-            for (int64_t q = lo + tid; q < hi; q += nth) {
-                if (s.fv_end >= 0) {
-                    if (!insf(q)) continue;
-                    le_restore_prev_ins(e, q, lk, insf);
-                } else {
-                    le_restore_prev(e, q, lk);
+        le_restore_scalars(e, p, base_in, after_in, ss.tail_kind, ss.tail_pend);
+        use_rec = lv.func == 2 && strategy != kRle && strategy != kHuffmanOnly && s.fv_end < 0 && le_tail_use_rec(e, p, ss.preins);
+        no_head = use_rec && le_tail_no_head(e) && !(s.resume && p - (kWSize - 1) < s.start_pos);
+        const TailPrep *tp = s.tail_prep ? prep + (s.tail_prep - 1) : nullptr;
+        took = tp && use_rec && no_head && !ss.link_cut && le_tail_prep_fits(*tp, e, p, preslid, ss.preins);
+        if (took) {
+            for (int i = tid * 16; i < kWindowSize + 512; i += nth * 16) *(uint4 *)(smem + i) = *(const uint4 *)(tp->window + i);
+            for (int i = tid * 8; i < kWSize; i += nth * 8) *(uint4 *)(e.prev + i) = *(const uint4 *)(tp->prev + i);
+            for (int i = tid; i < 2 * kTailRecMax; i += nth) pre_tab[i] = tp->pre_tab[i];
+            le_tail_take(e, *tp, pre_tab, p);
+            __syncthreads();
+        } else {
+            le_restore_image(e, tid, nth, preslid);
+            const int64_t img_base = preslid ? e.base - kWSize : e.base;
+            const bool same_window = s.resume && ps && ps->base - s.persist_off == img_base;
+            if (same_window) {
+                const int64_t valid = e.avail_end - img_base;
+                for (int w = tid; w < kWindowSize + 512; w += nth) {
+                    const int wi = preslid && w < kWSize ? w + kWSize : w;
+                    if (wi >= valid) e.window[w] = ps->window[wi];
                 }
-                if (!no_head && q >= s.start_pos) atomicMax(&head32[le_bucket(e, q)], (uint32_t)(q - e.base) + 1u);
+            }
+            if (!no_head) {
+                const int64_t shift = s.resume && ps ? e.base - (ps->base - s.persist_off) : 0;
+                for (int i = tid; i < kHashSize; i += nth) {
+                    int64_t hv = s.resume && ps ? (int64_t)ps->head[i] : 0;
+                    hv = hv != 0 && hv - shift > 0 ? hv - shift : 0;
+                    head32[i] = hv ? (uint32_t)hv + 1u : 0u;
+                }
             }
             __syncthreads();
 #ifdef ZS_FV_PROF
-            tk2 = wall_clock64();
+            tk1 = wall_clock64();
 #endif
-            if (!no_head)
-                for (int i = tid; i < kHashSize; i += nth) e.head[i] = (uint16_t)(head32[i] ? head32[i] - 1 : 0);
-        }
-        __syncthreads();
+            if (e.avail_end > 0) {
+                int64_t lo = p - (kWSize - 1);
+                if (lo < e.base) lo = e.base;
+                if (lo < 0) lo = 0;
+                int64_t hi = p;
+                if (hi > (int64_t)s.n - 5) hi = (int64_t)s.n - 5;
+                const uint32_t *gb = s.ins_bits;
+                auto insf = [gb](int64_t c) { return ((gb[c >> 5] >> (c & 31)) & 1u) != 0; };
+                for (int64_t q = lo + tid; q < hi; q += nth) {
+                    if (s.fv_end >= 0) {
+                        if (!insf(q)) continue;
+                        le_restore_prev_ins(e, q, lk, insf);
+                    } else {
+                        le_restore_prev(e, q, lk);
+                    }
+                    if (!no_head && q >= s.start_pos) atomicMax(&head32[le_bucket(e, q)], (uint32_t)(q - e.base) + 1u);
+                }
+                __syncthreads();
 #ifdef ZS_FV_PROF
-        tk3 = wall_clock64();
-        pf_restore[0] = tk0 - tk_start, pf_restore[1] = tk1 - tk0, pf_restore[2] = tk2 - tk1, pf_restore[3] = tk3 - tk2;
+                tk2 = wall_clock64();
 #endif
-    }
-    __shared__ uint32_t pre_tab[2 * kTailRecMax];
-    __shared__ uint32_t sh_tail_head[3];
+                if (!no_head)
+                    for (int i = tid; i < kHashSize; i += nth) e.head[i] = (uint16_t)(head32[i] ? head32[i] - 1 : 0);
+            }
+            __syncthreads();
+#ifdef ZS_FV_PROF
+            tk3 = wall_clock64();
+            pf_restore[0] = tk0 - tk_start, pf_restore[1] = tk1 - tk0, pf_restore[2] = tk2 - tk1, pf_restore[3] = tk3 - tk2;
+#endif
+        }
+    }
     {
         const int64_t hi = le_tail_record_end(e);
-        if (use_rec) {
-            for (int64_t q = p + tid; q < (no_head ? e.n - 5 : hi); q += nth) le_restore_prev(e, q, lk);
+        if (use_rec && !took) {
+            le_restore_prev_range(e, p, no_head ? e.n - 5 : hi, lk, tid, nth);
             if (tid < 3) sh_tail_head[tid] = 0;
             __syncthreads();
-            if (no_head) {
-                const uint32_t hb0 = le_tail_head_bucket(e, 0), hb1 = le_tail_head_bucket(e, 1), hb2 = le_tail_head_bucket(e, 2);
-                int64_t lo = p - (kWSize - 1);
-                if (lo < e.base) lo = e.base;
-                if (lo < 1) lo = 1;
-                for (int64_t q = lo + tid; q < e.n - 3; q += nth) {
-                    const uint32_t h = le_bucket(e, q);
-                    if (h == hb0 && q < e.n - 5) atomicMax(&sh_tail_head[0], (uint32_t)(q - e.base));
-                    if (h == hb1 && q < e.n - 4) atomicMax(&sh_tail_head[1], (uint32_t)(q - e.base));
-                    if (h == hb2 && q < e.n - 3) atomicMax(&sh_tail_head[2], (uint32_t)(q - e.base));
-                }
-            }
+            if (no_head) le_tail_head_scan(e, p, tid, nth, [&](int k, uint32_t w) { atomicMax(&sh_tail_head[k], w); });
             __syncthreads();
             e.no_head = no_head ? 1 : 0;
             e.tail_head[0] = (int)sh_tail_head[0], e.tail_head[1] = (int)sh_tail_head[1], e.tail_head[2] = (int)sh_tail_head[2];
-            for (int64_t q = p + tid; q < hi; q += nth) {
-                pre_tab[2 * (q - p)] = le_tail_record(e, (int)(q - e.base), (int)(e.n - q), lv.chain);
-                pre_tab[2 * (q - p) + 1] = le_tail_record(e, (int)(q - e.base), (int)(e.n - q), lv.chain >> 2);
-            }
+            le_tail_records(e, p, hi, pre_tab, tid, nth);
             e.pre_rec = pre_tab, e.pre_lo = p, e.pre_hi = hi;
             __syncthreads();
         }
@@ -2259,6 +2313,7 @@
     if (tid == 0) {
         ss.nsyms = (uint32_t)e.nsyms;
         ss.nblocks = e.nblocks;
+        if (s.tail_prep) ss.tail_prep = took ? 1 : 2;
     }
     if (!ps || s.final_run) return;
     __syncthreads();
@@ -2278,7 +2333,6 @@
     }
 }
 
-constexpr int kTailLds = (int)kScratchHead + 2 * kWSize + 4096;
 constexpr int kFastRunLds = kTailLds + kHeadCacheLds;
 static_assert(kFastRunLds + 1024 <= 160 * 1024, "a run's LDS");
 
diff --git a/zlibstream_amd/csrc/zs_lit_engine.h b/zlibstream_amd/csrc/zs_lit_engine.h
--- a/zlibstream_amd/csrc/zs_lit_engine.h
+++ b/zlibstream_amd/csrc/zs_lit_engine.h
@@ -889,8 +889,7 @@
     else le_run_slow(e, lane, nlanes);
 }
 
-ZS_HD_NOINLINE inline void le_restore(LitEngine &e, int64_t p, int64_t base, int64_t avail_end, int kind, uint32_t pend,
-                                      const uint16_t *link, int64_t preins, int lane, int nlanes, bool preslid = false) {
+ZS_HD void le_restore_scalars(LitEngine &e, int64_t p, int64_t base, int64_t avail_end, int kind, uint32_t pend) {
     e.base = base;
     e.avail_end = avail_end;
     if (e.avail_end > e.n) e.avail_end = e.n;
@@ -906,6 +905,15 @@
         }
         e.cur_wr = lo;
     }
+    e.strstart = (int)(p - e.base);
+    e.lookahead = (int)(e.avail_end - p);
+    e.match_available = (kind == kR) ? 0 : 1;
+    e.match_length = (kind == kXK || kind == kXK4) ? match_len(pend) : kMinMatch - 1;
+    e.match_start = (kind == kXK || kind == kXK4) ? (int)((p - 1 - match_dist(pend)) - e.base) : 0;
+    e.prev_length = kMinMatch - 1;
+    e.prev_match = 0;
+}
+ZS_HD void le_restore_image(LitEngine &e, int lane, int nlanes, bool preslid = false, bool with_head = true) {
     const int64_t ib = preslid ? e.base - kWSize : e.base;
     const int64_t valid = e.avail_end - ib;
     for (int w = lane; w < kWindowSize + 512; w += nlanes) {
@@ -915,15 +923,14 @@
         else if (ib >= kWSize && wi < kWindowSize) v = e.data[ib + wi - kWSize];
         e.window[w] = v;
     }
-    for (int i = lane; i < kHashSize; i += nlanes) e.head[i] = 0;
+    if (with_head)
+        for (int i = lane; i < kHashSize; i += nlanes) e.head[i] = 0;
     for (int i = lane; i < kWSize; i += nlanes) e.prev[i] = 0;
-    e.strstart = (int)(p - e.base);
-    e.lookahead = (int)(e.avail_end - p);
-    e.match_available = (kind == kR) ? 0 : 1;
-    e.match_length = (kind == kXK || kind == kXK4) ? match_len(pend) : kMinMatch - 1;
-    e.match_start = (kind == kXK || kind == kXK4) ? (int)((p - 1 - match_dist(pend)) - e.base) : 0;
-    e.prev_length = kMinMatch - 1;
-    e.prev_match = 0;
+}
+ZS_HD_NOINLINE inline void le_restore(LitEngine &e, int64_t p, int64_t base, int64_t avail_end, int kind, uint32_t pend,
+                                      const uint16_t *link, int64_t preins, int lane, int nlanes, bool preslid = false) {
+    le_restore_scalars(e, p, base, avail_end, kind, pend);
+    le_restore_image(e, lane, nlanes, preslid);
 }
 
 ZS_HD void le_restore_prev(LitEngine &e, int64_t q, const uint16_t *link) {
@@ -946,6 +953,63 @@
     e.prev[(int)(q - e.base) & kWMask] = (uint16_t)(c >= e.base ? c - e.base : 0);
 }
 ZS_HD uint32_t le_bucket(const LitEngine &e, int64_t q) { return le_hash(e, le_load32(e.window + (q - e.base) + 2)); }
+
+ZS_HD int64_t le_tail_prev_lo(const LitEngine &e, int64_t p) {
+    int64_t lo = p - (kWSize - 1);
+    if (lo < e.base) lo = e.base;
+    return lo < 0 ? 0 : lo;
+}
+ZS_HD void le_restore_prev_range(LitEngine &e, int64_t q0, int64_t q1, const uint16_t *link, int lane, int nlanes) {
+    for (int64_t q = q0 + lane; q < q1; q += nlanes) le_restore_prev(e, q, link);
+}
+ZS_HD bool le_tail_use_rec(const LitEngine &e, int64_t p, int64_t preins) {
+    const int64_t hi = le_tail_record_end(e);
+    return le_tail_reads_done(e) && preins < p && hi > p && hi - p <= kTailRecMax;
+}
+ZS_HD bool le_tail_no_head(const LitEngine &e) { return e.final_run && !e.wr_end && le_no_head_ok(e); }
+ZS_HD int64_t le_tail_scan_lo(const LitEngine &e, int64_t p) {
+    const int64_t lo = le_tail_prev_lo(e, p);
+    return lo < 1 ? 1 : lo;
+}
+template <class Max>
+ZS_HD void le_tail_head_scan(const LitEngine &e, int64_t p, int lane, int nlanes, Max &&mx) {
+    const uint32_t hb0 = le_tail_head_bucket(e, 0), hb1 = le_tail_head_bucket(e, 1), hb2 = le_tail_head_bucket(e, 2);
+    for (int64_t q = le_tail_scan_lo(e, p) + lane; q < e.n - 3; q += nlanes) {
+        const uint32_t h = le_bucket(e, q);
+        if (h == hb0 && q < e.n - 5) mx(0, (uint32_t)(q - e.base));
+        if (h == hb1 && q < e.n - 4) mx(1, (uint32_t)(q - e.base));
+        if (h == hb2 && q < e.n - 3) mx(2, (uint32_t)(q - e.base));
+    }
+}
+ZS_HD void le_tail_records(const LitEngine &e, int64_t lo, int64_t hi, uint32_t *tab, int lane, int nlanes) {
+    for (int64_t q = lo + lane; q < hi; q += nlanes) {
+        tab[2 * (q - lo)] = le_tail_record(e, (int)(q - e.base), (int)(e.n - q), e.lv.chain);
+        tab[2 * (q - lo) + 1] = le_tail_record(e, (int)(q - e.base), (int)(e.n - q), e.lv.chain >> 2);
+    }
+}
+struct TailPrep {
+    int32_t valid, preslid, p_lo, hi;
+    int64_t base;
+    int32_t tail_head[3], pad_[3];
+    uint32_t pre_tab[2 * kTailRecMax];
+    uint8_t window[kWindowSize + 512];
+    uint16_t prev[kWSize];
+};
+static_assert(offsetof(TailPrep, window) % 16 == 0 && offsetof(TailPrep, prev) % 16 == 0 && sizeof(TailPrep) % 16 == 0, "16-byte copies");
+ZS_HD bool le_tail_prep_plan(LitEngine &e, int64_t p_lo, int64_t base_in, int64_t after_in, bool &preslid) {
+    preslid = le_tail_preslide(e, p_lo, base_in, after_in, -1);
+    le_restore_scalars(e, p_lo, preslid ? base_in + kWSize : base_in, after_in, kR, 0);
+    return le_tail_use_rec(e, p_lo, -1) && le_tail_no_head(e);
+}
+ZS_HD bool le_tail_prep_fits(const TailPrep &t, const LitEngine &e, int64_t p, bool preslid, int64_t preins) {
+    return t.valid != 0 && t.base == e.base && (t.preslid != 0) == preslid && t.p_lo <= p && p < t.hi && preins < p;
+}
+ZS_HD void le_tail_take(LitEngine &e, const TailPrep &t, const uint32_t *tab, int64_t p) {
+    const int64_t lo = le_tail_scan_lo(e, p);
+    for (int k = 0; k < 3; k++) e.tail_head[k] = e.base + t.tail_head[k] >= lo ? t.tail_head[k] : 0;
+    e.no_head = 1;
+    e.pre_rec = tab, e.pre_lo = t.p_lo, e.pre_hi = t.hi;
+}
 
 struct AllIns {
     ZS_HD bool operator()(int64_t) const { return true; }
```
